# UCL-SML/Doubly-Stochastic-DGP

Hardware: AMD Instinct MI355X
Metric: ELBO-steps/sec (higher is better)
Workload: dtype f64

## Files before the change

### doubly-stochastic-dgp_amd/csrc/chain_policy.hpp

```cpp
#pragma once
#include <stdlib.h>
#include "plan_types.hpp"
#include "../../include/dsdgp.h"

#define XCH 64
#define HEAD_THREADS 512
#define GL_EPI_ROWS 64

#define SM_SMALL_BLOCKS 160
#define SM_BWD_RESIDENT_8W 768
static inline bool sm_small(int Mp, int64_t nblk, int D_in, bool bwd) {
  static const int64_t bwd_lim128 = getenv("DSDGP_SM_BWD_LIM128") ? atoll(getenv("DSDGP_SM_BWD_LIM128")) : SM_BWD_RESIDENT_8W;
  const int64_t lim = Mp > 128 ? ((int64_t)1 << 40) : (bwd ? bwd_lim128 : SM_SMALL_BLOCKS);
  return Mp >= 128 && Mp <= 256 && nblk <= lim && D_in <= XCH;
}
static inline int sm_nw(int Mp, int64_t nblk, int D_in, bool bwd) {
  return (Mp > 512 || (Mp == 512 && D_in <= XCH && !bwd)) ? 16 : (Mp > 256 ? 8 : (sm_small(Mp, nblk, D_in, bwd) ? 8 : 4));
}
static inline int64_t sm_hyp_parts(int64_t ld, int Mp, int D_in) { return (int64_t)sm_nw(Mp, ceil_div(ld, 16), D_in, true) * ceil_div(ld, 16); }
static inline int sm_adj_fusable(int Mp, int64_t nblk, int D_in, int D_out) {
  if (D_in > XCH) return 0;
  const int NW = sm_nw(Mp, nblk, D_in, true);
  const int xch = D_in < XCH ? D_in : XCH;
  return NW * 16 * xch >= 2 * 16 * D_out;
}
static inline int sm_cs_built(int Mp) { return Mp > 256 || Mp == 32 || Mp == 64 || Mp == 128 || Mp == 256; }

static inline bool save_c_enabled(int save_c, int Mp) { return save_c >= 2 || (save_c == 1 && Mp > 256); }
static inline int chain_d_split(int64_t nblk, int D_out) {
  int ds = 1;
  if (nblk < 256) ds = (int)std::min<int64_t>(4, std::max<int64_t>(1, 512 / nblk));
  else if (nblk < 512) ds = (int)std::min<int64_t>(1024 / nblk, D_out / 5);
  if (ds > D_out) ds = D_out;
  return ds < 1 ? 1 : ds;
}
static inline int bwd_d_split(int bwd_split, int Mp, bool has_part, int64_t nblk, int D_out) {
  const bool want = bwd_split >= 2 || (bwd_split == 1 && Mp > 256);
  return (want && has_part) ? chain_d_split(nblk, D_out) : 1;
}
static inline int layer_gemm_lik_blocks(int64_t Rin, int D_out) { return ceil_div(round_up(Rin, 16), GL_EPI_ROWS); }
static inline int head_draw_blocks(int64_t count) { return (int)std::min<int64_t>(64, ceil_div((count + 1) / 2, 4 * HEAD_THREADS)); }

static inline int layer_last_built(int Mp, int D_in, int D_out) { return (Mp == 128 || Mp == 256) && D_out == 1 && D_in <= 16; }
struct LastScope {
  int Mp, D_in, D_out, kern_kind;
  int hyp_rows;
  bool lik, save_A, save_C, want_F;
  int rep;
  bool whitened;
  int mean_kind, d_split;
  int bwd_d_split;
  bool want_E;
};
static inline int layer_last_fusable(const LastScope& s) {
  const int waves = s.Mp == 128 ? 4 : 8;
  return layer_last_built(s.Mp, s.D_in, s.D_out) && (s.kern_kind == DSDGP_KERN_RBF || s.kern_kind == DSDGP_KERN_MATERN52) &&
         s.hyp_rows >= waves && s.lik && s.save_A && !s.save_C && !s.want_F && s.rep == 1 && !s.whitened &&
         s.mean_kind == DSDGP_MEAN_ZERO && s.d_split <= 1 && s.bwd_d_split <= 1 && !s.want_E;
}
```

### doubly-stochastic-dgp_amd/csrc/common.hpp

```cpp
#pragma once
#include <hip/hip_runtime.h>
#include <stdint.h>
#include <stdlib.h>
#include <stdio.h>
#include <string.h>
#include <string>
#include <vector>
#include <map>

#include "../../include/dsdgp.h"

void dsdgp_set_error(const char* fmt, ...);

#define DS_HIP(call)                                                                         \
  do {                                                                                       \
    hipError_t e__ = (call);                                                                 \
    if (e__ != hipSuccess) {                                                                 \
      dsdgp_set_error("%s:%d: %s -> %s", __FILE__, __LINE__, #call, hipGetErrorString(e__)); \
      return DSDGP_ERR_HIP;                                                                  \
    }                                                                                        \
  } while (0)

#define DS_CHECK_ARG(cond)                                                  \
  do {                                                                      \
    if (!(cond)) {                                                          \
      dsdgp_set_error("%s:%d: bad argument: %s", __FILE__, __LINE__, #cond); \
      return DSDGP_ERR_BAD_ARG;                                             \
    }                                                                       \
  } while (0)

#include <atomic>
extern std::atomic<long long> g_dsdgp_launches;
#define DS_LAUNCH(...)                                                   \
  do {                                                                   \
    g_dsdgp_launches.fetch_add(1, std::memory_order_relaxed);            \
    hipLaunchKernelGGL(__VA_ARGS__);                                     \
  } while (0)

#define DS_TRY(call)            \
  do {                          \
    int rc__ = (call);          \
    if (rc__ != DSDGP_OK) return rc__; \
  } while (0)

struct ProfSlot {
  double ms = 0.0;
  int64_t launches = 0;
  std::vector<std::pair<hipEvent_t, hipEvent_t>> pending;
};

struct dsdgp_ctx {
  int device = 0;
  hipStream_t stream = nullptr;
  bool own_stream = false;
  hipStream_t side = nullptr;
  void* scratch = nullptr;
  size_t scratch_bytes = 0;
  int prof_on = 0;
  std::map<std::string, ProfSlot> prof;
  char* pin = nullptr;
  size_t pin_bytes = 0, pin_off = 0;
  void* potrf_plan = nullptr;
  void (*potrf_plan_free)(void*) = nullptr;
  int64_t potrf_key[4] = {0, 0, 0, 0};
};

int ctx_scratch(dsdgp_ctx* ctx, size_t bytes, void** out);
int ctx_upload(dsdgp_ctx* ctx, void* dst, const void* src, size_t bytes);

int multiclass_launch(dsdgp_ctx* ctx, const double* mean, const double* var, const double* Y, int64_t n, int64_t R, int K,
                      int mode, double wgt, double* out, double* dmean, double* dvar, int y_override);
int eval_mixture_launch(dsdgp_ctx* ctx, int kind, double p0, double p1, const double* p0_dev, const double* mean, const double* var,
                        const double* Y, int64_t n, int S, int DY, double* rows_out, double* acc, int accumulate);
int mixture_quantiles_launch(dsdgp_ctx* ctx, const double* mean, const double* var, double noise_var, const double* noise_dev,
                             int64_t n, int S, int DY, const double* probs, int P, double* q_out);
int mixture_calibration_launch(dsdgp_ctx* ctx, const double* mean, const double* var, double noise_var, const double* noise_dev,
                               const double* Y, int64_t n, int S, int DY, const double* probs, int P, double* rows_out, double* acc,
                               int accumulate);
int mixture_classification_launch(dsdgp_ctx* ctx, int kind, const double* mean, const double* var, const double* Y, int64_t n, int S,
                                  int DY, int bins, double* probs_out, double* rows_out, double* acc, int accumulate);

struct ProfScope {
  dsdgp_ctx* ctx;
  const char* name;
  hipEvent_t a = nullptr, b = nullptr;
  hipStream_t st;
  ProfScope(dsdgp_ctx* c, const char* n, hipStream_t stream = nullptr) : ctx(c), name(n), st(stream ? stream : c->stream) {
    if (ctx->prof_on) {
      hipEventCreate(&a);
      hipEventCreate(&b);
      hipEventRecord(a, st);
    }
  }
  ~ProfScope() {
    if (a) {
      hipEventRecord(b, st);
      ctx->prof[name].pending.push_back({a, b});
    }
  }
};

#ifdef __HIPCC__
#define DS_WAVE_ID(tid) __builtin_amdgcn_readfirstlane((int)(tid) >> 6)
#endif
#include "plan_types.hpp"
#define DSDGP_MAX_MP 2048

#ifdef __HIPCC__
typedef double d4 __attribute__((ext_vector_type(4)));
typedef const double __attribute__((address_space(1)))* gcptr;
typedef double __attribute__((address_space(1)))* gptr;
typedef double __attribute__((address_space(3)))* lptr;

#define DS_FIND_SEGMENT(idx, list, n, field, key)            \
  do {                                                       \
    int lo__ = 0, hi__ = (n)-1;                              \
    while (lo__ < hi__) {                                    \
      const int mid__ = (lo__ + hi__ + 1) >> 1;              \
      if ((key) >= (list)[mid__].field) lo__ = mid__;        \
      else hi__ = mid__ - 1;                                 \
    }                                                        \
    idx = lo__;                                              \
  } while (0)

__device__ __forceinline__ d4 mfma_f64(double a, double b, d4 c) {
  return __builtin_amdgcn_mfma_f64_16x16x4f64(a, b, c, 0, 0, 0);
}

__device__ __forceinline__ double sum_groups(double x) {
  const unsigned lo = __double2loint(x), hi = __double2hiint(x);
  const auto a = __builtin_amdgcn_permlane16_swap(lo, lo, false, false);
  const auto b = __builtin_amdgcn_permlane16_swap(hi, hi, false, false);
  const double y = __hiloint2double(b[0], a[0]) + __hiloint2double(b[1], a[1]);
  const unsigned lo2 = __double2loint(y), hi2 = __double2hiint(y);
  const auto c = __builtin_amdgcn_permlane32_swap(lo2, lo2, false, false);
  const auto d = __builtin_amdgcn_permlane32_swap(hi2, hi2, false, false);
  return __hiloint2double(d[0], c[0]) + __hiloint2double(d[1], c[1]);
}
template <int CTRL, int ROWMASK>
__device__ __forceinline__ double dpp_or_zero(double x) {
  const int lo = __builtin_amdgcn_update_dpp(0, __double2loint(x), CTRL, ROWMASK, 0xf, false);
  const int hi = __builtin_amdgcn_update_dpp(0, __double2hiint(x), CTRL, ROWMASK, 0xf, false);
  return __hiloint2double(hi, lo);
}
__device__ __forceinline__ double sum_wave(double x) {
  x += dpp_or_zero<0x111, 0xf>(x);
  x += dpp_or_zero<0x112, 0xf>(x);
  x += dpp_or_zero<0x114, 0xf>(x);
  x += dpp_or_zero<0x118, 0xf>(x);
  x += dpp_or_zero<0x142, 0xa>(x);
  x += dpp_or_zero<0x143, 0xc>(x);
  const unsigned lo = __builtin_amdgcn_readlane((int)__double2loint(x), 63);
  const unsigned hi = __builtin_amdgcn_readlane((int)__double2hiint(x), 63);
  return __hiloint2double(hi, lo);
}

template <int T>
__device__ __forceinline__ double block_sum(double x, double* red) {
  const int tid = threadIdx.x;
  __syncthreads();
  red[tid] = x;
  __syncthreads();
  for (int h = T / 2; h >= 1; h >>= 1) {
    if (tid < h) red[tid] += red[tid + h];
    __syncthreads();
  }
  return red[0];
}

template <int L>
__device__ __forceinline__ double bcast_lane(double x) {
  const unsigned lo = __builtin_amdgcn_readlane((int)__double2loint(x), L);
  const unsigned hi = __builtin_amdgcn_readlane((int)__double2hiint(x), L);
  return __hiloint2double((int)hi, (int)lo);
}

#define HYP_VAR 0
#define HYP_WVAR 1
#define HYP_KDIAG 2
#define HYP_DVAR 3
#define HYP_DWVAR 4
#define HYP_ILS 8

template <int KIND>
__device__ __forceinline__ double kern_val(double r2, double s2) {
  if (KIND == DSDGP_KERN_RBF) return s2 * exp(-0.5 * r2);
  const double s5 = 2.23606797749978969641;
  double r = sqrt(r2 + 1e-12);
  return s2 * (1.0 + s5 * r + (5.0 / 3.0) * (r * r)) * exp(-s5 * r);
}
template <int KIND>
__device__ __forceinline__ void kern_val_grad(double r2, double s2, double& k, double& dk) {
  if (KIND == DSDGP_KERN_RBF) {
    k = s2 * exp(-0.5 * r2);
    dk = -0.5 * k;
    return;
  }
  const double s5 = 2.23606797749978969641;
  double r = sqrt(r2 + 1e-12);
  double e = s2 * exp(-s5 * r);
  k = (1.0 + s5 * r + (5.0 / 3.0) * (r * r)) * e;
  dk = -(5.0 / 6.0) * (1.0 + s5 * r) * e;
}
__device__ __forceinline__ double kern_val_rt(int kind, double r2, double s2) {
  return kind == DSDGP_KERN_RBF ? kern_val<DSDGP_KERN_RBF>(r2, s2) : kern_val<DSDGP_KERN_MATERN52>(r2, s2);
}
#endif
```

### doubly-stochastic-dgp_amd/csrc/forward_plan.hpp

```cpp
#pragma once
#include "chain_policy.hpp"

static_assert(DSDGP_MAX_LAYERS <= 32, "FwdIn::caller_z is a 32-bit mask");
struct FwdIn {
  int64_t n;
  int S;
  bool prepare, save, need_last_F, lik_target, sample_w, with_grad;
  uint32_t caller_z;
  int L;
  bool white, lik_elementwise, lik_gaussian;
  int grad_first;
  bool grad_q_only, head_ok, overlap, timing;
  struct Layer {
    int Mp, M, D_in, D_out, kern_kind, mean_kind, prop;
    bool gemm, alg_g, need_tpt, has_C, has_bpart;
  } layer[DSDGP_MAX_LAYERS];
  struct { int white_fwd, cs_min_blocks, cs_min_dout, cs_max_dout, last_fuse, last_min_blocks, bwd_split, lik_fuse; } force;
};

enum DrawsAt : uint8_t { DRAWS_INLINE, DRAWS_HEAD, DRAWS_SIDE };
enum DrawFrom : uint8_t { DRAW_NONE, DRAW_CALLER, DRAW_HERE, DRAW_READY };
enum FwdLaunch : uint8_t { LAUNCH_CHAIN, LAUNCH_GEMM, LAUNCH_WITH_REVERSE };
enum LikRoute : uint8_t { LIK_NONE, LIK_IN_CHAIN, LIK_ELEMENTWISE, LIK_MULTICLASS };
struct FwdPlan {
  bool join_prep_first;
  DrawsAt draws;
  bool draws_ahead;
  int head_nblk;
  bool adjoints_from_lik, lik_in_chain;
  LikRoute lik;
  int lik_nblocks;
  struct Layer {
    int64_t Rin, ld;
    int rep;
    bool whitened, want_F;
    DrawFrom draw;
    bool save_A, save_C, save_XT1;
    int d_split;
    bool lik_epilogue;
    FwdLaunch launch;
    bool concat;
  } layer[DSDGP_MAX_LAYERS];
  int hyp_rows, bwd_d_split;
};

static inline bool last_chain_fusable(const FwdIn& in, const FwdPlan& p) {
  const int l = in.L - 1;
  const FwdIn::Layer& v = in.layer[l];
  const FwdPlan::Layer& y = p.layer[l];
  if (in.force.last_fuse == 0 || in.force.bwd_split >= 2 || !v.need_tpt || in.white || v.gemm || in.L < 2) return false;
  if (in.grad_q_only && in.grad_first == in.L - 1) return false;
  if (in.timing || ceil_div(y.Rin, 16) < in.force.last_min_blocks) return false;
  return layer_last_fusable(LastScope{v.Mp, v.D_in, v.D_out, v.kern_kind, p.hyp_rows, y.lik_epilogue, y.save_A, y.save_C, y.want_F, y.rep,
                                      y.whitened, v.mean_kind, y.d_split, p.bwd_d_split, !v.alg_g});
}

static inline FwdPlan fwd_plan(const FwdIn& in) {
  FwdPlan p{};
  const int L = in.L;
  const bool wf_ok = !in.white && !in.save && in.force.white_fwd != 0;
  p.join_prep_first = wf_ok;
  p.draws = !in.prepare ? DRAWS_INLINE : (in.head_ok ? DRAWS_HEAD : (in.overlap ? DRAWS_SIDE : DRAWS_INLINE));
  p.adjoints_from_lik = in.lik_target && in.with_grad && L > 1 && in.lik_elementwise;
  p.lik_in_chain = p.adjoints_from_lik && in.lik_gaussian && !in.sample_w && in.force.lik_fuse != 0;
  for (int l = 0; l < L; ++l) {
    const FwdIn::Layer& v = in.layer[l];
    FwdPlan::Layer& y = p.layer[l];
    const bool last = (l == L - 1);
    y.Rin = (l == 0) ? in.n : (int64_t)in.S * in.n;
    y.rep = (l == 0) ? in.S : 1;
    y.ld = round_up(y.Rin, 16);
    const int64_t nblk = y.ld / 16;
    y.want_F = !last || in.need_last_F;
    y.whitened = wf_ok && v.Mp <= 256 && !v.gemm;
    if (!y.want_F) y.draw = DRAW_NONE;
    else if (in.caller_z >> l & 1) y.draw = DRAW_CALLER;
    else y.draw = (p.draws != DRAWS_INLINE && !last) ? DRAW_READY : DRAW_HERE;
    if (y.draw == DRAW_READY) {
      p.draws_ahead = true;
      if (p.draws == DRAWS_HEAD) p.head_nblk = std::max(p.head_nblk, head_draw_blocks((int64_t)in.S * in.n * v.D_out));
    }
    y.save_A = in.save && (in.white || l >= in.grad_first);
    y.save_C = y.save_A && v.has_C && sm_cs_built(v.Mp) &&
               (v.Mp > 256 || (nblk > in.force.cs_min_blocks && v.D_out >= in.force.cs_min_dout && v.D_out <= in.force.cs_max_dout));
    if (v.gemm) y.save_C = y.save_A && v.has_C;
    const bool q_lowest = y.save_A && in.grad_q_only && !in.white && l == in.grad_first;
    if (q_lowest) y.save_C = false;
    y.save_XT1 = y.save_A && !q_lowest;
    y.d_split = chain_d_split(nblk, v.D_out);
    y.lik_epilogue = last && p.lik_in_chain;
    y.launch = v.gemm ? LAUNCH_GEMM : LAUNCH_CHAIN;
    y.concat = v.prop > 0 && !last;
  }
  const FwdIn::Layer& v = in.layer[L - 1];
  const FwdPlan::Layer& y = p.layer[L - 1];
  p.hyp_rows = (int)(sm_hyp_parts(y.ld, v.Mp, v.D_in) / (y.ld / 16));
  p.bwd_d_split = bwd_d_split(in.force.bwd_split, v.Mp, v.has_bpart, y.ld / 16, v.D_out);
  if (last_chain_fusable(in, p)) p.layer[L - 1].launch = LAUNCH_WITH_REVERSE;
  if (in.lik_target) {
    const int64_t R = (int64_t)in.S * in.n;
    p.lik = p.lik_in_chain ? LIK_IN_CHAIN : (in.lik_elementwise ? LIK_ELEMENTWISE : LIK_MULTICLASS);
    if (p.lik_in_chain) p.lik_nblocks = v.gemm ? layer_gemm_lik_blocks(y.Rin, v.D_out) : (int)(y.ld / 16) * y.d_split;
    else if (in.lik_elementwise) p.lik_nblocks = ceil_div((p.adjoints_from_lik ? round_up(R, 16) : R) * v.D_out, 256);
    else p.lik_nblocks = ceil_div(R, 256);
  }
  return p;
}

struct FwdUsed { const double *X, *z; int64_t zs_s, zs_n, zs_d; };
template <class FwdArgs>
struct FwdRecord {
  struct Layer : FwdUsed { int64_t Rin, ld; int rep; bool c_saved; } layer[DSDGP_MAX_LAYERS];
  int64_t n = 0;
  int S = 0;
  bool adjoints_from_lik = false;
  bool last_pending = false;
  FwdArgs last_fwd;
  int hyp_rows = 0;

  void forward_done(const FwdIn& in, const FwdPlan& p, const FwdUsed* used, const FwdArgs* pending) {
    n = in.n; S = in.S; adjoints_from_lik = p.adjoints_from_lik;
    for (int l = 0; l < in.L; ++l) {
      const FwdPlan::Layer& y = p.layer[l];
      Layer& r = layer[l];
      static_cast<FwdUsed&>(r) = used[l];
      r.Rin = y.Rin; r.ld = y.ld; r.rep = y.rep; r.c_saved = y.save_C;
    }
    last_pending = pending != nullptr;
    if (pending) { last_fwd = *pending; hyp_rows = p.hyp_rows; }
  }
  void adjoints_from_caller() { adjoints_from_lik = false; }
  void last_launched() { last_pending = false; }
};
```

### doubly-stochastic-dgp_amd/csrc/layer.hpp

```cpp
#pragma once
#include "common.hpp"
#include "chain_policy.hpp"

struct LayerFwdArgs {
  const double* X;
  int64_t Rin;
  int32_t rep;
  int32_t D_in, D_out, M;
  const double* Zp;
  const double* Zs;
  const double* hyp;
  const double* LinvT;
  const double* Linv;
  const double* Tp;
  const double* TpT;
  const double* qmu;
  int32_t qmu_ld;
  int32_t mean_kind;
  const double* mean_A;
  const double* mean_b;
  const double* z;
  int64_t zs_s, zs_n, zs_d;
  int64_t n_inner;
  double jitter;
  double* F;
  double* mean;
  double* var;
  double* Asave;
  double* Csave;
  int64_t ldA;
  int32_t d_split;
  double* XT1;
  unsigned long long* phase_clk;
  const double* lik_Y;
  const double* lik_const;
  double lik_w;
  double* lik_part;
  double *lik_MB, *lik_VB;
  int64_t lik_ld;
};

struct LayerBwdArgs {
  const double* X;
  int64_t Rin;
  int32_t D_in, D_out, M, DP4;
  const double* Zp;
  const double* Zs;
  const double* hyp;
  const double* Kinv;
  const double* Linv;
  const double* LinvT;
  const double* Sd;
  const double* qmu4;
  const double* Asave;
  const double* Csave;
  const double* Tp;
  const double* TpT;
  int64_t ldA;
  const double* VB;
  const double* MB;
  double* E;
  double* GW;
  double* dX;
  int32_t mean_kind;
  const double* mean_A;
  double* hyp_part;
  double* MBp;
  double* VBp;
  const double* zp;
  int64_t zp_s, zp_n, zp_d, n_inner;
  const double* varp;
  int32_t Dp, prop;
  double jitter;
  unsigned long long* phase_clk;
  int32_t d_split;
  double* part;
  int* part_cnt;
  const double* up_dF;
  int32_t up_rep, up_ld, up_off;
  const double* up_z;
  int64_t up_zs, up_zn, up_zd, up_n_inner;
  const double* up_var;
  double up_jitter;
  double *MBw, *VBw;
};

int wgrad_launch(dsdgp_ctx* ctx, const WgradJob* jobs_dev, int njobs, int total_tasks, int nsplit, int64_t ld, int64_t Rp,
                 hipStream_t stream = nullptr);
int layer_fwd_sm_launch(dsdgp_ctx* ctx, const LayerFwdArgs& a, int Mp, int kern_kind, int white);
int layer_bwd_sm_launch(dsdgp_ctx* ctx, const LayerBwdArgs& a, int Mp, int kern_kind, int white);
int layer_last_launch(dsdgp_ctx* ctx, const LayerFwdArgs& a, const LayerBwdArgs& b, int Mp, int kern_kind, int hyp_rows);

struct GemmLayerWs {
  double* T1;
  double* T2;
  double* Pb;
  double* colsq;
  double* MUT;
  double* qmuT;
  double* ZZ;
  double* OUTt;
  double* svar;
  int64_t pb_doubles;
};
#define GL_MAX_GROUPS 4
int layer_gemm_hyp_parts(int64_t ld, int Mp);
int layer_fwd_gemm_launch(dsdgp_ctx* ctx, const LayerFwdArgs& a, int Mp, int kern_kind, int white, const GemmLayerWs& ws);
int layer_bwd_gemm_launch(dsdgp_ctx* ctx, const LayerBwdArgs& b, int Mp, int kern_kind, int white, const GemmLayerWs& ws);
```

### doubly-stochastic-dgp_amd/csrc/layer_sm.hip

```cpp
#include <stdlib.h>

#include "layer.hpp"

int layer_fwd_sm_a(dsdgp_ctx*, const LayerFwdArgs&, int, int, int, int);
int layer_fwd_sm_b(dsdgp_ctx*, const LayerFwdArgs&, int, int, int, int);
int layer_fwd_sm_c(dsdgp_ctx*, const LayerFwdArgs&, int, int, int, int);
int layer_bwd_sm_a(dsdgp_ctx*, const LayerBwdArgs&, int, int, int, int);
int layer_bwd_sm_b(dsdgp_ctx*, const LayerBwdArgs&, int, int, int, int);
int layer_bwd_sm_c(dsdgp_ctx*, const LayerBwdArgs&, int, int, int, int);

int layer_fwd_sm_launch(dsdgp_ctx* ctx, const LayerFwdArgs& a, int Mp, int kern_kind, int white) {
  const int small = sm_small(Mp, ceil_div(a.Rin, 16), a.D_in, false);
  if (Mp < 128) return layer_fwd_sm_a(ctx, a, Mp, kern_kind, white, small);
  if (Mp <= 256) return layer_fwd_sm_b(ctx, a, Mp, kern_kind, white, small);
  return layer_fwd_sm_c(ctx, a, Mp, kern_kind, white, small);
}
int layer_bwd_sm_launch(dsdgp_ctx* ctx, const LayerBwdArgs& a, int Mp, int kern_kind, int white) {
  const int small = sm_small(Mp, ceil_div(a.ldA, 16), a.D_in, true);
  if (Mp < 128) return layer_bwd_sm_a(ctx, a, Mp, kern_kind, white, small);
  if (Mp <= 256) return layer_bwd_sm_b(ctx, a, Mp, kern_kind, white, small);
  return layer_bwd_sm_c(ctx, a, Mp, kern_kind, white, small);
}
```

### doubly-stochastic-dgp_amd/csrc/layer_sm_impl.hpp

```cpp
#pragma once
#include <stdlib.h>

#include "layer.hpp"

template <bool D4>
__device__ __forceinline__ int act_slot(int m) {
  return D4 ? ((m & ~15) | ((m & 3) << 2) | ((m >> 2) & 3)) : m;
}
template <bool D4>
__device__ __forceinline__ int out_slot(int ib, int g, int t) {
  return D4 ? 16 * ib + 4 * g + t : 16 * ib + g + 4 * t;
}

template <int Mp, bool D4>
__device__ __forceinline__ d4 chain_block(const double* __restrict__ WR, const double* __restrict__ WT,
                                          const double* __restrict__ actb, int ib, int kb, int g, int c, d4 acc) {
  if constexpr (D4) {
    const d4 w4 = *reinterpret_cast<const d4*>(WR + (int64_t)(16 * ib + c) * Mp + 16 * kb + 4 * g);
#pragma unroll
    for (int s = 0; s < 4; ++s) acc = mfma_f64(w4[s], actb[(16 * kb + 4 * s + g) * 16 + c], acc);
  } else {
    const double* __restrict__ w = WT + (int64_t)(16 * kb + g) * Mp + 16 * ib + c;
#pragma unroll
    for (int s = 0; s < 4; ++s) acc = mfma_f64(w[(int64_t)(4 * s) * Mp], actb[(16 * kb + 4 * s + g) * 16 + c], acc);
  }
  return acc;
}

template <int Mp, bool D4>
__device__ __forceinline__ d4 chain_range(const double* __restrict__ WR, const double* __restrict__ WT,
                                          const double* __restrict__ actb, int ib, int lo, int hi, int g, int c, d4 acc) {
  if constexpr (D4) {
#pragma unroll 4
    for (int kb = lo; kb < hi; ++kb) acc = chain_block<Mp, true>(WR, WT, actb, ib, kb, g, c, acc);
    return acc;
  } else {
    if (lo >= hi) return acc;
    const unsigned off = (unsigned)(g * Mp + 16 * ib + c);
    auto wld = [&](int kbx, int s) { return (WT + (size_t)(16 * kbx + 4 * s) * Mp)[off]; };
    double wa[4], wb[4];
    int kb = lo;
#pragma unroll
    for (int s = 0; s < 4; ++s) wa[s] = wld(kb, s);
    while (kb + 1 < hi) {
#pragma unroll
      for (int s = 0; s < 4; ++s) wb[s] = wld(kb + 1, s);
#pragma unroll
      for (int s = 0; s < 4; ++s) acc = mfma_f64(wa[s], actb[(16 * kb + 4 * s + g) * 16 + c], acc);
      ++kb;
      if (kb + 1 < hi) {
#pragma unroll
        for (int s = 0; s < 4; ++s) wa[s] = wld(kb + 1, s);
      }
#pragma unroll
      for (int s = 0; s < 4; ++s) acc = mfma_f64(wb[s], actb[(16 * kb + 4 * s + g) * 16 + c], acc);
      ++kb;
    }
    if (kb < hi) {
#pragma unroll
      for (int s = 0; s < 4; ++s) acc = mfma_f64(wa[s], actb[(16 * kb + 4 * s + g) * 16 + c], acc);
    }
    return acc;
  }
}

template <int Mp, bool UPPER>
__device__ __forceinline__ void chain_range2(const double* __restrict__ WT, const double* __restrict__ actb, int ib0, int ib1, int nkb,
                                             int g, int c, d4& acc0, d4& acc1) {
  const unsigned off0 = (unsigned)(g * Mp + 16 * ib0 + c), off1 = (unsigned)(g * Mp + 16 * ib1 + c);
  auto wld = [&](int kbx, int s, unsigned off) { return (WT + (size_t)(16 * kbx + 4 * s) * Mp)[off]; };
  if constexpr (UPPER) {
    acc0 = chain_range<Mp, false>(nullptr, WT, actb, ib0, ib0, ib1, g, c, acc0);
  }
  const int lo = UPPER ? ib1 : 0, hi = UPPER ? nkb : ib0 + 1;
  if (lo < hi) {
    double a0[4], a1[4];
    int kb = lo;
#pragma unroll
    for (int s = 0; s < 4; ++s) {
      a0[s] = wld(kb, s, off0);
      a1[s] = wld(kb, s, off1);
    }
    for (; kb + 1 < hi; ++kb) {
#pragma unroll
      for (int s = 0; s < 4; ++s) {
        const double bv = actb[(16 * kb + 4 * s + g) * 16 + c];
        acc0 = mfma_f64(a0[s], bv, acc0);
        acc1 = mfma_f64(a1[s], bv, acc1);
        a0[s] = wld(kb + 1, s, off0);
        a1[s] = wld(kb + 1, s, off1);
      }
#pragma unroll
      for (int s = 0; s < 4; ++s) {
        __builtin_amdgcn_sched_group_barrier(0x008, 2, 0);
        __builtin_amdgcn_sched_group_barrier(0x020, 2, 0);
      }
    }
#pragma unroll
    for (int s = 0; s < 4; ++s) {
      const double bv = actb[(16 * kb + 4 * s + g) * 16 + c];
      acc0 = mfma_f64(a0[s], bv, acc0);
      acc1 = mfma_f64(a1[s], bv, acc1);
    }
  }
  if constexpr (!UPPER) {
    acc1 = chain_range<Mp, false>(nullptr, WT, actb, ib1, ib0 + 1, ib1 + 1, g, c, acc1);
  }
}

template <int Mp, int MPB>
__device__ __forceinline__ void chain_dense2(const double* __restrict__ WT, const double* __restrict__ actb, int ib0, int ib1, int g, int c,
                                             d4& acc0, d4& acc1) {
  const unsigned off0 = (unsigned)(g * Mp + 16 * ib0 + c), off1 = (unsigned)(g * Mp + 16 * ib1 + c);
  auto wld = [&](int kbx, int s, unsigned off) { return (WT + (size_t)(16 * kbx + 4 * s) * Mp)[off]; };
  double a0[4], a1[4];
#pragma unroll
  for (int s = 0; s < 4; ++s) {
    a0[s] = wld(0, s, off0);
    a1[s] = wld(0, s, off1);
  }
  double bv = actb[g * 16 + c];
#pragma unroll
  for (int kb = 0; kb < MPB; ++kb) {
#pragma unroll
    for (int s = 0; s < 4; ++s) {
      const int kn = (s == 3) ? (kb + 1) % MPB : kb, sn = (s + 1) & 3;
      const double bvn = actb[(16 * kn + 4 * sn + g) * 16 + c];
      acc0 = mfma_f64(a0[s], bv, acc0);
      acc1 = mfma_f64(a1[s], bv, acc1);
      if (kb + 1 < MPB) {
        a0[s] = wld(kb + 1, s, off0);
        a1[s] = wld(kb + 1, s, off1);
      }
      bv = bvn;
      if (kb + 1 < MPB) __builtin_amdgcn_sched_barrier(0);
    }
  }
}

template <int MPB, int NW>
struct Own {
  static constexpr int NQ = (MPB + NW - 1) / NW;
  static __device__ __forceinline__ int ib(int wave, int q) {
    if (NQ >= 2) return (q & 1) ? (q >> 1) * (2 * NW) + (2 * NW - 1) - wave : (q >> 1) * (2 * NW) + wave;
    return wave;
  }
  static __device__ __forceinline__ bool skip(int ib) { return (MPB % NW != 0) && ib >= MPB; }
  static __device__ __forceinline__ bool active(int wave) { return MPB >= NW || wave < MPB; }
};

template <int MPB, int NW>
struct OwnCS {
  static constexpr bool CUSTOM = (NW == 8) && (MPB == 8 || MPB == 16);
  static constexpr int NQ = CUSTOM ? MPB / 8 : Own<MPB, NW>::NQ;
  static constexpr int NLOAD = CUSTOM ? 4 : NW;
  static __device__ __forceinline__ int ib(int wave, int q) {
    if constexpr (!CUSTOM) return Own<MPB, NW>::ib(wave, q);
    if constexpr (MPB == 8) return wave < 4 ? wave : 11 - wave;
    if (wave < 4) return q == 0 ? 7 - wave : wave;
    return q == 0 ? 19 - wave : 4 + wave;
  }
  static __device__ __forceinline__ bool active(int wave) { return CUSTOM || Own<MPB, NW>::active(wave); }
};

static inline constexpr int sm_db(int NW) { return NW == 4 ? 8 : (NW == 8 ? 4 : 1); }

struct SmLds {
  int xs, act, red, total;
};
static inline SmLds sm_lds(int Mp, int D_in, int D_out, int NW, bool wide, int nbuf = 1) {
  SmLds L;
  int o = 0;
  const int xch = D_in < XCH ? D_in : XCH;
  L.xs = o; o += 16 * (xch + 1);
  o = (int)round_up(o, 2);
  L.act = o; o += Mp * 16;
  L.red = o;
  const bool mu_early = (NW == 4) && !wide;
  const int db = sm_db(NW);
  const int red_fwd = NW * 16 + 2 * db * NW * 16 + (mu_early ? NW * 16 * D_out : 2 * db * NW * 16);
  const int red_bwd = NW * 16 * xch;
  int red = red_fwd > red_bwd ? red_fwd : red_bwd;
  if (nbuf == 2 && red < Mp * 16) red = Mp * 16;
  o += red;
  L.total = o;
  return L;
}

template <int NW>
__device__ __forceinline__ void stage_x_over_l(const double* X, const double* ils, double* xs, int Din, int j0, int jn, int64_t r0,
                                               int64_t Rin, int tid) {
  for (int idx = tid; idx < 16 * jn; idx += NW * 64) {
    const int rr = idx / jn, j = idx % jn;
    int64_t row = r0 + rr;
    if (row > Rin - 1) row = Rin - 1;
    xs[rr * (jn + 1) + j] = X[row * Din + j0 + j] * ils[j0 + j];
  }
}

template <int NQ, int MPB, int NW>
__device__ __forceinline__ void sqdist_chunk_masked(const double* __restrict__ zs, const double* xs, int Din, int j0, int jn, int wave,
                                                    int g, int c, d4 (&zx)[NQ], double (&zsq)[NQ], double& xx) {
  for (int kk = 0; kk < jn; kk += 16) {
    const int ns = (jn - kk >= 16) ? 4 : (jn - kk + 3) >> 2;
    double b[4];
    int jc[4];
    bool in[4];
#pragma unroll
    for (int s = 0; s < 4; ++s) {
      const int j = kk + 4 * s + g;
      in[s] = j < jn;
      jc[s] = in[s] ? j : jn - 1;
      const double v = xs[c * (jn + 1) + jc[s]];
      b[s] = in[s] ? v : 0.0;
      xx = fma(b[s], b[s], xx);
    }
#pragma unroll
    for (int q = 0; q < NQ; ++q) {
      const int ib = Own<MPB, NW>::ib(wave, q);
      if (Own<MPB, NW>::skip(ib)) continue;
      const double* __restrict__ zr = zs + (int64_t)(16 * ib + c) * Din + j0;
      double av[4];
#pragma unroll
      for (int s = 0; s < 4; ++s) {
        if (s < ns) {
          const double v = zr[jc[s]];
          av[s] = in[s] ? v : 0.0;
        }
      }
#pragma unroll
      for (int s = 0; s < 4; ++s) {
        if (s < ns) {
          zx[q] = mfma_f64(av[s], b[s], zx[q]);
          zsq[q] = fma(av[s], av[s], zsq[q]);
        }
      }
    }
  }
}
template <int NQ>
__device__ __forceinline__ void sqdist_finish(const d4 (&zx)[NQ], const double (&zsq)[NQ], double xx, double* scratch, int wave, int g,
                                              int c, d4 (&r2)[NQ]) {
  xx = sum_groups(xx);
  double* zrow = scratch + wave * NQ * 16;
#pragma unroll
  for (int q = 0; q < NQ; ++q) {
    const double zq = sum_groups(zsq[q]);
    if (g == 0) zrow[q * 16 + c] = zq;
  }
  __builtin_amdgcn_wave_barrier();
#pragma unroll
  for (int q = 0; q < NQ; ++q)
#pragma unroll
    for (int t = 0; t < 4; ++t) {
      const double v = zrow[q * 16 + g + 4 * t] + xx - 2.0 * zx[q][t];
      r2[q][t] = v > 0.0 ? v : 0.0;
    }
}
template <int NQ, int MPB, int NW>
__device__ __forceinline__ void sqdist_narrow(const double* __restrict__ zs, const double* xs, int Din, int wave, int g, int c, bool act,
                                              double* scratch, d4 (&r2)[NQ]) {
  d4 zx[NQ];
  double zsq[NQ];
#pragma unroll
  for (int q = 0; q < NQ; ++q) { zx[q] = (d4){0, 0, 0, 0}; zsq[q] = 0.0; }
  double xx = 0.0;
  if (act) sqdist_chunk_masked<NQ, MPB, NW>(zs, xs, Din, 0, Din, wave, g, c, zx, zsq, xx);
  sqdist_finish<NQ>(zx, zsq, xx, scratch, wave, g, c, r2);
}

template <int NQ, int MPB, int NW>
__device__ __forceinline__ void sm_sqdist(const double* __restrict__ zs, const double* __restrict__ X,
                                          const double* __restrict__ ils, double* xs, int Din, int64_t r0, int64_t Rin,
                                          int tid, int wave, int g, int c, bool act, double* scratch, d4 (&r2)[NQ]) {
  d4 zx[NQ];
  double zsq[NQ];
#pragma unroll
  for (int q = 0; q < NQ; ++q) { zx[q] = (d4){0, 0, 0, 0}; zsq[q] = 0.0; }
  double xx = 0.0;
  for (int j0 = 0; j0 < Din; j0 += XCH) {
    const int jn = (Din - j0 < XCH) ? Din - j0 : XCH;
    if (j0 > 0) __syncthreads();
    stage_x_over_l<NW>(X, ils, xs, Din, j0, jn, r0, Rin, tid);
    __syncthreads();
    if (act) {
      if ((jn & 15) == 0 && (Din & 3) == 0) {
#pragma unroll
        for (int u = 0; u < XCH / 16; ++u) {
          const int kk = 16 * u;
          if (kk >= jn) break;
          double b[4];
#pragma unroll
          for (int s = 0; s < 4; ++s) {
            b[s] = xs[c * (jn + 1) + kk + 4 * g + s];
            xx = fma(b[s], b[s], xx);
          }
#pragma unroll
          for (int q = 0; q < NQ; ++q) {
            const int ib = Own<MPB, NW>::ib(wave, q);
            if (Own<MPB, NW>::skip(ib)) continue;
            const d4 av = *reinterpret_cast<const d4*>(zs + (int64_t)(16 * ib + c) * Din + j0 + kk + 4 * g);
#pragma unroll
            for (int s = 0; s < 4; ++s) {
              zx[q] = mfma_f64(av[s], b[s], zx[q]);
// ... 239 lines not shown
  }
  fprintf(stderr, "[span] %d wgs: launch %.1f us | wg duration avg %.1f max %.1f us | start avg %.1f max %.1f us | %d late starters (avg duration %.1f us)\n",
          nwg, span, dur / nwg, dur_max, start / nwg, start_max, nlate, nlate ? late / nlate : 0.0);
  if (nwg >= 512) {
    double ds[8] = {0}, dx[8] = {0};
    int ns[8] = {0}, nx[8] = {0};
    for (int w = 0; w < nwg; ++w) {
      const double d = (double)(h[(size_t)w * 8 + last_slot] - h[(size_t)w * 8]) * 0.01;
      const int k = std::min(w >> 8, 7);
      ds[k] += d; ++ns[k]; dx[w & 7] += d; ++nx[w & 7];
    }
    fprintf(stderr, "[span]   mean duration by slot w >> 8:");
    for (int k = 0; k < 8 && ns[k]; ++k) fprintf(stderr, " %.1f", ds[k] / ns[k]);
    fprintf(stderr, " | by XCD w & 7:");
    for (int x = 0; x < 8; ++x) fprintf(stderr, " %.1f", dx[x] / std::max(nx[x], 1));
    fprintf(stderr, "\n");
  }
}
#define FWD_STAMP(i) do { if (a.phase_clk && tid == 0 && blockIdx.y == 0) a.phase_clk[(int64_t)blockIdx.x * 8 + (i)] = __builtin_amdgcn_s_memrealtime(); } while (0)
template <int MPB, int NW, bool WIDE, bool LIK>
constexpr int fwd_min_waves() { return (LIK && NW == 4) ? 5 : ((NW == 8 && MPB == 16 && !WIDE && !LIK) ? 4 : 1); }
template <int MPB, int NW, int KIND, bool WHITE, bool WIDE, bool LIK>
__global__ __launch_bounds__(NW * 64, (fwd_min_waves<MPB, NW, WIDE, LIK>())) void k_layer_fwd_sm(const LayerFwdArgs a, const SmLds L) {
  extern __shared__ __attribute__((aligned(16))) double smem[];
  constexpr int Mp = MPB * 16, NQ = Own<MPB, NW>::NQ;
  constexpr bool D4 = (MPB > 16);
  constexpr bool ILV = D4 || (MPB >= 16);
  const int Din = a.D_in, Dout = a.D_out;
  const int qld = a.qmu_ld ? a.qmu_ld : Dout;
  const int tid = threadIdx.x, lane = tid & 63, wave = DS_WAVE_ID(tid);
  const int g = lane >> 4, c = lane & 15;
  double* xs = smem + L.xs;
  double* actb = smem + L.act;
  double* red_s1 = smem + L.red;
  constexpr int DB = sm_db(NW);
  double* red_s2 = red_s1 + NW * 16;
  double* red_mu = red_s2 + 2 * DB * NW * 16;
  constexpr bool MU_EARLY = (NW == 4) && !WIDE;
  const double* ils = a.hyp + HYP_ILS;
  const int64_t r0 = (int64_t)blockIdx.x * 16;
  const bool act = Own<MPB, NW>::active(wave);
  const double s2 = a.hyp[HYP_VAR];
  FWD_STAMP(0);

  if (a.XT1 && blockIdx.y == 0) store_xt1<NW>(a, r0, tid);
  {
    d4 r2[NQ];
    if constexpr (!WIDE) {
      stage_x_over_l<NW>(a.X, ils, xs, Din, 0, Din, r0, a.Rin, tid);
      __syncthreads();
      sqdist_narrow<NQ, MPB, NW>(a.Zs, xs, Din, wave, g, c, act, red_s1, r2);
    } else {
      sm_sqdist<NQ, MPB, NW>(a.Zs, a.X, ils, xs, Din, r0, a.Rin, tid, wave, g, c, act, red_s1, r2);
    }
    if (act) {
#pragma unroll
      for (int q = 0; q < NQ; ++q) {
        const int ib = Own<MPB, NW>::ib(wave, q);
        if (Own<MPB, NW>::skip(ib)) continue;
        kuf_tile_store<KIND, D4>(r2[q], s2, a.M, actb, ib, g, c);
      }
    }
  }
  __syncthreads();
  FWD_STAMP(1);

  d4 acc[NQ];
#pragma unroll
  for (int q = 0; q < NQ; ++q) acc[q] = (d4){0, 0, 0, 0};
  constexpr bool PAIR = (NQ == 2) && !D4 && (MPB % NW == 0);
  if (act) {
    if constexpr (PAIR) {
      chain_range2<Mp, false>(a.LinvT, actb, Own<MPB, NW>::ib(wave, 0), Own<MPB, NW>::ib(wave, 1), MPB, g, c, acc[0], acc[1]);
    } else {
#pragma unroll
      for (int q = 0; q < NQ; ++q) {
        const int ib = Own<MPB, NW>::ib(wave, q);
        if (Own<MPB, NW>::skip(ib)) continue;
        acc[q] = chain_range<Mp, D4>(a.Linv, a.LinvT, actb, ib, 0, ib + 1, g, c, acc[q]);
      }
    }
  }
  sumsq_partial<NQ>(acc, red_s1, wave, g, c, act);
  __syncthreads();
  if (act) {
#pragma unroll
    for (int q = 0; q < NQ; ++q) {
      const int ib = Own<MPB, NW>::ib(wave, q);
      if (Own<MPB, NW>::skip(ib)) continue;
#pragma unroll
      for (int t = 0; t < 4; ++t) actb[out_slot<D4>(ib, g, t) * 16 + c] = acc[q][t];
    }
  }
  __syncthreads();
  FWD_STAMP(2);
  if (!WHITE) {
#pragma unroll
    for (int q = 0; q < NQ; ++q) acc[q] = (d4){0, 0, 0, 0};
    if (act) {
      if constexpr (PAIR) {
        chain_range2<Mp, true>(a.Linv, actb, Own<MPB, NW>::ib(wave, 0), Own<MPB, NW>::ib(wave, 1), MPB, g, c, acc[0], acc[1]);
      } else {
#pragma unroll
        for (int q = 0; q < NQ; ++q) {
          const int ib = Own<MPB, NW>::ib(wave, q);
          if (Own<MPB, NW>::skip(ib)) continue;
          acc[q] = chain_range<Mp, D4>(a.LinvT, a.Linv, actb, ib, ib, MPB, g, c, acc[q]);
        }
      }
    }
    __syncthreads();
    if (act) {
#pragma unroll
      for (int q = 0; q < NQ; ++q) {
        const int ib = Own<MPB, NW>::ib(wave, q);
        if (Own<MPB, NW>::skip(ib)) continue;
#pragma unroll
        for (int t = 0; t < 4; ++t) actb[out_slot<D4>(ib, g, t) * 16 + c] = acc[q][t];
      }
    }
  }
  FWD_STAMP(3);
  if constexpr (MU_EARLY) {
    for (int d0 = 0; d0 < Dout; d0 += 16) {
      d4 mu4 = (d4){0, 0, 0, 0};
      if (act) {
        const bool din = d0 + c < Dout;
        const int dc = din ? d0 + c : Dout - 1;
#pragma unroll
        for (int q = 0; q < NQ; ++q) {
          const int ib = Own<MPB, NW>::ib(wave, q);
          if (Own<MPB, NW>::skip(ib)) continue;
          double qv[4];
#pragma unroll
          for (int t = 0; t < 4; ++t) qv[t] = a.qmu[(int64_t)(16 * ib + g + 4 * t) * qld + dc];
#pragma unroll
          for (int t = 0; t < 4; ++t) mu4 = mfma_f64(din ? qv[t] : 0.0, acc[q][t], mu4);
        }
      }
#pragma unroll
      for (int t = 0; t < 4; ++t) {
        const int d = d0 + g + 4 * t;
        if (d < Dout) red_mu[(wave * Dout + d) * 16 + c] = mu4[t];
      }
    }
  }
  __syncthreads();
  FWD_STAMP(4);

  const double kdiag = a.hyp[HYP_KDIAG];
  const double lik_s2 = LIK ? a.lik_const[0] : 1.0;
  const double lik_c0 = -0.91893853320467274178 - 0.5 * log(lik_s2);
  double lik_ve = 0.0, lik_dl = 0.0;
  const int dchunk = (Dout + (int)gridDim.y - 1) / (int)gridDim.y;
  const int d_lo = (int)blockIdx.y * dchunk, d_hi = (d_lo + dchunk < Dout) ? d_lo + dchunk : Dout;
  for (int d0 = d_lo, grp = 0; d0 < d_hi; d0 += DB, ++grp) {
    const int gs = (d_hi - d0 < DB) ? d_hi - d0 : DB;
    double* rs2 = red_s2 + (grp & 1) * DB * NW * 16;
    double* rmu_g = red_mu + (grp & 1) * DB * NW * 16;
    for (int dd = 0; dd < gs; ++dd) {
      const int d = d0 + dd;
      d4 cacc[NQ];
#pragma unroll
      for (int q = 0; q < NQ; ++q) cacc[q] = (d4){0, 0, 0, 0};
      if (act) {
        const double* __restrict__ TdT = a.TpT + (int64_t)d * Mp * Mp;
        const double* __restrict__ Td = a.Tp + (int64_t)d * Mp * Mp;
        if constexpr (PAIR) {
          chain_range2<Mp, true>(Td, actb, Own<MPB, NW>::ib(wave, 0), Own<MPB, NW>::ib(wave, 1), MPB, g, c, cacc[0], cacc[1]);
        } else {
#pragma unroll
          for (int q = 0; q < NQ; ++q) {
            const int ib = Own<MPB, NW>::ib(wave, q);
            if (Own<MPB, NW>::skip(ib)) continue;
            cacc[q] = chain_range<Mp, D4>(TdT, Td, actb, ib, ib, MPB, g, c, cacc[q]);
          }
        }
      }
      double p = 0.0, mu = 0.0;
      if (act) {
        if (a.Csave) {
          const int64_t r = r0 + c;
          double* __restrict__ Cd = a.Csave + ((int64_t)blockIdx.x * Dout + d) * (Mp * 16) + c;
#pragma unroll
          for (int q = 0; q < NQ; ++q) {
            const int ib = Own<MPB, NW>::ib(wave, q);
            if (Own<MPB, NW>::skip(ib)) continue;
#pragma unroll
            for (int t = 0; t < 4; ++t) {
              const double cv = (r < a.Rin) ? cacc[q][t] : 0.0;
              Cd[out_slot<D4>(ib, g, t) * 16] = cv;
            }
          }
        }
#pragma unroll
        for (int q = 0; q < NQ; ++q) {
          const int ib = Own<MPB, NW>::ib(wave, q);
          if (Own<MPB, NW>::skip(ib)) continue;
#pragma unroll
          for (int t = 0; t < 4; ++t) {
            p = fma(cacc[q][t], cacc[q][t], p);
            if constexpr (!MU_EARLY) mu = fma(acc[q][t], a.qmu[(int64_t)(16 * ib + g + 4 * t) * qld + d], mu);
          }
        }
      }
      p = sum_groups(p);
      if constexpr (!MU_EARLY) mu = sum_groups(mu);
      if (g == 0) {
        rs2[(dd * NW + wave) * 16 + c] = p;
        if constexpr (!MU_EARLY) rmu_g[(dd * NW + wave) * 16 + c] = mu;
      }
    }
    __syncthreads();
    const bool flat = a.rep > 1 && a.mean_kind != DSDGP_MEAN_LINEAR;
    const int n_items = 16 * gs * (flat ? a.rep : 1);
    for (int e = tid; e < n_items; e += NW * 64) {
      const int s0 = flat ? e / (16 * gs) : 0, e2 = e % (16 * gs);
      const int cc = e2 / gs, dd = e2 % gs, d = d0 + dd;
      const int64_t r = r0 + cc;
      if (r >= a.Rin) {
        if (LIK && r < a.lik_ld && s0 == 0) {
          a.lik_MB[(int64_t)d * a.lik_ld + r] = 0.0;
          a.lik_VB[(int64_t)d * a.lik_ld + r] = 0.0;
        }
        continue;
      }
      double s1 = 0.0, s2sum = 0.0, mu = 0.0;
#pragma unroll
      for (int w = 0; w < NW; ++w) {
        s1 += red_s1[w * 16 + cc];
        s2sum += rs2[(dd * NW + w) * 16 + cc];
        mu += MU_EARLY ? red_mu[(w * Dout + d) * 16 + cc] : rmu_g[(dd * NW + w) * 16 + cc];
      }
      const double var = kdiag - s1 + s2sum;
      if (a.mean_kind == DSDGP_MEAN_IDENTITY) {
        mu += a.X[r * Din + d];
      } else if (a.mean_kind == DSDGP_MEAN_LINEAR) {
        double m2 = 0.0;
        for (int j = 0; j < Din; ++j) m2 = fma(a.X[r * Din + j], a.mean_A[(int64_t)j * Dout + d], m2);
        mu += m2 + (a.mean_b ? a.mean_b[d] : 0.0);
      }
      const double sd = sqrt(var + a.jitter);
      const int s_lo = flat ? s0 : 0, s_hi = flat ? s0 + 1 : a.rep;
      for (int s = s_lo; s < s_hi; ++s) {
        const int64_t orow = (int64_t)s * a.Rin + r;
        const int64_t o = orow * Dout + d;
        if (a.mean) a.mean[o] = mu;
        if (a.var) a.var[o] = var;
        if (a.F && a.z) {
          const double zv = a.z[(orow / a.n_inner) * a.zs_s + (orow % a.n_inner) * a.zs_n + d * a.zs_d];
          a.F[o] = mu + zv * sd;
        }
        if constexpr (LIK) {
          const double y = a.lik_Y[(orow % a.n_inner) * Dout + d];
          const double q = (y - mu) * (y - mu) + var;
          lik_ve += lik_c0 - 0.5 * q / lik_s2;
          lik_dl += -0.5 / lik_s2 + 0.5 * q / (lik_s2 * lik_s2);
          a.lik_MB[(int64_t)d * a.lik_ld + orow] = -a.lik_w * (y - mu) / lik_s2;
          a.lik_VB[(int64_t)d * a.lik_ld + orow] = 0.5 * a.lik_w / lik_s2;
        }
      }
    }
  }
  if constexpr (LIK) {
    lik_ve = sum_wave(lik_ve);
    lik_dl = sum_wave(lik_dl);
    __syncthreads();
    if (lane == 0) {
      red_s1[2 * wave] = lik_ve;
      red_s1[2 * wave + 1] = lik_dl;
    }
    __syncthreads();
    if (tid == 0) {
      double sv = 0.0, sd2 = 0.0;
      for (int w = 0; w < NW; ++w) {
        sv += red_s1[2 * w];
        sd2 += red_s1[2 * w + 1];
      }
      const int64_t wg = (int64_t)blockIdx.y * gridDim.x + blockIdx.x;
      a.lik_part[2 * wg] = sv;
      a.lik_part[2 * wg + 1] = sd2;
    }
  }
  FWD_STAMP(5);
  if (act && a.Asave && blockIdx.y == 0) {
    const int64_t r = r0 + c;
    if (r < a.ldA) {
#pragma unroll
      for (int q = 0; q < NQ; ++q) {
        const int ib = Own<MPB, NW>::ib(wave, q);
        if (Own<MPB, NW>::skip(ib)) continue;
#pragma unroll
        for (int t = 0; t < 4; ++t)
          a.Asave[(int64_t)(16 * ib + g + 4 * t) * a.ldA + r] = (r < a.Rin) ? actb[out_slot<D4>(ib, g, t) * 16 + c] : 0.0;
      }
    }
  }
  FWD_STAMP(6);
}

#define BWD_STAMP(i) do { if (a.phase_clk && tid == 0) a.phase_clk[(int64_t)blockIdx.x * 8 + (i)] = __builtin_amdgcn_s_memrealtime(); } while (0)
template <int MPB, int NW, bool WIDE, bool CS>
constexpr int bwd_min_waves() { return (NW == 8 && !WIDE && !CS) ? (MPB <= 8 ? 6 : 4) : ((NW == 4 && MPB == 8 && !WIDE && !CS) ? 5 : 1); }
template <int MPB, int NW, int KIND, bool WHITE, bool WIDE, bool CS>
__global__ __launch_bounds__(NW * 64, (bwd_min_waves<MPB, NW, WIDE, CS>())) void k_layer_bwd_sm(const LayerBwdArgs a, const SmLds L) {
  extern __shared__ __attribute__((aligned(16))) double smem[];
  constexpr int Mp = MPB * 16, NQ = Own<MPB, NW>::NQ;
  constexpr bool D4 = (MPB > 16);
  constexpr bool ILV = D4 || (MPB >= 16);
  const int Din = a.D_in, Dout = a.D_out;
  const int tid = threadIdx.x, lane = tid & 63, wave = tid >> 6;
  const int g = lane >> 4, c = lane & 15;
  const double* __restrict__ zs = a.Zs;
  double* xs = smem + L.xs;
  double* actb = smem + L.act;
  double* redx = smem + L.red;
  const double* ils = a.hyp + HYP_ILS;
  const int64_t r0 = (int64_t)blockIdx.x * 16;
  const bool act = Own<MPB, NW>::active(wave);
  const double s2 = a.hyp[HYP_VAR];
  const int64_t r = r0 + c;
  const bool rin = r < a.ldA, rvalid = r < a.Rin;
  BWD_STAMP(0);
  if (a.up_dF) adjoint_prologue<NW>(a, redx, L.total - L.red, r0, tid);
  d4 av[NQ], acc[NQ];
#pragma unroll
  for (int q = 0; q < NQ; ++q) {
    const int ib = Own<MPB, NW>::ib(wave, q);
    acc[q] = av[q] = (d4){0, 0, 0, 0};
    if (Own<MPB, NW>::skip(ib)) continue;
    const bool live = act && rin;
    const double* __restrict__ ap = a.Asave + (int64_t)(16 * (act ? ib : 0) + g) * a.ldA + (rin ? r : 0);
    double ld[4];
#pragma unroll
    for (int t = 0; t < 4; ++t) ld[t] = ap[(int64_t)(4 * t) * a.ldA];
#pragma unroll
    for (int t = 0; t < 4; ++t) {
      const double v = live ? ld[t] : 0.0;
      av[q][t] = v;
      if (!CS && act) actb[out_slot<D4>(ib, g, t) * 16 + c] = v;
    }
  }
  if constexpr (!WIDE) stage_x_over_l<NW>(a.X, ils, xs, Din, 0, Din, r0, a.Rin, tid);
  const double bv0l = a.MB[(int64_t)g * a.ldA + (rin ? r : 0)];
  const double bv1l = a.MB[(int64_t)(a.DP4 > 4 ? 4 + g : g) * a.ldA + (rin ? r : 0)];
  const double bv0 = (act && rin) ? bv0l : 0.0;
  const double bv1 = (act && rin && a.DP4 > 4) ? bv1l : 0.0;
  double gsum = 0.0;
  const int n_split = (int)gridDim.y;
  const int dchunk = (Dout + n_split - 1) / n_split;
  const int d_lo = (int)blockIdx.y * dchunk, d_hi = (d_lo + dchunk < Dout) ? d_lo + dchunk : Dout;
  __shared__ int s_ticket;
  auto merge_split = [&](auto& T, auto ib_of) -> bool {
    if (n_split == 1) return true;
    constexpr int NT = sizeof(T) / sizeof(T[0]);
    const int64_t pstride = (int64_t)Mp * 16 + 16;
    double* mine = a.part + ((int64_t)blockIdx.x * n_split + blockIdx.y) * pstride;
#pragma unroll
    for (int q = 0; q < NT; ++q) {
      const int ib = ib_of(q);
      if (ib < 0) continue;
#pragma unroll
      for (int t = 0; t < 4; ++t) __hip_atomic_store(&mine[(16 * ib + g + 4 * t) * 16 + c], T[q][t], __ATOMIC_RELAXED, __HIP_MEMORY_SCOPE_AGENT);
    }
    if (wave == 0 && g == 0) __hip_atomic_store(&mine[Mp * 16 + c], gsum, __ATOMIC_RELAXED, __HIP_MEMORY_SCOPE_AGENT);
    asm volatile("s_waitcnt vmcnt(0)" ::: "memory");
    __syncthreads();
    if (tid == 0) s_ticket = __hip_atomic_fetch_add(a.part_cnt + blockIdx.x, 1, __ATOMIC_RELAXED, __HIP_MEMORY_SCOPE_AGENT);
    __syncthreads();
    if (s_ticket != n_split - 1) return false;
    if (tid == 0) __hip_atomic_store(a.part_cnt + blockIdx.x, 0, __ATOMIC_RELAXED, __HIP_MEMORY_SCOPE_AGENT);
    const double* base = a.part + (int64_t)blockIdx.x * n_split * pstride;
#pragma unroll
    for (int q = 0; q < NT; ++q) T[q] = (d4){0, 0, 0, 0};
    gsum = 0.0;
    for (int y = 0; y < n_split; ++y) {
      const double* p = base + y * pstride;
#pragma unroll
      for (int q = 0; q < NT; ++q) {
        const int ib = ib_of(q);
        if (ib < 0) continue;
#pragma unroll
        for (int t = 0; t < 4; ++t) T[q][t] += __hip_atomic_load(&p[(16 * ib + g + 4 * t) * 16 + c], __ATOMIC_RELAXED, __HIP_MEMORY_SCOPE_AGENT);
      }
      gsum += __hip_atomic_load(&p[Mp * 16 + c], __ATOMIC_RELAXED, __HIP_MEMORY_SCOPE_AGENT);
    }
    return true;
  };
  BWD_STAMP(1);
  if constexpr (CS) {
    using OC = OwnCS<MPB, NW>;
    constexpr bool DBUF = (MPB <= 16);
    constexpr int NLT = OC::NLOAD * 64;
    constexpr int NS = Mp * 16 / (NLT * 2);
    double* buf1 = DBUF ? smem + L.red : actb;
    const bool stager = tid < NLT;
    const int e0 = 2 * tid;
    const int scc = e0 & 15;
    typedef double d2 __attribute__((ext_vector_type(2)));
    d2 tmp[NS];
    auto stage_load = [&](int d) {
      if (!stager) return;
      const d2 v2 = 2.0 * *reinterpret_cast<const d2*>(a.VB + (int64_t)d * a.ldA + r0 + scc);
      const double* __restrict__ Cd = a.Csave + ((int64_t)blockIdx.x * Dout + d) * (Mp * 16) + e0;
#pragma unroll
      for (int i = 0; i < NS; ++i) tmp[i] = v2 * *reinterpret_cast<const d2*>(Cd + i * 2 * NLT);
    };
    auto stage_store = [&](double* buf) {
      if (!stager) return;
#pragma unroll
      for (int i = 0; i < NS; ++i) *reinterpret_cast<d2*>(buf + e0 + i * 2 * NLT) = tmp[i];
    };
    constexpr bool PREF = (NW < 16);
    d4 cacc[OC::NQ];
#pragma unroll
    for (int q = 0; q < OC::NQ; ++q) cacc[q] = (d4){0, 0, 0, 0};
    const bool cact = OC::active(wave);
    if (PREF && d_lo < d_hi) stage_load(d_lo);
    if (DBUF && d_lo < d_hi) stage_store(actb);
    for (int d = d_lo; d < d_hi; ++d) {
      gsum += rin ? a.VB[(int64_t)d * a.ldA + r] : 0.0;
      const int dpar = (d - d_lo) & 1;
      double* cur = (DBUF && dpar) ? buf1 : actb;
      if (DBUF) {
        if (d + 1 < d_hi) stage_load(d + 1);
        __syncthreads();
      } else {
        __syncthreads();
        if (!PREF) stage_load(d);
        stage_store(actb);
        __syncthreads();
        if (PREF && d + 1 < d_hi) stage_load(d + 1);
      }
      if (cact) {
        const double* __restrict__ Td = a.Tp + (int64_t)d * Mp * Mp;
        const double* __restrict__ TdT = a.TpT + (int64_t)d * Mp * Mp;
#pragma unroll
        for (int q = 0; q < OC::NQ; ++q) {
          const int ib = OC::ib(wave, q);
          if (!OC::CUSTOM && Own<MPB, NW>::skip(ib)) continue;
#pragma unroll 4
          for (int kb = 0; kb <= ib; ++kb) cacc[q] = chain_block<Mp, D4>(Td, TdT, cur, ib, kb, g, c, cacc[q]);
        }
      }
      if (DBUF && d + 1 < d_hi) stage_store(dpar ? actb : buf1);
    }
    if (!merge_split(cacc, [&](int q) { const int ib = OC::ib(wave, q); return (cact && (OC::CUSTOM || !Own<MPB, NW>::skip(ib))) ? ib : -1; })) return;
    if (cact) {
      for (int sp = 0; sp < a.DP4 / 4; ++sp) {
        const double bv = sp == 0 ? bv0 : (sp == 1 ? bv1 : (rin ? a.MB[(int64_t)(4 * sp + g) * a.ldA + r] : 0.0));
#pragma unroll
        for (int q = 0; q < OC::NQ; ++q) {
          const int ib = OC::ib(wave, q);
          if (!OC::CUSTOM && Own<MPB, NW>::skip(ib)) continue;
          cacc[q] = mfma_f64(a.qmu4[(int64_t)(16 * ib + c) * a.DP4 + 4 * sp + g], bv, cacc[q]);
        }
      }
    }
    __syncthreads();
    if (cact) {
#pragma unroll
      for (int q = 0; q < OC::NQ; ++q) {
        const int ib = OC::ib(wave, q);
        if (!OC::CUSTOM && Own<MPB, NW>::skip(ib)) continue;
#pragma unroll
        for (int t = 0; t < 4; ++t) actb[out_slot<D4>(ib, g, t) * 16 + c] = cacc[q][t];
      }
    }
    __syncthreads();
    if (WHITE) {
      if (act) {
#pragma unroll
        for (int q = 0; q < NQ; ++q) {
          const int ib = Own<MPB, NW>::ib(wave, q);
          if (Own<MPB, NW>::skip(ib)) continue;
#pragma unroll
          for (int t = 0; t < 4; ++t) actb[out_slot<D4>(ib, g, t) * 16 + c] -= 2.0 * gsum * av[q][t];
        }
      }
      __syncthreads();
    }
  } else {
  __syncthreads();
  constexpr bool PAIRD = (NQ == 2) && !D4 && (MPB % NW == 0);
  if constexpr (PAIRD) {
    const int ib0 = Own<MPB, NW>::ib(wave, 0), ib1 = Own<MPB, NW>::ib(wave, 1);
    const unsigned off0 = (unsigned)(g * Mp + 16 * ib0 + c), off1 = (unsigned)(g * Mp + 16 * ib1 + c);
    const int t_last = d_hi * MPB - 1;
    auto wld = [&](int t, int s, unsigned off) { return (a.Sd + (size_t)(16 * t + 4 * s) * Mp)[off]; };
    double w0[4], w1[4];
    if (d_lo < d_hi) {
#pragma unroll
      for (int s = 0; s < 4; ++s) {
        w0[s] = wld(d_lo * MPB, s, off0);
        w1[s] = wld(d_lo * MPB, s, off1);
      }
    }
    const int64_t rc = rin ? r : 0;
    double vd_next = d_lo < d_hi ? a.VB[(int64_t)d_lo * a.ldA + rc] : 0.0;
    for (int d = d_lo; d < d_hi; ++d) {
      const double vd = rin ? vd_next : 0.0;
      gsum += vd;
      const double vd2 = 2.0 * vd;
      d4 y0 = (d4){0, 0, 0, 0}, y1 = (d4){0, 0, 0, 0};
      double bv = actb[g * 16 + c];
#pragma unroll
      for (int kb = 0; kb < MPB; ++kb) {
        int tn = d * MPB + kb + 1;
        if (kb == MPB - 1 && tn > t_last) tn = t_last;
#pragma unroll
        for (int s = 0; s < 4; ++s) {
          const int kn = (s == 3) ? (kb + 1) % MPB : kb, sn = (s + 1) & 3;
          const double bvn = actb[(16 * kn + 4 * sn + g) * 16 + c];
          y0 = mfma_f64(w0[s], bv, y0);
          y1 = mfma_f64(w1[s], bv, y1);
          w0[s] = wld(tn, s, off0);
          w1[s] = wld(tn, s, off1);
          bv = bvn;
          if (kb == 1 && s == 0) vd_next = a.VB[(int64_t)(d + 1 < d_hi ? d + 1 : d) * a.ldA + rc];
          __builtin_amdgcn_sched_barrier(0);
        }
      }
#pragma unroll
      for (int t = 0; t < 4; ++t) {
        acc[0][t] = fma(vd2, y0[t], acc[0][t]);
        acc[1][t] = fma(vd2, y1[t], acc[1][t]);
      }
    }
  } else
  for (int d = d_lo; d < d_hi; ++d) {
    const double vd = rin ? a.VB[(int64_t)d * a.ldA + r] : 0.0;
    gsum += vd;
    const double vd2 = 2.0 * vd;
    if (act) {
      const double* __restrict__ Sd = a.Sd + (int64_t)d * Mp * Mp;
      if constexpr (ILV) {
        d4 y[NQ];
#pragma unroll
        for (int q = 0; q < NQ; ++q) y[q] = (d4){0, 0, 0, 0};
#pragma unroll 4
        for (int kb = 0; kb < MPB; ++kb) {
#pragma unroll
          for (int q = 0; q < NQ; ++q) {
            const int ibq = Own<MPB, NW>::ib(wave, q);
            if (!Own<MPB, NW>::skip(ibq)) y[q] = chain_block<Mp, D4>(Sd, Sd, actb, ibq, kb, g, c, y[q]);
          }
        }
#pragma unroll
        for (int q = 0; q < NQ; ++q)
#pragma unroll
          for (int t = 0; t < 4; ++t) acc[q][t] = fma(vd2, y[q][t], acc[q][t]);
      } else {
#pragma unroll
        for (int q = 0; q < NQ; ++q) {
          const int ib = Own<MPB, NW>::ib(wave, q);
          if (Own<MPB, NW>::skip(ib)) continue;
          const double* __restrict__ W = Sd + 16 * ib + c + (int64_t)g * Mp;
          d4 y = (d4){0, 0, 0, 0};
#pragma unroll 4
          for (int kb = 0; kb < MPB; ++kb) {
#pragma unroll
            for (int s = 0; s < 4; ++s)
              y = mfma_f64(W[(int64_t)(16 * kb + 4 * s) * Mp], actb[(16 * kb + 4 * s + g) * 16 + c], y);
          }
#pragma unroll
          for (int t = 0; t < 4; ++t) acc[q][t] = fma(vd2, y[t], acc[q][t]);
        }
      }
    }
  }
  if (!merge_split(acc, [&](int q) { const int ib = Own<MPB, NW>::ib(wave, q); return (act && !Own<MPB, NW>::skip(ib)) ? ib : -1; })) return;
  }
  BWD_STAMP(2);
  if constexpr (!CS) {
  if (act) {
    for (int sp = 0; sp < a.DP4 / 4; ++sp) {
      const double bv = sp == 0 ? bv0 : (sp == 1 ? bv1 : (rin ? a.MB[(int64_t)(4 * sp + g) * a.ldA + r] : 0.0));
#pragma unroll
      for (int q = 0; q < NQ; ++q) {
        const int ib = Own<MPB, NW>::ib(wave, q);
        if (Own<MPB, NW>::skip(ib)) continue;
        acc[q] = mfma_f64(a.qmu4[(int64_t)(16 * ib + c) * a.DP4 + 4 * sp + g], bv, acc[q]);
      }
    }
  }
  __syncthreads();
  if (act) {
#pragma unroll
    for (int q = 0; q < NQ; ++q) {
      const int ib = Own<MPB, NW>::ib(wave, q);
      if (Own<MPB, NW>::skip(ib)) continue;
#pragma unroll
      for (int t = 0; t < 4; ++t) {
        if (WHITE) acc[q][t] -= 2.0 * gsum * av[q][t];
        actb[out_slot<D4>(ib, g, t) * 16 + c] = acc[q][t];
      }
    }
  }
  __syncthreads();
  }
  BWD_STAMP(3);
  d4 bb[NQ];
#pragma unroll
  for (int q = 0; q < NQ; ++q) bb[q] = (d4){0, 0, 0, 0};
  constexpr bool PAIRK = (NQ == 2) && !D4 && !CS && (MPB % NW == 0);
  if constexpr (PAIRK) {
    if constexpr (WHITE) {
      const int wu = DS_WAVE_ID(tid);
      chain_range2<Mp, true>(a.Linv, actb, Own<MPB, NW>::ib(wu, 0), Own<MPB, NW>::ib(wu, 1), MPB, g, c, bb[0], bb[1]);
    } else {
      chain_dense2<Mp, MPB>(a.Kinv, actb, Own<MPB, NW>::ib(wave, 0), Own<MPB, NW>::ib(wave, 1), g, c, bb[0], bb[1]);
    }
  } else
  if (act) {
    if (WHITE || !ILV) {
#pragma unroll
      for (int q = 0; q < NQ; ++q) {
        const int ib = Own<MPB, NW>::ib(wave, q);
        if (Own<MPB, NW>::skip(ib)) continue;
#pragma unroll 4
        for (int kb = (WHITE ? ib : 0); kb < MPB; ++kb)
          bb[q] = WHITE ? chain_block<Mp, D4>(a.LinvT, a.Linv, actb, ib, kb, g, c, bb[q])
                        : chain_block<Mp, D4>(a.Kinv, a.Kinv, actb, ib, kb, g, c, bb[q]);
      }
    } else {
#pragma unroll 4
      for (int kb = 0; kb < MPB; ++kb) {
#pragma unroll
        for (int q = 0; q < NQ; ++q) {
          const int ibq = Own<MPB, NW>::ib(wave, q);
          if (!Own<MPB, NW>::skip(ibq)) bb[q] = chain_block<Mp, D4>(a.Kinv, a.Kinv, actb, ibq, kb, g, c, bb[q]);
        }
      }
    }
  }
  BWD_STAMP(4);
  d4 r2[NQ];
  if constexpr (WIDE) sm_sqdist<NQ, MPB, NW>(zs, a.X, ils, xs, Din, r0, a.Rin, tid, wave, g, c, act, redx, r2);
  else sqdist_narrow<NQ, MPB, NW>(zs, xs, Din, wave, g, c, act, redx, r2);
  __syncthreads();
  BWD_STAMP(5);
  double svar = 0.0;
  if (act) {
#pragma unroll
    for (int q = 0; q < NQ; ++q) {
      const int ib = Own<MPB, NW>::ib(wave, q);
      if (Own<MPB, NW>::skip(ib)) continue;
#pragma unroll
      for (int t = 0; t < 4; ++t) {
        const int m = 16 * ib + g + 4 * t;
        const double e = WHITE ? bb[q][t] : bb[q][t] - gsum * av[q][t];
        const double kbar = WHITE ? e : e - gsum * av[q][t];
        bb[q][t] = kbar_to_w<KIND>(kbar, r2[q][t], s2, rvalid && (m < a.M), svar);
        if (rin && a.E) a.E[(int64_t)m * a.ldA + r] = e;
      }
    }
  }
  BWD_STAMP(6);
  double* hp = hyp_part_row(a, NW, wave);
  hyp_head_store(svar, gsum, s2, rvalid, hp, wave, lane);
  if constexpr (!(NW == 4 && MPB == 8 && !WIDE && !CS)) {
    input_side_epilogue<NQ, MPB, NW, WIDE>(a, bb, xs, redx, hp, r0, tid, wave, g, c, act);
  } else {
    for (int j0 = 0; j0 < Din; j0 += XCH) {
      const int jn = (Din - j0 < XCH) ? Din - j0 : XCH;
      const bool single = 16 * jn <= NW * 64;
      double pre_mb = 0.0, pre_z = 0.0, pre_var = 1.0;
      if ((a.dX || a.MBp) && single && tid < 16 * jn) {
        const int j = a.MBp ? tid / 16 : tid % jn, cc = a.MBp ? tid % 16 : tid / jn;
        const int64_t row = r0 + cc;
        if (row < a.Rin) {
          if (a.mean_kind == DSDGP_MEAN_IDENTITY) pre_mb = a.MB[(int64_t)(j0 + j) * a.ldA + row];
          const int d = j0 + j - a.prop;
          if (a.MBp && d >= 0) {
            pre_z = a.zp[(row / a.n_inner) * a.zp_s + (row % a.n_inner) * a.zp_n + d * a.zp_d];
            pre_var = a.varp[row * a.Dp + d];
          }
        }
      }
      double w1 = 0.0;
      if (act) {
#pragma unroll
        for (int q = 0; q < NQ; ++q)
#pragma unroll
          for (int t = 0; t < 4; ++t) w1 += bb[q][t];
      }
      w1 = sum_groups(w1);
      for (int kk = 0; kk < jn; kk += 16) {
        d4 wz = (d4){0, 0, 0, 0}, z2 = (d4){0, 0, 0, 0};
        if (act) {
          const int jc = (kk + c < jn) ? kk + c : jn - 1;
#pragma unroll
          for (int q = 0; q < NQ; ++q) {
            const int ib = Own<MPB, NW>::ib(wave, q);
            if (Own<MPB, NW>::skip(ib)) continue;
            double zv[4];
#pragma unroll
            for (int t = 0; t < 4; ++t) zv[t] = zs[(int64_t)(16 * ib + g + 4 * t) * Din + j0 + jc];
#pragma unroll
            for (int t = 0; t < 4; ++t) {
              wz = mfma_f64(zv[t], bb[q][t], wz);
              z2 = mfma_f64(zv[t] * zv[t], bb[q][t], z2);
            }
          }
        }
#pragma unroll
        for (int t = 0; t < 4; ++t) {
          const int j = kk + g + 4 * t;
          const bool in = j < jn;
          const double xv = xs[c * (jn + 1) + (in ? j : jn - 1)];
          if ((a.dX || a.MBp) && in) redx[(wave * jn + j) * 16 + c] = act ? fma(xv, w1, -wz[t]) : 0.0;
          double sl = act ? fma(xv * xv, w1, fma(-2.0 * xv, wz[t], z2[t])) : 0.0;
          sl += dpp_or_zero<0x111, 0xf>(sl);
          sl += dpp_or_zero<0x112, 0xf>(sl);
          sl += dpp_or_zero<0x114, 0xf>(sl);
          sl += dpp_or_zero<0x118, 0xf>(sl);
          if (c == 15 && in) hp[2 + j0 + j] = -2.0 * ils[j0 + j] * sl;
        }
      }
      if (a.dX || a.MBp) {
        __syncthreads();
        for (int idx = tid; idx < 16 * jn; idx += NW * 64) {
          const int j = a.MBp ? idx / 16 : idx % jn, cc = a.MBp ? idx % 16 : idx / jn;
          const int64_t row = r0 + cc;
          if (row < a.Rin) {
            double sx = 0.0;
#pragma unroll
            for (int w = 0; w < NW; ++w) sx += redx[(w * jn + j) * 16 + cc];
            double dx = 2.0 * ils[j0 + j] * sx;
            if (a.mean_kind == DSDGP_MEAN_IDENTITY) {
              dx += single ? pre_mb : a.MB[(int64_t)(j0 + j) * a.ldA + row];
            } else if (a.mean_kind == DSDGP_MEAN_LINEAR) {
              for (int d = 0; d < Dout; ++d) dx = fma(a.mean_A[(int64_t)(j0 + j) * Dout + d], a.MB[(int64_t)d * a.ldA + row], dx);
            }
            if (a.MBp) {
              const int d = j0 + j - a.prop;
              if (d >= 0) {
                const double zv = single ? pre_z : a.zp[(row / a.n_inner) * a.zp_s + (row % a.n_inner) * a.zp_n + d * a.zp_d];
                const double vv = single ? pre_var : a.varp[row * a.Dp + d];
                a.MBp[(int64_t)d * a.ldA + row] = dx;
                a.VBp[(int64_t)d * a.ldA + row] = dx * zv * 0.5 * rsqrt(vv + a.jitter);
              }
            } else {
              a.dX[row * Din + j0 + j] = dx;
            }
          } else if (a.MBp && row < a.ldA && j0 + j >= a.prop) {
            a.MBp[(int64_t)(j0 + j - a.prop) * a.ldA + row] = 0.0;
            a.VBp[(int64_t)(j0 + j - a.prop) * a.ldA + row] = 0.0;
          }
        }
      }
    }
  }
  if (act && rin) acc_to_global<NQ, MPB, NW>(bb, a.GW, a.ldA, r, true, wave, g);
  BWD_STAMP(7);
}


template <int MPB, int NW, int KIND, bool WHITE, bool WIDE, bool LIK>
static int fwd_sm_go2(dsdgp_ctx* ctx, const LayerFwdArgs& a) {
  const SmLds L = sm_lds(MPB * 16, a.D_in, a.D_out, NW, WIDE);
  const size_t lds = (size_t)L.total * sizeof(double);
  if (lds > 160 * 1024) {
    dsdgp_set_error("layer_fwd(sm): needs %zu B LDS (> 160 KiB): D_out too large for this M", lds);
    return DSDGP_ERR_UNSUPPORTED;
  }
  if (lds > 64 * 1024)
    {
      static int lds_set = 0;
      if ((int)lds > lds_set) {
        DS_HIP(hipFuncSetAttribute((const void*)k_layer_fwd_sm<MPB, NW, KIND, WHITE, WIDE, LIK>, hipFuncAttributeMaxDynamicSharedMemorySize, (int)lds));
        lds_set = (int)lds;
      }
    }
  ProfScope ps(ctx, "layer_fwd");
  const int nrow = ceil_div(a.Rin, 16);
  int ds = a.d_split > 0 ? a.d_split : 1;
  if (ds > a.D_out) ds = a.D_out;
  static const bool timing = getenv("DSDGP_FWD_TIMING") != nullptr;
  if (timing) {
    unsigned long long* clk = nullptr;
    DS_HIP(hipMalloc(&clk, (size_t)nrow * 8 * sizeof(unsigned long long)));
    LayerFwdArgs b = a;
    b.phase_clk = clk;
    DS_LAUNCH((k_layer_fwd_sm<MPB, NW, KIND, WHITE, WIDE, LIK>), dim3(nrow, ds), dim3(NW * 64), lds, ctx->stream, b, L);
    DS_HIP(hipStreamSynchronize(ctx->stream));
    std::vector<unsigned long long> h((size_t)nrow * 8);
    DS_HIP(hipMemcpy(h.data(), clk, h.size() * sizeof(unsigned long long), hipMemcpyDeviceToHost));
    hipFree(clk);
    double ph[6] = {0, 0, 0, 0, 0, 0};
    for (int w = 0; w < nrow; ++w)
      for (int i = 0; i < 6; ++i) ph[i] += (double)(h[(size_t)w * 8 + i + 1] - h[(size_t)w * 8 + i]);
    phase_span_report(h, nrow, 6);
    const double u = 0.01 / nrow;
    fprintf(stderr, "[fwd phases] Mp=%d NW=%d D_out=%d wgs=%dx%d  us/wg: Kuf tile %.2f | a1 %.2f | a %.2f | mean partials %.2f | per-output + epilogue %.2f | "
            "Asave %.2f | sum %.2f\n", MPB * 16, NW, a.D_out, nrow, ds, ph[0] * u, ph[1] * u, ph[2] * u, ph[3] * u, ph[4] * u,
            ph[5] * u, (ph[0] + ph[1] + ph[2] + ph[3] + ph[4] + ph[5]) * u);
    return DSDGP_OK;
  }
  DS_LAUNCH((k_layer_fwd_sm<MPB, NW, KIND, WHITE, WIDE, LIK>), dim3(nrow, ds), dim3(NW * 64), lds, ctx->stream, a, L);
  DS_HIP(hipGetLastError());
  return DSDGP_OK;
}
template <int MPB, int NW, int KIND, bool WHITE, bool WIDE>
static int fwd_sm_go(dsdgp_ctx* ctx, const LayerFwdArgs& a) {
  if (a.lik_Y) return fwd_sm_go2<MPB, NW, KIND, WHITE, WIDE, true>(ctx, a);
  return fwd_sm_go2<MPB, NW, KIND, WHITE, WIDE, false>(ctx, a);
}
template <int MPB, int NW, int KIND, bool WHITE, bool WIDE, bool CS>
static int bwd_phase_timing(dsdgp_ctx* ctx, const LayerBwdArgs& a0, const SmLds& L, size_t lds) {
  const int nwg = (int)ceil_div(a0.ldA, 16);
  unsigned long long* clk = nullptr;
  DS_HIP(hipMalloc(&clk, (size_t)nwg * 8 * sizeof(unsigned long long)));
  LayerBwdArgs a = a0;
  a.phase_clk = clk;
  DS_LAUNCH((k_layer_bwd_sm<MPB, NW, KIND, WHITE, WIDE, CS>), dim3(nwg, a.d_split > 1 ? a.d_split : 1), dim3(NW * 64), lds, ctx->stream, a, L);
  DS_HIP(hipStreamSynchronize(ctx->stream));
  std::vector<unsigned long long> h((size_t)nwg * 8);
  DS_HIP(hipMemcpy(h.data(), clk, h.size() * sizeof(unsigned long long), hipMemcpyDeviceToHost));
  hipFree(clk);
  double ph[7] = {0, 0, 0, 0, 0, 0, 0};
  for (int w = 0; w < nwg; ++w) {
    for (int i = 0; i < 7; ++i) ph[i] += (double)(h[(size_t)w * 8 + i + 1] - h[(size_t)w * 8 + i]);
  }
  phase_span_report(h, nwg, 7);
  const double u = 0.01 / nwg;
  fprintf(stderr, "[bwd phases] Mp=%d NW=%d D_out=%d wgs=%d  us/wg: A-tile %.2f | d-loop %.2f | mean+abar %.2f | Kinv %.2f | x-stage %.2f | "
          "kernel+E/GW %.2f | hyp+dX %.2f | sum %.2f\n", MPB * 16, NW, a.D_out, nwg, ph[0] * u, ph[1] * u, ph[2] * u, ph[3] * u, ph[4] * u, ph[5] * u,
          ph[6] * u, (ph[0] + ph[1] + ph[2] + ph[3] + ph[4] + ph[5] + ph[6]) * u);
  return DSDGP_OK;
}
template <int MPB, int NW, int KIND, bool WHITE, bool WIDE, bool CS>
static int bwd_sm_go2(dsdgp_ctx* ctx, const LayerBwdArgs& a) {
  const SmLds L = sm_lds(MPB * 16, a.D_in, a.D_out, NW, WIDE, (CS && MPB <= 16) ? 2 : 1);
  const size_t lds = (size_t)L.total * sizeof(double);
  if (lds > 160 * 1024) {
    dsdgp_set_error("layer_bwd(sm): needs %zu B LDS (> 160 KiB)", lds);
    return DSDGP_ERR_UNSUPPORTED;
  }
  if (lds > 64 * 1024)
    {
      static int lds_set = 0;
      if ((int)lds > lds_set) {
        DS_HIP(hipFuncSetAttribute((const void*)k_layer_bwd_sm<MPB, NW, KIND, WHITE, WIDE, CS>, hipFuncAttributeMaxDynamicSharedMemorySize, (int)lds));
        lds_set = (int)lds;
      }
    }
  ProfScope ps(ctx, "layer_bwd");
  static const bool timing = getenv("DSDGP_BWD_TIMING") != nullptr;
  if (timing) return bwd_phase_timing<MPB, NW, KIND, WHITE, WIDE, CS>(ctx, a, L, lds);
  DS_LAUNCH((k_layer_bwd_sm<MPB, NW, KIND, WHITE, WIDE, CS>), dim3(ceil_div(a.ldA, 16), a.d_split > 1 ? a.d_split : 1), dim3(NW * 64), lds,
                     ctx->stream, a, L);
  DS_HIP(hipGetLastError());
  return DSDGP_OK;
}
template <int MPB, int NW>
constexpr bool sm_cs_inst() { return MPB > 16 || MPB == 2 || MPB == 4 || MPB == 8 || MPB == 16; }
template <int MPB, int NW, int KIND, bool WHITE, bool WIDE>
static int bwd_sm_go(dsdgp_ctx* ctx, const LayerBwdArgs& a) {
  if constexpr (sm_cs_inst<MPB, NW>()) {
    if (a.Csave) return bwd_sm_go2<MPB, NW, KIND, WHITE, WIDE, true>(ctx, a);
  }
  return bwd_sm_go2<MPB, NW, KIND, WHITE, WIDE, false>(ctx, a);
}



#define SM_CASE2(FN, MPB, NW, KIND, ARGS)                                                              \
  if (wide) return white ? FN<MPB, NW, KIND, true, true> ARGS : FN<MPB, NW, KIND, false, true> ARGS;      \
  return white ? FN<MPB, NW, KIND, true, false> ARGS : FN<MPB, NW, KIND, false, false> ARGS;
#define SM_CASE(FN, MPB, NW, ARGS)                                           \
  case MPB * 16:                                                             \
    if (kern_kind == DSDGP_KERN_RBF) { SM_CASE2(FN, MPB, NW, DSDGP_KERN_RBF, ARGS) }   \
    SM_CASE2(FN, MPB, NW, DSDGP_KERN_MATERN52, ARGS)
#define SM_SMALL_CASE(FN, MPB, ARGS)                                                                       \
  if (Mp == MPB * 16) {                                                                                    \
    if (kern_kind == DSDGP_KERN_RBF)                                                                       \
      return white ? FN<MPB, 8, DSDGP_KERN_RBF, true, false> ARGS : FN<MPB, 8, DSDGP_KERN_RBF, false, false> ARGS; \
    return white ? FN<MPB, 8, DSDGP_KERN_MATERN52, true, false> ARGS : FN<MPB, 8, DSDGP_KERN_MATERN52, false, false> ARGS; \
  }
#define SM_NOT_BUILT                                                                     \
  dsdgp_set_error("layer chain: padded inducing count %d not built (32..1024)", Mp);     \
  return DSDGP_ERR_UNSUPPORTED;
```

### doubly-stochastic-dgp_amd/csrc/model.hip

```cpp
#include "layer.hpp"
#include "likelihood.hpp"
#include "linalg.hpp"
#include <stdlib.h>
#include <hip/hip_ext.h>

int gram_launch(dsdgp_ctx* ctx, int kind, const double* X, int64_t n, const double* X2, int64_t n2, int D,
                const double* hyp_dev, double diag_add, int symmetric, double* out, int64_t ld);

#define SOFTPLUS_LOWER 1e-6

#include "model_plan.hpp"
#include "prepare_plan.hpp"
#include "forward_plan.hpp"
#include "model_types.hpp"
#include "model_layout.hpp"
#include "model_kernels.hpp"

static int validate_desc(const dsdgp_model_desc* d) {
  DS_CHECK_ARG(d && d->L >= 1 && d->L <= DSDGP_MAX_LAYERS && d->n_theta > 0);
  DS_CHECK_ARG(d->lik_kind == DSDGP_LIK_MULTICLASS || lik_family(d->lik_kind) != LIKF_NONE);
  DS_CHECK_ARG((d->lik_kind != DSDGP_LIK_POISSON && d->lik_kind != DSDGP_LIK_STUDENT_T) || d->lik_aux > 0.0);
  DS_CHECK_ARG(!lik_has_param(d->lik_kind) || (d->off_lik_var >= 0 && d->off_lik_var < d->n_theta));
  for (int l = 0; l < d->L; ++l) {
    const dsdgp_layer_desc& y = d->layers[l];
    DS_CHECK_ARG(y.M >= 1 && y.D_in >= 1 && y.D_out >= 1);
    DS_CHECK_ARG(y.kern_kind == DSDGP_KERN_RBF || y.kern_kind == DSDGP_KERN_MATERN52);
    if (pad_M(y.M) > DSDGP_MAX_MP) {
      dsdgp_set_error("layer %d: M=%d inducing points: built up to M = %d", l, y.M, DSDGP_MAX_MP);
      return DSDGP_ERR_UNSUPPORTED;
    }
    DS_CHECK_ARG(y.input_prop_dim >= 0 && y.input_prop_dim <= y.D_in);
    if (l > 0) DS_CHECK_ARG(y.D_in == d->layers[l - 1].D_out + d->layers[l - 1].input_prop_dim);
    if (y.mean_kind == DSDGP_MEAN_IDENTITY) DS_CHECK_ARG(y.D_in == y.D_out);
    if (y.mean_kind == DSDGP_MEAN_LINEAR) DS_CHECK_ARG(y.mean_A != nullptr || y.off_mean_A >= 0);
  }
  return DSDGP_OK;
}

extern "C" int dsdgp_model_workspace_bytes(const dsdgp_model_desc* desc, int64_t n_max, int32_t s_max, int64_t* bytes) {
  DS_TRY(validate_desc(desc));
  DS_CHECK_ARG(bytes && n_max > 0 && s_max > 0);
  dsdgp_model tmp{};
  parse_force(&tmp);
  tmp.desc = *desc;
  tmp.n_max = n_max;
  tmp.s_max = s_max;
  size_t total = 0;
  layout(&tmp, nullptr, &total);
  *bytes = (int64_t)total;
  return DSDGP_OK;
}

static void fill_gemm(GemmProblem& P, const double* A, const double* B, double* C, int m, int n, int k, int lda, int ldb,
                      int ldc, int tA, int tB, int batch, int64_t sA, int64_t sB, int64_t sC, int reduce) {
  memset(&P, 0, sizeof(P));
  P.A = A; P.B = B; P.C = C;
  P.m = m; P.n = n; P.k = k;
  P.lda = lda; P.ldb = ldb; P.ldc = ldc;
  P.transA = tA; P.transB = tB;
  P.batch = batch; P.sA = sA; P.sB = sB; P.sC = sC; P.batch_reduce = reduce;
  P.alpha = 1.0; P.beta = 0.0;
}

extern "C" int dsdgp_model_create(dsdgp_ctx* ctx, const dsdgp_model_desc* desc, int64_t n_max, int32_t s_max,
                                  double* theta, double* grad, double* adam_m, double* adam_v, void* workspace,
                                  int64_t workspace_bytes, dsdgp_model** out) {
  DS_CHECK_ARG(ctx && out && theta && workspace);
  DS_TRY(validate_desc(desc));
  DS_CHECK_ARG(((uintptr_t)workspace & 255) == 0);
  DS_CHECK_ARG(((uintptr_t)theta & 15) == 0 && ((uintptr_t)grad & 15) == 0 && ((uintptr_t)adam_m & 15) == 0 && ((uintptr_t)adam_v & 15) == 0);
  dsdgp_model* m = new dsdgp_model();
  parse_force(m);
  m->ctx = ctx;
  m->desc = *desc;
  m->n_max = n_max;
  m->s_max = s_max;
  m->theta = theta; m->grad = grad; m->adam_m = adam_m; m->adam_v = adam_v;
  size_t total = 0;
  layout(m, (char*)workspace, &total);
  for (int l = 0; l < desc->L; ++l)
    if (m->L[l].dev.Mp > 1024 && !m->L[l].gemm) {
      dsdgp_set_error("layer %d: M=%d needs the GEMM-formulated passes, which DSDGP_FORCE switched off", l, desc->layers[l].M);
      delete m;
      return DSDGP_ERR_UNSUPPORTED;
    }
  if ((int64_t)total > workspace_bytes) {
    dsdgp_set_error("workspace too small: need %zu bytes, got %lld", total, (long long)workspace_bytes);
    delete m;
    return DSDGP_ERR_WORKSPACE;
  }
  hipStream_t st = ctx->stream;
  DS_HIP(hipMemsetAsync(workspace, 0, total, st));
  for (int l = 0; l < desc->L; ++l) {
    LayerState& S = m->L[l];
    S.meanA = (S.dev.off_mean_A >= 0) ? theta + S.dev.off_mean_A : S.d.mean_A;
    S.meanb = (S.dev.off_mean_b >= 0) ? theta + S.dev.off_mean_b : nullptr;
  }
  const int L = desc->L;
  std::vector<LayerDev> ld(L);
  std::vector<PotrfItem> items(L);
  std::vector<GemmProblem> gf, g1, g2, w1, w2, w3, wz, gpt;
  m->gemm_order_used = 0;
  auto plan_lpt = [&](GemmProblem* probs, int n) -> int {
    std::vector<int32_t> order;
    const int total = gemm_plan_lpt(probs, n, order);
    if (order.empty() || m->gemm_order_used + (int64_t)order.size() > m->gemm_order_cap) return gemm_plan(probs, n);
    int32_t* dst = m->gemm_order + m->gemm_order_used;
    if (hipMemcpyAsync(dst, order.data(), order.size() * sizeof(int32_t), hipMemcpyHostToDevice, st) != hipSuccess ||
        hipStreamSynchronize(st) != hipSuccess)
      return gemm_plan(probs, n);
    for (int i = 0; i < n; ++i) {
      probs[i].order = dst;
      probs[i].n_order = (int32_t)(order.size() / 2);
    }
    m->gemm_order_used += (int64_t)order.size();
    return total;
  };
  int64_t asm_elems = 0;
  for (int l = 0; l < L; ++l) {
    const LayerDev& v = m->L[l].dev;
    ld[l] = v;
    items[l] = PotrfItem{v.Kp, v.Linv, v.LinvT, v.scal, v.Mp, v.Mp, v.M,
                         getenv("DSDGP_POTRF_TIMING") ? 7 : (desc->white ? 0 : 8) , 0, 0};
    const int Mp = v.Mp;
    const int64_t MM = (int64_t)Mp * Mp;
    GemmProblem P;
    const size_t gf0 = gf.size() + 1, g10 = g1.size(), g20 = g2.size(), gp0 = gpt.size();
    fill_gemm(P, v.LinvT, v.Linv, v.Kinv, Mp, Mp, Mp, Mp, Mp, Mp, 0, 0, 1, 0, 0, 0, 0);
    P.lower_only = 1; P.tri = 8 | 1 | 16;
    gf.push_back(P);
    fill_gemm(P, v.Linv, v.Tp, v.V, Mp, Mp, Mp, Mp, Mp, Mp, 0, 0, v.D_out, 0, MM, MM, 0);
    P.lower_only = 1; P.tri = 2 | 1;
    gf.push_back(P);
    fill_gemm(P, v.Linv, v.qmu4, v.nL, Mp, v.DP4, Mp, Mp, v.DP4, v.DP4, 0, 0, 1, 0, 0, 0, 0);
    P.tri = 2;
    gf.push_back(P);
    if (!(Mp > 256 && save_c_enabled(m->force.save_c, Mp)) || v.alg_g) {
      fill_gemm(P, v.Tp, v.Tp, v.Sd, Mp, Mp, Mp, Mp, Mp, Mp, 0, 1, v.D_out, MM, MM, MM, 0);
      P.lower_only = 1; P.tri = 2 | 4 | 16;
      gf.push_back(P);
    }
    fill_gemm(P, v.Kinv, v.Tp, v.U, Mp, Mp, Mp, Mp, Mp, Mp, 0, 0, v.D_out, 0, MM, MM, 0);
    P.tri = 1;
    g1.push_back(P);
    fill_gemm(P, v.Kinv, v.qmu4, v.n4, Mp, v.DP4, Mp, Mp, v.DP4, v.DP4, 0, 0, 1, 0, 0, 0, 0);
    g1.push_back(P);
    fill_gemm(P, v.bigred + MM, v.Tp, v.PT, Mp, Mp, Mp, Mp, Mp, Mp, 0, 0, v.D_out, MM, MM, MM, 0);
    P.lower_only = 1; P.tri = 1;
    gpt.push_back(P);
    if (v.alg_g) {
      fill_gemm(P, v.Kinv, v.Sd, v.KS, Mp, Mp, Mp, Mp, Mp, Mp, 0, 0, v.D_out, 0, MM, MM, 0);
      g1.push_back(P);
      fill_gemm(P, v.KS, v.bigred + MM, v.GS, Mp, Mp, Mp, Mp, Mp, Mp, 0, 0, v.D_out, MM, MM, MM, 0);
      gpt.push_back(P);
    }
    fill_gemm(P, v.U, v.U, v.UU, Mp, Mp, Mp, Mp, Mp, Mp, 0, 1, v.D_out, MM, MM, MM, 0);
    P.lower_only = 1; P.tri = 16;
    g2.push_back(P);
    if (v.D_in > WIDE_DIN) {
      fill_gemm(P, v.wm, v.Zp1, v.WZ, Mp, v.DinP16, Mp, Mp, v.DinP16, v.DinP16, 0, 0, 1, 0, 0, 0, 0);
      wz.push_back(P);
    }
    {
      LayerState& Sq = m->L[l];
      std::vector<GemmProblem> lq(gf.begin() + gf0, gf.end());
      Sq.lq_nf = (int)lq.size();
      Sq.lq_tf = plan_lpt(lq.data(), Sq.lq_nf);
      std::vector<GemmProblem> q1(g1.begin() + g10, g1.end()), q2(g2.begin() + g20, g2.end());
      Sq.lq_n1 = (int)q1.size(); Sq.lq_t1 = plan_lpt(q1.data(), Sq.lq_n1);
      Sq.lq_n2 = (int)q2.size(); Sq.lq_t2 = plan_lpt(q2.data(), Sq.lq_n2);
      std::vector<GemmProblem> qp(gpt.begin() + gp0, gpt.end());
      Sq.lq_np = (int)qp.size(); Sq.lq_tp = plan_lpt(qp.data(), Sq.lq_np);
      lq.insert(lq.end(), q1.begin(), q1.end());
      lq.insert(lq.end(), q2.begin(), q2.end());
      lq.insert(lq.end(), qp.begin(), qp.end());
      DS_CHECK_ARG(lq.size() <= 12);
      DS_HIP(hipMemcpyAsync(Sq.lq, lq.data(), lq.size() * sizeof(GemmProblem), hipMemcpyHostToDevice, st));
      DS_HIP(hipStreamSynchronize(st));
    }
    m->kuu_blocks = std::max(m->kuu_blocks, std::min(1024, (Mp / 16) * (Mp / 16)));
    asm_elems = std::max<int64_t>(asm_elems, (int64_t)v.D_out * v.M * v.M);
    m->prep_blocks = (int)std::max<int64_t>(m->prep_blocks, std::min<int64_t>(2048, (int64_t)v.D_out * Mp * Mp / 2048));
    fill_gemm(P, v.bigred + MM, v.Tp, v.PT, Mp, Mp, Mp, Mp, Mp, Mp, 0, 0, v.D_out, MM, MM, MM, 0);
    w1.push_back(P);
    fill_gemm(P, v.Kp, v.wLbar, v.wH, Mp, Mp, Mp, Mp, Mp, Mp, 1, 0, 1, 0, 0, 0, 0);
    w1.push_back(P);
    fill_gemm(P, v.wH, v.Linv, v.wY, Mp, Mp, Mp, Mp, Mp, Mp, 0, 0, 1, 0, 0, 0, 0);
    w2.push_back(P);
    fill_gemm(P, v.Linv, v.wY, v.wX, Mp, Mp, Mp, Mp, Mp, Mp, 1, 0, 1, 0, 0, 0, 0);
    w3.push_back(P);
    {
      LayerState& St = m->L[l];
      GemmProblem ng[4];
      fill_gemm(ng[0], v.ngTI, v.ngTbar, v.ngH, Mp, Mp, Mp, Mp, Mp, Mp, 1, 0, v.D_out, MM, MM, MM, 0);
      fill_gemm(ng[1], v.ngTinv, v.ngTinv, v.ngSinv, Mp, Mp, Mp, Mp, Mp, Mp, 1, 0, v.D_out, MM, MM, MM, 0);
      ng[0].lower_only = 1; ng[0].tri = 8 | 1;
      ng[1].lower_only = 1; ng[1].tri = 8 | 1 | 16;
      St.ng_t1 = plan_lpt(ng, 2);
      fill_gemm(ng[2], v.ngH, v.ngTinv, v.ngY, Mp, Mp, Mp, Mp, Mp, Mp, 0, 0, v.D_out, MM, MM, MM, 0);
      ng[2].tri = 2 | 1;
      St.ng_t2 = plan_lpt(ng + 2, 1);
      fill_gemm(ng[3], v.ngTinv, v.ngY, v.ngX, Mp, Mp, Mp, Mp, Mp, Mp, 1, 0, v.D_out, MM, MM, MM, 0);
      ng[3].tri = 8 | 1;
      St.ng_t3 = plan_lpt(ng + 3, 1);
      DS_HIP(hipMemcpyAsync(St.ng_gp, ng, sizeof(ng), hipMemcpyHostToDevice, st));
      std::vector<PotrfItem> it(v.D_out);
      for (int d = 0; d < v.D_out; ++d)
        it[d] = PotrfItem{v.ngA + d * MM, v.ngLAinv + d * MM, v.ngLAinvT + d * MM, v.ngScal + 2 * d, Mp, Mp, v.M, 0, 0, 0};
      DS_HIP(hipMemcpyAsync(St.ng_items, it.data(), it.size() * sizeof(PotrfItem), hipMemcpyHostToDevice, st));
      DS_HIP(hipStreamSynchronize(st));
      St.big = Mp >= big_mp(m->uniform_big) && Mp % 64 == 0;
      if (St.big) {
        const bool need_lu = desc->white != 0;
        if (!m->uniform_big) DS_TRY(bigchol_build(ctx, St.big_k, v.Kp, v.Linv, v.LinvT, v.scal, 1, MM, 2, Mp, v.M, nullptr, false, need_lu));
        else if (l == 0) DS_TRY(bigchol_build(ctx, m->big_all, v.Kp, v.Linv, v.LinvT, v.scal, L, MM, 8, Mp, v.M, nullptr, false, need_lu));
        DS_TRY(bigchol_build(ctx, St.big_ngA, v.ngA, v.ngLAinv, v.ngLAinvT, v.ngScal, v.D_out, MM, 2, Mp, v.M, nullptr, false, false));
        DS_TRY(bigchol_build(ctx, St.big_ngT, v.ngTI, v.ngTinv, nullptr, nullptr, v.D_out, MM, 0, Mp, v.M, nullptr, true));
      }
    }
  }
  m->tail_ok = m->force.tail != 0 && !desc->white;
  for (int l = 0; l < L; ++l) {
    m->tail_ok = m->tail_ok && m->L[l].dev.D_in <= WIDE_DIN;
    m->mp_max_all = std::max(m->mp_max_all, (int)m->L[l].dev.Mp);
    m->m_max_all = std::max(m->m_max_all, (int)m->L[l].dev.M);
  }
  for (int l = 0; l < L; ++l) {
    LayerDev& v = m->L[l].dev;
    const bool fold = v.D_in <= WIDE_DIN && (int64_t)m->kuu_blocks * 256 >= (int64_t)v.Mp * v.Mp;
    v.hyp_parts = m->tail_ok ? v.M : (fold ? m->kuu_blocks : -NPART);
    ld[l].hyp_parts = v.hyp_parts;
    v.kl_parts = ld[l].kl_parts = m->mp_max_all >= 512 ? 512 : NPART;
    if (!fold) m->need_hyp_part = true;
  }
  m->head_ok = m->force.head != 0 && !m->uniform_big;
  for (int l = 0; l < L; ++l) m->head_ok = m->head_ok && m->L[l].dev.Mp <= HEAD_MAX_N && m->L[l].dev.D_in <= HEAD_MAX_DIN;
  m->n_fwd = (int)gf.size(); m->t_fwd = plan_lpt(gf.data(), m->n_fwd);
  m->n_bwd1 = (int)g1.size(); m->t_bwd1 = plan_lpt(g1.data(), m->n_bwd1);
  m->n_pt = (int)gpt.size(); m->t_pt = plan_lpt(gpt.data(), m->n_pt);
  DS_HIP(hipMemcpyAsync(m->gp_pt, gpt.data(), gpt.size() * sizeof(GemmProblem), hipMemcpyHostToDevice, st));
  m->n_bwd2 = (int)g2.size(); m->t_bwd2 = plan_lpt(g2.data(), m->n_bwd2);
  m->n_wz = (int)wz.size();
  if (m->n_wz) {
    m->t_wz = plan_lpt(wz.data(), m->n_wz);
    DS_HIP(hipMemcpyAsync(m->gp_wz, wz.data(), wz.size() * sizeof(GemmProblem), hipMemcpyHostToDevice, st));
  }
  m->asm_blocks = (int)std::min<int64_t>(2048, std::max<int64_t>(64, asm_elems / 1024));
  m->n_w = L;
  m->t_w1 = plan_lpt(w1.data(), 2 * L); m->t_w2 = plan_lpt(w2.data(), L); m->t_w3 = plan_lpt(w3.data(), L);
  DS_HIP(hipMemcpyAsync(m->gp_w1, w1.data(), w1.size() * sizeof(GemmProblem), hipMemcpyHostToDevice, st));
  DS_HIP(hipMemcpyAsync(m->gp_w2, w2.data(), w2.size() * sizeof(GemmProblem), hipMemcpyHostToDevice, st));
  DS_HIP(hipMemcpyAsync(m->gp_w3, w3.data(), w3.size() * sizeof(GemmProblem), hipMemcpyHostToDevice, st));
  DS_HIP(hipMemcpyAsync(m->layers_dev, ld.data(), L * sizeof(LayerDev), hipMemcpyHostToDevice, st));
  DS_HIP(hipMemcpyAsync(m->potrf_items, items.data(), L * sizeof(PotrfItem), hipMemcpyHostToDevice, st));
  DS_HIP(hipMemcpyAsync(m->gp_fwd, gf.data(), gf.size() * sizeof(GemmProblem), hipMemcpyHostToDevice, st));
  DS_HIP(hipMemcpyAsync(m->gp_bwd1, g1.data(), g1.size() * sizeof(GemmProblem), hipMemcpyHostToDevice, st));
  DS_HIP(hipMemcpyAsync(m->gp_bwd2, g2.data(), g2.size() * sizeof(GemmProblem), hipMemcpyHostToDevice, st));
  std::vector<double> mask(desc->n_theta, 0.0);
  auto mark = [&](int64_t off, int64_t cnt, int on) {
    for (int64_t i = 0; i < cnt; ++i) mask[off + i] = (double)on;
  };
  for (int l = 0; l < L; ++l) {
    const dsdgp_layer_desc& y = desc->layers[l];
    mark(y.off_Z, (int64_t)y.M * y.D_in, y.trainable_Z);
    mark(y.off_q_mu, (int64_t)y.M * y.D_out, y.trainable_q_mu);
    if (y.trainable_q_sqrt)
      for (int64_t d = 0; d < y.D_out; ++d)
        for (int64_t i = 0; i < y.M; ++i) mark(y.off_q_sqrt + (d * y.M + i) * y.M, i + 1, 1);
    mark(y.off_kvar, 1, 2 * y.trainable_kvar);
    mark(y.off_kls, y.ard ? y.D_in : 1, 2 * y.trainable_kls);
    if (y.has_white) mark(y.off_wvar, 1, 2 * y.trainable_wvar);
    if (y.mean_kind == DSDGP_MEAN_LINEAR && y.off_mean_A >= 0) mark(y.off_mean_A, (int64_t)y.D_in * y.D_out, y.trainable_mean_A);
    if (y.mean_kind == DSDGP_MEAN_LINEAR && y.off_mean_b >= 0) mark(y.off_mean_b, y.D_out, y.trainable_mean_b);
  }
  if (lik_has_param(desc->lik_kind)) mark(desc->off_lik_var, 1, 2 * desc->trainable_lik_var);
  DS_HIP(hipMemcpyAsync(m->mask, mask.data(), mask.size() * sizeof(double), hipMemcpyHostToDevice, st));
  DS_HIP(hipStreamSynchronize(st));
  m->overlap = !(getenv("DSDGP_NO_OVERLAP") && atoi(getenv("DSDGP_NO_OVERLAP")));
  if (!ctx->side) DS_HIP(hipStreamCreateWithFlags(&ctx->side, hipStreamNonBlocking));
  m->side = ctx->side;

  const unsigned evf = hipEventDisableTiming;
  for (int l = 0; l < L; ++l) {
    DS_HIP(hipEventCreateWithFlags(&m->ev_bwd[l], evf));
  }
  DS_HIP(hipEventCreateWithFlags(&m->ev_side, evf));
  DS_HIP(hipEventCreateWithFlags(&m->ev_fork, evf));
  DS_HIP(hipEventCreateWithFlags(&m->ev_prep_side, evf));
  DS_HIP(hipEventCreateWithFlags(&m->ev_z, evf));
  DS_HIP(hipEventCreateWithFlags(&m->ev_kinv, evf));
  m->plan_n = -1;
  m->plan_S = -1;
  *out = m;
  return DSDGP_OK;
}

extern "C" int dsdgp_model_destroy(dsdgp_model* m) {
  if (m) {
    hipStreamSynchronize(m->ctx->stream);
    hipStreamSynchronize(m->side);

    for (int l = 0; l < m->desc.L; ++l) {
      hipEventDestroy(m->ev_bwd[l]);
    }
    hipEventDestroy(m->ev_side);

    hipEventDestroy(m->ev_fork); hipEventDestroy(m->ev_prep_side); hipEventDestroy(m->ev_z); hipEventDestroy(m->ev_kinv);
    for (int l = 0; l < m->desc.L; ++l) {
      if (l == 0) bigchol_free(m->big_all);
      bigchol_free(m->L[l].big_k); bigchol_free(m->L[l].big_ngA); bigchol_free(m->L[l].big_ngT);
    }
    delete m;
  }
  return DSDGP_OK;
}

#include "model_schedule.hpp"

extern "C" int dsdgp_model_train_step(dsdgp_model* m, const double* X, const double* Y, int64_t n, int32_t S, const double* const* zs,
                                      const int64_t* zstride, uint64_t seed, double data_scale, double kl_weight, double lr, double beta1,
                                      double beta2, double eps, int64_t t, double* out) {
  DS_CHECK_ARG(X && Y);
  return train_step_impl(m, X, Y, n, S, zs, zstride, seed, data_scale, kl_weight, lr, beta1, beta2, eps, t, out, nullptr);
}
extern "C" int dsdgp_model_train_step_minibatch(dsdgp_model* m, const double* X_all, const double* Y_all, const int64_t* idx,
                                                int64_t idx_offset, int64_t n, int32_t S, uint64_t seed, double data_scale, double kl_weight,
                                                double lr, double beta1, double beta2, double eps, int64_t t, double* out) {
  DS_CHECK_ARG(X_all && Y_all && idx && idx_offset >= 0);
  const GatherSrc gs{X_all, Y_all, idx + idx_offset};
  return train_step_impl(m, nullptr, nullptr, n, S, nullptr, nullptr, seed, data_scale, kl_weight, lr, beta1, beta2, eps, t, out, &gs);
}

extern "C" int dsdgp_model_set_bucket_callback(dsdgp_model* m, dsdgp_bucket_fn fn, void* user) {
  DS_CHECK_ARG(m != nullptr);
  if (fn) {
    for (int l = 0; l < m->desc.L; ++l) {
      const dsdgp_layer_desc& d = m->L[l].d;
      const int64_t lo = theta_segment_lo(m, l), hi = theta_segment_lo(m, l + 1);
      const int64_t offs[] = {d.off_q_mu, d.off_q_sqrt, d.off_kvar, d.off_kls, d.has_white ? d.off_wvar : lo,
                              d.off_mean_A >= 0 ? d.off_mean_A : lo, d.off_mean_b >= 0 ? d.off_mean_b : lo};
      bool ok = lo < hi;
      for (int64_t o : offs) ok = ok && o >= lo && o < hi;
      if (!ok) {
        dsdgp_set_error("dsdgp_model_set_bucket_callback: the parameters of layer %d do not form one contiguous segment of theta "
                        "ordered [layer 0 | layer 1 | ... | likelihood]", l);
        return DSDGP_ERR_UNSUPPORTED;
      }
    }
  }
  m->bucket_fn = fn;
  m->bucket_user = user;
  return DSDGP_OK;
}

extern "C" int dsdgp_model_set_grad_first_layer(dsdgp_model* m, int32_t first) {
  DS_CHECK_ARG(m && first >= 0 && first < m->desc.L);
  m->grad_first = first;
  return DSDGP_OK;
}
extern "C" int dsdgp_model_set_grad_q_only(dsdgp_model* m, int32_t on) {
  DS_CHECK_ARG(m != nullptr);
  m->grad_q_only = on != 0;
  return DSDGP_OK;
}

extern "C" int dsdgp_model_track_theta(dsdgp_model* m, int enable) {
  DS_CHECK_ARG(m != nullptr);
  m->ps.set_track_theta(enable != 0);
  return DSDGP_OK;
}
extern "C" int dsdgp_model_theta_changed(dsdgp_model* m) {
  DS_CHECK_ARG(m != nullptr);
  m->ps.theta_moved();
  return DSDGP_OK;
}

extern "C" int dsdgp_model_layer_kl(dsdgp_model* m, int32_t l, double* out) {
  DS_CHECK_ARG(m && out && l >= 0 && l < m->desc.L);
  DS_TRY(ensure_prepared(m));
  DS_LAUNCH(k_kl_final, dim3(1), dim3(256), 0, m->ctx->stream, m->layers_dev, m->desc.L);
  DS_HIP(hipGetLastError());
  DS_HIP(hipMemcpyAsync(out, m->L[l].dev.klv, sizeof(double), hipMemcpyDeviceToDevice, m->ctx->stream));
  return DSDGP_OK;
}

extern "C" int dsdgp_model_layer_matrix(dsdgp_model* m, int32_t l, int32_t which, double* out, int64_t ld_out) {
  DS_CHECK_ARG(m && out && l >= 0 && l < m->desc.L);
  DS_CHECK_ARG(which >= DSDGP_MAT_LU && which <= DSDGP_MAT_KUINV);
  const LayerDev& v = m->L[l].dev;
  DS_CHECK_ARG(ld_out >= v.Mp);
  if (which == DSDGP_MAT_LU && !m->desc.white) {
    dsdgp_set_error("dsdgp_model_layer_matrix: layer %d keeps no Lu (it is written back for white = True models only)", l);
    return DSDGP_ERR_UNSUPPORTED;
  }
  DS_TRY(ensure_prepared(m));
  DS_TRY(join_prep(m));
  const double* src = which == DSDGP_MAT_LU ? v.Kp : which == DSDGP_MAT_LUINV ? v.Linv : which == DSDGP_MAT_LUINVT ? v.LinvT : v.Kinv;
  const size_t row = (size_t)v.Mp * sizeof(double);
  DS_HIP(hipStreamSynchronize(m->side));
  DS_HIP(hipMemcpy2DAsync(out, (size_t)ld_out * sizeof(double), src, row, row, (size_t)v.Mp, hipMemcpyDefault, m->ctx->stream));
  DS_HIP(hipStreamSynchronize(m->ctx->stream));
  return DSDGP_OK;
}

extern "C" int dsdgp_lik_elbo_readout(dsdgp_ctx* ctx, int32_t kind, double p0, double p1, const double* mean, const double* var,
                                      const double* Y, int64_t n, int32_t S, int32_t DY, double w, const double* sample_w,
                                      double* part, double* dmean, double* dvar, double* MBt, double* VBt, int64_t ldt) {
  DS_CHECK_ARG(ctx && mean && var && Y && part && n > 0 && S > 0 && DY > 0);
  DS_CHECK_ARG(lik_params_ok(kind, p0, p1));
  DS_CHECK_ARG(!dmean == !dvar && !MBt == !VBt && !(dmean && MBt));
  const int64_t R = (int64_t)S * n, total = R * DY;
  DS_CHECK_ARG(!MBt || ldt >= R);
  const int64_t cover = MBt ? ldt * DY : total;
  DS_CHECK_ARG((cover + 255) / 256 <= 0x7fffffff);
  const int nblocks = ceil_div(cover, 256);
  void* scr;
  DS_TRY(ctx_scratch(ctx, 2 * sizeof(double), &scr));
  const double lc[2] = {p0, 0.0};
  DS_TRY(ctx_upload(ctx, scr, lc, sizeof(lc)));
  lik_dispatch(kind, [&](auto fam) {
    DS_LAUNCH(k_lik_elbo<decltype(fam)::value>, dim3(nblocks), dim3(256), 0, ctx->stream, (int)kind, (const double*)scr, p1, mean, var, Y, n,
              (int)S, (int)DY, w, sample_w, part, dmean, dvar, MBt, VBt, ldt);
  });
  DS_HIP(hipGetLastError());
  return DSDGP_OK;
}

extern "C" int dsdgp_multiclass_readout(dsdgp_ctx* ctx, const double* mean, const double* var, const double* Y, int64_t n, int32_t S,
                                        int32_t K, double w, const double* sample_w, double* ve, double* dmean, double* dvar) {
  DS_CHECK_ARG(ctx && mean && var && Y && ve && dmean && dvar && n > 0 && S > 0);
  const int64_t R = (int64_t)S * n;
  DS_TRY(multiclass_launch(ctx, mean, var, Y, n, R, K, 0, w, ve, dmean, dvar, -1));
  if (sample_w) {
    const int64_t cnt = R * K;
    DS_LAUNCH(k_scale_by_sample, dim3((int)std::min<int64_t>(2048, ceil_div(cnt, 256))), dim3(256), 0, ctx->stream, sample_w, n, (int)S,
              (int)K, R, ve, dmean, dvar);
  }
  DS_HIP(hipGetLastError());
  return DSDGP_OK;
}

extern "C" int dsdgp_model_layer_conditional(dsdgp_model* m, int32_t l, const double* X, int64_t n, double* mean,
                                             double* var) {
  DS_CHECK_ARG(m && X && mean && var && l >= 0 && l < m->desc.L && n > 0);
  m->ps.workspace_overwritten();
  DS_TRY(ensure_prepared(m));
  LayerState& St = m->L[l];
  const LayerDev& v = St.dev;
  LayerFwdArgs a{};
  a.X = X; a.Rin = n; a.rep = 1;
  a.D_in = v.D_in; a.D_out = v.D_out; a.M = v.M;
  a.Zp = v.Zp; a.Zs = v.Zs; a.hyp = v.hyp; a.LinvT = v.LinvT; a.Linv = v.Linv; a.Tp = v.Tp; a.TpT = v.TpT; a.qmu = v.qmu;
  a.mean_kind = St.d.mean_kind; a.mean_A = St.meanA; a.mean_b = St.meanb;
  a.jitter = m->desc.jitter;
  a.n_inner = n;
  a.mean = mean; a.var = var;
  a.ldA = round_up(n, 16);
  if (St.gemm) {
    const int64_t chunk = St.ld_max - St.ld_max % 16;
    DS_CHECK_ARG(chunk > 0);
    for (int64_t r0 = 0; r0 < n; r0 += chunk) {
      LayerFwdArgs c = a;
      c.Rin = std::min<int64_t>(chunk, n - r0);
      c.n_inner = c.Rin;
      c.X = X + r0 * v.D_in;
      c.mean = mean + r0 * v.D_out;
      c.var = var + r0 * v.D_out;
      c.ldA = round_up(c.Rin, 16);
      DS_TRY(layer_fwd_gemm_launch(m->ctx, c, v.Mp, v.kern_kind, m->desc.white ? 1 : 0, m->gws));
    }
    return DSDGP_OK;
  }
  return layer_fwd_sm_launch(m->ctx, a, v.Mp, v.kern_kind, m->desc.white);
}

extern "C" int dsdgp_reparameterize(dsdgp_ctx* ctx, const double* mean, const double* var, const double* z, double jitter,
                                    int64_t count, double* out) {
  DS_CHECK_ARG(ctx && mean && var && z && out && count > 0);
  const int nb = (int)std::min<int64_t>(4096, ceil_div(count, 256));
  DS_LAUNCH(k_reparam, dim3(nb), dim3(256), 0, ctx->stream, mean, var, z, jitter, count, out);
  DS_HIP(hipGetLastError());
  return DSDGP_OK;
}

extern "C" int dsdgp_randn(dsdgp_ctx* ctx, uint64_t seed, uint64_t stream, int64_t count, double* out) {
  DS_CHECK_ARG(ctx && out && count > 0);
  return randn_async(ctx, seed, stream, count, out);
}

#include "model_extras.hpp"
```

### doubly-stochastic-dgp_amd/csrc/model_layout.hpp

```cpp
#pragma once
static void layout(dsdgp_model* m, char* base, size_t* total) {
  Bump b{base, 0};
  const dsdgp_model_desc& D = m->desc;
  m->layers_dev = b.take<LayerDev>(D.L);
  m->mask = b.take<double>(D.n_theta);
  m->lik_const = b.take<double>(8);
  m->scal4 = b.take<double>(8);
  const int64_t Rlast = (int64_t)m->s_max * m->n_max;
  m->lik_blocks_max = std::max(ceil_div((Rlast + 16) * D.layers[D.L - 1].D_out, 256) + 1,
                               4 * ceil_div(Rlast, 16) + 4);
  m->lik_part = b.take<double>((size_t)m->lik_blocks_max * 2);
  m->Xmb = b.take<double>((size_t)m->n_max * D.layers[0].D_in);
  m->Ymb = b.take<double>((size_t)m->n_max * D.layers[D.L - 1].D_out);
  m->lik_dmean = b.take<double>((size_t)Rlast * D.layers[D.L - 1].D_out);
  m->lik_dvar = b.take<double>((size_t)Rlast * D.layers[D.L - 1].D_out);
  m->potrf_items = b.take<PotrfItem>(D.L);
  m->gp_fwd = b.take<GemmProblem>(4 * D.L);
  m->gp_bwd1 = b.take<GemmProblem>(4 * D.L);
  m->gp_pt = b.take<GemmProblem>(2 * D.L);
  m->gp_bwd2 = b.take<GemmProblem>(D.L);
  m->gp_wz = b.take<GemmProblem>(D.L);
  m->gp_w1 = b.take<GemmProblem>(2 * D.L); m->gp_w2 = b.take<GemmProblem>(D.L); m->gp_w3 = b.take<GemmProblem>(D.L);
  m->rjobs_cap = 0;
  for (int l = 0; l < D.L; ++l) m->rjobs_cap += plan_red_slots(D.layers[l].D_out);
  m->rjobs = b.take<RedJob>(m->rjobs_cap);
  bool uniform = D.L > 1 && pad_M(D.layers[0].M) >= big_mp(true);
  for (int l = 1; l < D.L; ++l) uniform = uniform && D.layers[l].M == D.layers[0].M;
  uniform = uniform && pad_M(D.layers[0].M) % 64 == 0;
  m->uniform_big = uniform;
  double *Kp_all = nullptr, *Linv_all = nullptr, *LinvT_all = nullptr, *scal_all = nullptr;
  if (uniform) {
    const size_t MM0 = (size_t)pad_M(D.layers[0].M) * pad_M(D.layers[0].M);
    Kp_all = b.take<double>(D.L * MM0); Linv_all = b.take<double>(D.L * MM0); LinvT_all = b.take<double>(D.L * MM0);
    scal_all = b.take<double>(D.L * 8);
  }
  for (int l = 0; l < D.L; ++l) {
    LayerState& S = m->L[l];
    const dsdgp_layer_desc& d = D.layers[l];
    S.d = d;
    LayerDev& v = S.dev;
    v.M = d.M; v.Mp = pad_M(d.M); v.D_in = d.D_in; v.D_out = d.D_out;
    v.DP4 = (int)round_up(d.D_out, 4); v.DP16 = (int)round_up(d.D_out, 16); v.DinP16 = (int)round_up(d.D_in + 1, 16);
    v.kern_kind = d.kern_kind; v.ard = d.ard; v.has_white = d.has_white; v.white = D.white; v.hyp_parts = -NPART;
    v.off_Z = d.off_Z; v.off_q_mu = d.off_q_mu; v.off_q_sqrt = d.off_q_sqrt;
    v.off_kvar = d.off_kvar; v.off_kls = d.off_kls; v.off_wvar = d.off_wvar; v.kvar_identity = d.kvar_identity ? 1 : 0;
    const size_t Mp = v.Mp, MM = Mp * Mp;
    v.Zp = b.take<double>(Mp * d.D_in);
    v.Zs = b.take<double>(Mp * d.D_in);
    v.hyp = b.take<double>(HYP_ILS + 2 * d.D_in + 8);
    v.Tp = b.take<double>(d.D_out * MM);
    v.TpT = b.take<double>(d.D_out * MM);
    v.qmu = b.take<double>(Mp * d.D_out);
    v.qmu4 = b.take<double>(Mp * v.DP4);
    if (uniform) {
      v.Kp = Kp_all + l * MM; v.Linv = Linv_all + l * MM; v.LinvT = LinvT_all + l * MM; v.scal = scal_all + l * 8;
    } else {
      v.Kp = b.take<double>(MM); v.Linv = b.take<double>(MM); v.LinvT = b.take<double>(MM); v.scal = b.take<double>(16);
    }
    v.Kinv = b.take<double>(MM);
    v.V = b.take<double>(d.D_out * MM); v.nL = b.take<double>(Mp * v.DP4); v.Sd = b.take<double>(d.D_out * MM);
    v.klv = b.take<double>(8);
    v.U = b.take<double>(d.D_out * MM); v.n4 = b.take<double>(Mp * v.DP4); v.PT = b.take<double>(d.D_out * MM);
    v.UU = b.take<double>(d.D_out * MM); v.Kbar = b.take<double>(MM); v.wm = b.take<double>(MM); v.wk = b.take<double>(MM);
    v.bigred = b.take<double>((1 + d.D_out) * MM);
    v.thinq = b.take<double>(Mp * v.DP16);
    v.thinz = b.take<double>(Mp * v.DinP16);
    v.hyp_red = b.take<double>(d.D_in + 2 + 8);
    v.klpart = b.take<double>(512);
    v.ngTI = b.take<double>(d.D_out * MM); v.ngTinv = b.take<double>(d.D_out * MM); v.ngTbar = b.take<double>(d.D_out * MM);
    v.ngH = b.take<double>(d.D_out * MM); v.ngY = b.take<double>(d.D_out * MM); v.ngX = b.take<double>(d.D_out * MM);
    v.ngSinv = b.take<double>(d.D_out * MM); v.ngA = b.take<double>(d.D_out * MM); v.ngLAinv = b.take<double>(d.D_out * MM);
    v.ngLAinvT = b.take<double>(d.D_out * MM); v.ngV = b.take<double>(d.D_out * Mp);
    v.ngTheta1 = b.take<double>(d.D_out * Mp); v.ngScal = b.take<double>(4 * d.D_out + 8);
    v.wLbar = b.take<double>(MM); v.wH = b.take<double>(MM); v.wY = b.take<double>(MM); v.wX = b.take<double>(MM);
    v.hyp2part = b.take<double>(1024 * (d.D_in + 2));
    {
      const int alg_env = m->force.alg_g;
      const int64_t R_l = (l == 0) ? m->n_max : (int64_t)m->s_max * m->n_max;
      v.alg_g = (!D.white && (alg_env == 1 || (alg_env < 0 && (int64_t)4 * d.D_out * v.Mp <= R_l))) ? 1 : 0;
      v.need_tpt = (v.Mp > 256 || save_c_enabled(m->force.save_c, v.Mp) || (m->force.gemm_mp > 0 && v.Mp >= m->force.gemm_mp)) ? 1 : 0;
      if (l == D.L - 1 && D.L >= 2 && !D.white && m->force.last_fuse != 0 && layer_last_built(v.Mp, d.D_in, d.D_out)) v.need_tpt = 1;
      v.KS = v.alg_g ? b.take<double>(d.D_out * MM) : nullptr;
      v.GS = v.alg_g ? b.take<double>(d.D_out * MM) : nullptr;
    }
    v.off_mean_A = (d.mean_kind == DSDGP_MEAN_LINEAR) ? d.off_mean_A : -1;
    v.off_mean_b = (d.mean_kind == DSDGP_MEAN_LINEAR) ? d.off_mean_b : -1;
    S.mean_grad = (v.off_mean_A >= 0 && d.trainable_mean_A) || (v.off_mean_b >= 0 && d.trainable_mean_b);
    v.meanAB = S.mean_grad ? b.take<double>((size_t)64 * ceil_div(v.DinP16, 64) * v.DP16) : nullptr;
    v.R2 = b.take<double>(MM);
    v.Zp1 = b.take<double>(Mp * v.DinP16); v.WZ = b.take<double>(Mp * v.DinP16);
    S.R_max = (int64_t)m->s_max * m->n_max;
    const int64_t Rin_max = (l == 0) ? m->n_max : S.R_max;
    S.ld_max = round_up(Rin_max, 16);
    const size_t Mw = pad_Mw(v.Mp);
    S.A = b.take<double>(Mw * S.ld_max); S.E = b.take<double>(Mw * S.ld_max); S.GW = b.take<double>(Mw * S.ld_max);
    S.C = save_c_enabled(m->force.save_c, (int)Mp) ? b.take<double>((size_t)d.D_out * Mp * S.ld_max) : nullptr;
    S.VB = b.take<double>(v.DP16 * S.ld_max); S.MB = b.take<double>(v.DP16 * S.ld_max);
    S.XT1 = b.take<double>((size_t)round_up(v.DinP16, 64) * S.ld_max);
    S.F = b.take<double>(S.R_max * d.D_out); S.mean = b.take<double>(S.R_max * d.D_out);
    S.var = b.take<double>(S.R_max * d.D_out); S.zbuf = b.take<double>(S.R_max * d.D_out + 2);
    S.prop = (l + 1 < D.L) ? d.input_prop_dim : 0;
    S.dF = b.take<double>(S.R_max * (d.D_out + S.prop));
    S.Xcat = S.prop ? b.take<double>(S.R_max * (d.D_out + S.prop)) : nullptr;
    S.cap = plan_caps(v.alg_g, d.D_out, v.Mp, v.DP16, v.DinP16, S.mean_grad, S.ld_max);
    S.part_big = b.take<double>(S.cap.part_big); S.part_thin = b.take<double>(S.cap.part_thin);
    S.part_mean = S.mean_grad ? b.take<double>(S.cap.part_mean) : nullptr;
    S.gemm = m->force.gemm_mp > 0 && v.Mp >= m->force.gemm_mp;
    S.hyp_part = b.take<double>((size_t)(std::max<int64_t>(std::max<int64_t>(sm_hyp_parts(S.ld_max, v.Mp, d.D_in), layer_gemm_hyp_parts(S.ld_max, v.Mp)),
                                                           8 * 160) + 16) * (d.D_in + 2));
    S.bpart = b.take<double>((size_t)1024 * (Mp * 16 + 16));
    S.bcnt = b.take<int>(512);
    S.lq = b.take<GemmProblem>(12);
    S.wj = b.take<WgradJob>(S.cap.jobs); S.wtick = b.take<int32_t>(S.cap.ticks);
    S.ng_gp = b.take<GemmProblem>(4);
    S.ng_items = b.take<PotrfItem>(d.D_out);
  }
  {
    int64_t cap = 0;
    for (int l = 0; l < D.L; ++l) {
      const int64_t t64 = ceil_div(pad_Mw(m->L[l].dev.Mp), 64);
      cap += (int64_t)(20 * D.layers[l].D_out + 24) * t64 * t64;
    }
    m->gemm_order_cap = 2 * 2 * cap;
    m->gemm_order = b.take<int32_t>((size_t)m->gemm_order_cap);
  }
  {
    int64_t ML = 0, cq = 0, mut = 0, qt = 0, zz = 0, ot = 0, sv = 0;
    for (int l = 0; l < D.L; ++l) {
      const LayerState& S = m->L[l];
      if (!S.gemm) continue;
      const LayerDev& v = S.dev;
      const int64_t ld = S.ld_max, nzz16 = round_up(2 * v.D_in + 1, 16);
      ML = std::max<int64_t>(ML, (int64_t)v.Mp * ld);
      cq = std::max<int64_t>(cq, (int64_t)(1 + v.D_out) * ceil_div(v.Mp, 128) * ld);
      mut = std::max<int64_t>(mut, (int64_t)v.DP16 * ld);
      qt = std::max<int64_t>(qt, (int64_t)v.DP16 * v.Mp);
      zz = std::max<int64_t>(zz, nzz16 * v.Mp);
      ot = std::max<int64_t>(ot, nzz16 * ld);
      sv = std::max<int64_t>(sv, (int64_t)ceil_div(ld, 32) * ceil_div(v.Mp, 32));
    }
    if (ML > 0) {
      m->gws.T1 = b.take<double>(ML); m->gws.T2 = b.take<double>(ML); m->gws.Pb = b.take<double>((GL_MAX_GROUPS + 1) * ML);
      m->gws.pb_doubles = (GL_MAX_GROUPS + 1) * ML;
      m->gws.colsq = b.take<double>(cq); m->gws.MUT = b.take<double>(mut); m->gws.qmuT = b.take<double>(qt);
      m->gws.ZZ = b.take<double>(zz); m->gws.OUTt = b.take<double>(ot); m->gws.svar = b.take<double>(sv + 16);
    }
  }
  *total = (size_t)round_up((int64_t)b.off, 256);
}
```

### doubly-stochastic-dgp_amd/csrc/model_schedule.hpp

```cpp
#pragma once
static bool overlap_on(const dsdgp_model* m, int64_t n, int S) {
  const char* no = getenv("DSDGP_NO_OVERLAP");
  if (!m->overlap || (no && atoi(no))) return false;
  int mp_max = 0;
  for (int l = 0; l < m->desc.L; ++l) mp_max = std::max(mp_max, (int)m->L[l].dev.Mp);
  return n * S * (int64_t)mp_max >= (int64_t)m->force.overlap_min;
}

static const GemmProblem* lq_unks(const LayerState& S) { return S.lq + S.lq_nf; }
static const GemmProblem* lq_uut(const LayerState& S) { return lq_unks(S) + S.lq_n1; }
static const GemmProblem* lq_pt(const LayerState& S) { return lq_uut(S) + S.lq_n2; }

static int join_prep(dsdgp_model* m) {
  if (m->side_pending) {
    DS_HIP(hipStreamWaitEvent(m->ctx->stream, m->ev_prep_side, 0));
    m->side_pending = false;
  }
  return DSDGP_OK;
}

static_assert(DSDGP_MAX_LAYERS <= 32, "PrepIn::blocked is a 32-bit mask");
static PrepIn prep_in(const dsdgp_model* m, bool with_grad, bool side) {
  PrepIn in{with_grad, side, m->desc.L, m->desc.white != 0, m->grad_first, m->head_ok, m->uniform_big, 0u, 0, big_mp(false), m->force.ext_ev != 0};
  for (int l = 0; l < in.L; ++l) {
    in.mp_max = std::max(in.mp_max, (int)m->L[l].dev.Mp);
    if (m->L[l].big) in.blocked |= 1u << l;
  }
  return in;
}
static int launch_grad_side(dsdgp_ctx* ctx, const LayerState& Sq, hipStream_t st) {
  DS_TRY(gemm_launch(ctx, lq_unks(Sq), Sq.lq_n1, Sq.lq_t1, st));
  return gemm_launch(ctx, lq_uut(Sq), Sq.lq_n2, Sq.lq_t2, st);
}
static int prepare_async(dsdgp_model* m, bool with_grad = false, bool side = false, const HeadRand* hr = nullptr,
                         const HeadGather* hg = nullptr) {
  dsdgp_ctx* ctx = m->ctx;
  const int L = m->desc.L;
  m->ps.workspace_overwritten();
  DS_TRY(join_prep(m));
  const PrepIn in = prep_in(m, with_grad, side);
  const PrepPlan p = prep_plan(m->ps, in);
  const int mp_max = in.mp_max;
  if (p.head) {
    ProfScope ps(ctx, "potrf");
    const size_t lds = head_lds_bytes(mp_max);
    static size_t lds_set = 0;
    if (lds > lds_set) {
      DS_HIP(hipFuncSetAttribute((const void*)k_head, hipFuncAttributeMaxDynamicSharedMemorySize, (int)lds));
      lds_set = lds;
    }
    HeadRand none{};
    const HeadRand& r = hr ? *hr : none;
    HeadGather gnone{};
    const HeadGather& gq = hg ? *hg : gnone;
    const int nprep = std::max(32, m->prep_blocks / 2);
    g_dsdgp_launches.fetch_add(1, std::memory_order_relaxed);
    hipExtLaunchKernelGGL(k_head, dim3(1 + nprep + r.nblk + gq.nblk, L), dim3(HEAD_THREADS), (uint32_t)lds, ctx->stream, nullptr,
                          p.fork_on_head ? m->ev_fork : nullptr, 0, (const double*)m->theta, (const LayerDev*)m->layers_dev, m->lik_const,
                          (int64_t)m->desc.off_lik_var, lik_has_param(m->desc.lik_kind) ? 1 : 0, m->desc.jitter, nprep,
                          p.keep_kuu ? 1 : 0, m->desc.white ? 1 : 0, getenv("DSDGP_POTRF_TIMING") ? 1 : 0, r, gq);
    DS_HIP(hipGetLastError());
  } else if (p.prep_kuu) {
    DS_LAUNCH(k_prep_kuu, dim3(m->prep_blocks + (p.kuu_blocks ? m->kuu_blocks : 0), L), dim3(256), 0, ctx->stream, m->theta, m->layers_dev,
                       m->lik_const, m->desc.off_lik_var, lik_has_param(m->desc.lik_kind) ? 1 : 0, m->desc.jitter,
                       m->prep_blocks, p.keep_kuu ? 1 : 0);
    DS_HIP(hipGetLastError());
  }
  switch (p.factor) {
    case FACTOR_NONE: case FACTOR_IN_HEAD: break;
    case FACTOR_BATCHED_BLOCKED: DS_TRY(bigchol_run(ctx, m->big_all)); break;
    case FACTOR_PER_LAYER:
      for (int l = 0; l < L; ++l) {
        if (p.blocked >> l & 1) DS_TRY(bigchol_run(ctx, m->L[l].big_k));
        else DS_TRY(potrf_launch(ctx, m->potrf_items + l, 1, m->L[l].dev.Mp));
      }
      break;
    case FACTOR_ONE_WG_BATCH: DS_TRY(potrf_launch(ctx, m->potrf_items, L, mp_max)); break;
  }
  if (p.early) {
    m->ps.prepare_done(p);
    return DSDGP_OK;
  }
  hipStream_t st = ctx->stream;
  if (p.fork) {
    if (!p.fork_on_head) DS_HIP(hipEventRecord(m->ev_fork, ctx->stream));
    DS_HIP(hipStreamWaitEvent(m->side, m->ev_fork, 0));
    st = m->side;
  }
  const int klb = mp_max >= 512 ? 512 : NPART;
  if (p.fwd == REDO_LAYER) {
    LayerState& Sq = m->L[p.fwd_layer];
    DS_TRY(gemm_launch(ctx, Sq.lq, Sq.lq_nf, Sq.lq_tf, st));
    DS_LAUNCH(k_kl_part, dim3(klb, 1), dim3(256), 0, st, m->layers_dev + p.fwd_layer);
  } else if (p.fwd == REDO_ALL) {
    DS_TRY(gemm_launch(ctx, m->gp_fwd, m->n_fwd, m->t_fwd, st));
    DS_LAUNCH(k_kl_part, dim3(klb, L), dim3(256), 0, st, m->layers_dev);
  }
  DS_HIP(hipGetLastError());
  m->kinv_pending = false;
  if (p.rec_kinv) {
    DS_HIP(hipEventRecord(m->ev_kinv, m->side));
    m->kinv_pending = true;
  }
  if (p.grad == REDO_LAYER) DS_TRY(launch_grad_side(ctx, m->L[p.grad_layer], st));
  else if (p.grad == REDO_FROM) {
    for (int l = p.grad_layer; l < L; ++l) DS_TRY(launch_grad_side(ctx, m->L[l], st));
  } else if (p.grad == REDO_ALL) {
    DS_TRY(gemm_launch(ctx, m->gp_bwd1, m->n_bwd1, m->t_bwd1, st));
    DS_TRY(gemm_launch(ctx, m->gp_bwd2, m->n_bwd2, m->t_bwd2, st));
  }
  if (p.rec_prep_side) {
    DS_HIP(hipEventRecord(m->ev_prep_side, m->side));
    m->side_pending = true;
  }
  m->ps.prepare_done(p);
  return DSDGP_OK;
}
static int ensure_prepared(dsdgp_model* m) { return m->ps.prepared ? DSDGP_OK : prepare_async(m); }

static int read_info(dsdgp_model* m, int* info) {
  if (!info) return DSDGP_OK;
  *info = 0;
  if (getenv("DSDGP_POTRF_TIMING")) {
    double sc[12];
    hipMemcpyAsync(sc, m->L[0].dev.scal, sizeof(sc), hipMemcpyDeviceToHost, m->ctx->stream);
    hipStreamSynchronize(m->ctx->stream);
    if (m->head_ok)
      fprintf(stderr, "[head cycles] start + Z staging %.0f | Ku %.0f | first panel %.0f | block columns 1.. (+ inverse rows) %.0f | logdet + last two "
              "inverse rows %.0f || wave 0 in the loop: tile %.0f, barrier %.0f, panel %.0f, barrier %.0f\n", sc[2], sc[3], sc[4], sc[5], sc[6], sc[7],
              sc[8], sc[9], sc[10]);
    else
      fprintf(stderr, "[potrf cycles] factor %.0f inverse %.0f panel %.0f trailing %.0f logdet+writeback %.0f copyin+trtri %.0f\n", sc[2],
              sc[3], sc[4], sc[5], sc[6], sc[7]);
  }
  for (int l = 0; l < m->desc.L; ++l) {
    double sc[2];
    DS_HIP(hipMemcpyAsync(sc, m->L[l].dev.scal, sizeof(sc), hipMemcpyDeviceToHost, m->ctx->stream));
    DS_HIP(hipStreamSynchronize(m->ctx->stream));
    if (sc[1] != 0.0 && *info == 0) *info = (int)sc[1];
  }
  if (*info) {
    dsdgp_set_error("Cholesky decomposition was not successful (layer Kuu pivot %d)", *info);
    return DSDGP_ERR_NOT_SPD;
  }
  return DSDGP_OK;
}

extern "C" int dsdgp_model_prepare(dsdgp_model* m, int* info) {
  DS_CHECK_ARG(m != nullptr);
  DS_TRY(prepare_async(m));
  return read_info(m, info);
}

static int randn_async(dsdgp_ctx* ctx, uint64_t seed, uint64_t stream, int64_t count, double* out, hipStream_t st = nullptr) {
  const int nb = (int)std::min<int64_t>(2048, ceil_div((count + 1) / 2, 256));
  DS_LAUNCH(k_randn, dim3(nb > 0 ? nb : 1), dim3(256), 0, st ? st : ctx->stream, seed, stream, count, out);
  DS_HIP(hipGetLastError());
  return DSDGP_OK;
}

struct FwdCall {
  const double* X;
  int64_t n;
  int S;
  const double* const* zs;
  const int64_t* zstride;
  uint64_t seed;
  double *const *Fs, *const *Fmeans, *const *Fvars;
  const double* lik_Y;
  double lik_w;
};
struct GatherSrc {
  const double *Xs, *Ys;
  const int64_t* idx;
};
static FwdIn fwd_in(const dsdgp_model* m, const FwdCall& c, bool prepare, bool save, bool need_last_F, bool lik_target) {
  static const bool timing = getenv("DSDGP_FWD_TIMING") || getenv("DSDGP_BWD_TIMING");
  const dsdgp_model::Force& f = m->force;
  FwdIn in{};
  in.n = c.n; in.S = c.S;
  in.prepare = prepare; in.save = in.with_grad = save; in.need_last_F = need_last_F; in.lik_target = lik_target; in.sample_w = m->sample_w != nullptr;
  in.L = m->desc.L; in.white = m->desc.white != 0;
  in.lik_elementwise = lik_family(m->desc.lik_kind) != LIKF_NONE; in.lik_gaussian = m->desc.lik_kind == DSDGP_LIK_GAUSSIAN;
  in.grad_first = m->grad_first; in.grad_q_only = m->grad_q_only; in.head_ok = m->head_ok; in.overlap = overlap_on(m, c.n, c.S); in.timing = timing;
  for (int l = 0; l < in.L; ++l) {
    const LayerState& St = m->L[l];
    const LayerDev& v = St.dev;
    if (c.zs && c.zs[l]) in.caller_z |= 1u << l;
    in.layer[l] = FwdIn::Layer{v.Mp, v.M, v.D_in, v.D_out, v.kern_kind, St.d.mean_kind, St.prop, St.gemm, v.alg_g != 0, v.need_tpt != 0, St.C != nullptr,
                               St.bpart != nullptr};
  }
  in.force = {f.white_fwd, f.cs_min_blocks, f.cs_min_dout, f.cs_max_dout, f.last_fuse, f.last_min_blocks, f.bwd_split, f.lik_fuse};
  return in;
}

static int forward_layers(dsdgp_model* m, const FwdCall& c, const FwdIn& in, const FwdPlan& p) {
  dsdgp_ctx* ctx = m->ctx;
  const int L = m->desc.L;
  m->ps.workspace_overwritten();
  if (p.join_prep_first) DS_TRY(join_prep(m));
  const double* Xin = c.X;
  FwdUsed used[DSDGP_MAX_LAYERS];
  LayerFwdArgs a{};
  for (int l = 0; l < L; ++l) {
    LayerState& St = m->L[l];
    const LayerDev& v = St.dev;
    const FwdPlan::Layer& y = p.layer[l];
    a = LayerFwdArgs{};
    a.X = Xin; a.Rin = y.Rin; a.rep = y.rep;
    a.D_in = v.D_in; a.D_out = v.D_out; a.M = v.M;
    a.Zp = v.Zp; a.Zs = v.Zs; a.hyp = v.hyp; a.LinvT = v.LinvT; a.Linv = v.Linv; a.Tp = v.Tp; a.TpT = v.TpT; a.qmu = v.qmu;
    if (y.whitened) { a.Tp = v.V; a.qmu = v.nL; a.qmu_ld = v.DP4; }
    a.mean_kind = St.d.mean_kind; a.mean_A = St.meanA; a.mean_b = St.meanb;
    a.jitter = m->desc.jitter;
    a.n_inner = c.n;
    if (y.draw == DRAW_CALLER) {
      a.z = c.zs[l];
      a.zs_s = c.zstride[3 * l]; a.zs_n = c.zstride[3 * l + 1]; a.zs_d = c.zstride[3 * l + 2];
    } else if (y.draw != DRAW_NONE) {
      if (y.draw == DRAW_HERE) DS_TRY(randn_async(ctx, c.seed, (uint64_t)l, (int64_t)c.S * c.n * v.D_out, St.zbuf));
      a.z = St.zbuf;
      a.zs_s = c.n * v.D_out; a.zs_n = v.D_out; a.zs_d = 1;
    }
    a.F = y.want_F ? ((c.Fs && c.Fs[l]) ? c.Fs[l] : St.F) : nullptr;
    a.mean = (c.Fmeans && c.Fmeans[l]) ? c.Fmeans[l] : St.mean;
    a.var = (c.Fvars && c.Fvars[l]) ? c.Fvars[l] : St.var;
    a.ldA = y.ld;
    a.Asave = y.save_A ? St.A : nullptr; a.Csave = y.save_C ? St.C : nullptr; a.XT1 = y.save_XT1 ? St.XT1 : nullptr;
    a.d_split = y.d_split;
    if (y.lik_epilogue) {
      a.lik_Y = c.lik_Y; a.lik_const = m->lik_const; a.lik_w = c.lik_w; a.lik_part = m->lik_part;
      a.lik_MB = St.MB; a.lik_VB = St.VB; a.lik_ld = y.ld;
    }
    switch (y.launch) {
      case LAUNCH_WITH_REVERSE: break;
      case LAUNCH_GEMM: DS_TRY(layer_fwd_gemm_launch(ctx, a, v.Mp, v.kern_kind, m->desc.white ? 1 : 0, m->gws)); break;
      case LAUNCH_CHAIN: DS_TRY(layer_fwd_sm_launch(ctx, a, v.Mp, v.kern_kind, m->desc.white || y.whitened)); break;
    }
    used[l] = FwdUsed{a.X, a.z, a.zs_s, a.zs_n, a.zs_d};
    if (y.concat) {
      const int64_t R = (int64_t)c.S * c.n, cnt = R * (v.D_out + St.prop);
      DS_LAUNCH(k_concat_prop, dim3((int)std::min<int64_t>(4096, ceil_div(cnt, 256))), dim3(256), 0, ctx->stream, Xin, y.Rin,
                         v.D_in, St.prop, a.F, v.D_out, R, St.Xcat);
      DS_HIP(hipGetLastError());
      Xin = St.Xcat;
    } else {
      Xin = a.F;
    }
  }
  m->fwd.forward_done(in, p, used, p.layer[L - 1].launch == LAUNCH_WITH_REVERSE ? &a : nullptr);
  return DSDGP_OK;
}

static HeadRand head_rand(const dsdgp_model* m, const FwdCall& c, const FwdPlan& p) {
  HeadRand hr{};
  hr.seed = c.seed; hr.nblk = p.head_nblk;
  for (int l = 0; l < m->desc.L; ++l)
    if (p.layer[l].draw == DRAW_READY) {
      hr.out[l] = m->L[l].zbuf;
      hr.count[l] = (int64_t)c.S * c.n * m->L[l].dev.D_out;
    }
  return hr;
}
static int inner_draws(dsdgp_model* m, const FwdCall& c, const FwdPlan& p) {
  DS_HIP(hipEventRecord(m->ev_fork, m->ctx->stream));
  DS_HIP(hipStreamWaitEvent(m->side, m->ev_fork, 0));
  for (int l = 0; l < m->desc.L; ++l)
    if (p.layer[l].draw == DRAW_READY) DS_TRY(randn_async(m->ctx, c.seed, (uint64_t)l, (int64_t)c.S * c.n * m->L[l].dev.D_out, m->L[l].zbuf, m->side));
  if (p.draws_ahead) DS_HIP(hipEventRecord(m->ev_z, m->side));
  return DSDGP_OK;
}
static int forward_pass(dsdgp_model* m, const FwdCall& c, const FwdIn& in, const GatherSrc* gs = nullptr, FwdPlan* plan = nullptr) {
  DS_CHECK_ARG(c.n > 0 && c.n <= m->n_max && c.S > 0 && c.S <= m->s_max);
  const FwdPlan p = fwd_plan(in);
  if (in.prepare) {
    const bool ahead_in_head = p.draws == DRAWS_HEAD && p.draws_ahead;
    const HeadRand hr = ahead_in_head ? head_rand(m, c, p) : HeadRand{};
    if (p.draws == DRAWS_SIDE) DS_TRY(inner_draws(m, c, p));
    HeadGather hg{};
    if (gs) {
      const int dx = m->desc.layers[0].D_in, dy = (m->desc.lik_kind == DSDGP_LIK_MULTICLASS) ? 1 : m->desc.layers[in.L - 1].D_out;
      if (m->head_ok) {
        hg = HeadGather{gs->Xs, gs->Ys, gs->idx, m->Xmb, m->Ymb, c.n, dx, dy, (int)std::min<int64_t>(16, ceil_div(c.n * (dx + dy), 2 * HEAD_THREADS))};
      } else {
        DS_TRY(dsdgp_gather_rows2(m->ctx, gs->Xs, dx, m->Xmb, gs->Ys, dy, m->Ymb, gs->idx, c.n, 0));
      }
    }
    DS_TRY(prepare_async(m, in.with_grad, in.overlap, ahead_in_head ? &hr : nullptr, (gs && m->head_ok) ? &hg : nullptr));
    if (p.draws == DRAWS_SIDE && p.draws_ahead) DS_HIP(hipStreamWaitEvent(m->ctx->stream, m->ev_z, 0));
  } else {
    DS_TRY(ensure_prepared(m));
  }
  if (plan) *plan = p;
  return forward_layers(m, c, in, p);
}

extern "C" int dsdgp_model_propagate(dsdgp_model* m, const double* X, int64_t n, int32_t S, const double* const* zs,
                                     const int64_t* zstride, uint64_t seed, double* const* Fs, double* const* Fmeans,
                                     double* const* Fvars) {
  DS_CHECK_ARG(m && X);
  DS_CHECK_ARG(!zs || zstride);
  const FwdCall c{X, n, S, zs, zstride, seed, Fs, Fmeans, Fvars, nullptr, 0.0};
  return forward_pass(m, c, fwd_in(m, c, false, false, true, false));
}

static int mixture_forward(const char* who, dsdgp_model* m, const double* X, int64_t n, int S, const double* const* zs,
                           const int64_t* zstride, uint64_t seed, bool needs_gaussian, const LayerState** last) {
  DS_CHECK_ARG(!zs || zstride);
  if (m->sample_w) {
    dsdgp_set_error("%s: quadrature sample weights are set (dsdgp_model_set_sample_weights); the mixture is an unweighted mean", who);
    return DSDGP_ERR_UNSUPPORTED;
  }
  if (needs_gaussian && m->desc.lik_kind != DSDGP_LIK_GAUSSIAN) {
    dsdgp_set_error("%s: the predictive y of likelihood kind %d is not a Gaussian mixture; only the latent f (level 0) is covered", who,
                    m->desc.lik_kind);
    return DSDGP_ERR_UNSUPPORTED;
  }
  const FwdCall c{X, n, S, zs, zstride, seed, nullptr, nullptr, nullptr, nullptr, 0.0};
  DS_TRY(forward_pass(m, c, fwd_in(m, c, false, false, true, false)));
  *last = &m->L[m->desc.L - 1];
  return DSDGP_OK;
}

extern "C" int dsdgp_model_evaluate(dsdgp_model* m, const double* X, const double* Y, int64_t n, int32_t S, const double* const* zs,
                                    const int64_t* zstride, uint64_t seed, double* rows_out, double* acc, int accumulate) {
  DS_CHECK_ARG(m && X && Y && acc);
  const LayerState* last;
  DS_TRY(mixture_forward("dsdgp_model_evaluate", m, X, n, S, zs, zstride, seed, false, &last));
  const int kind = m->desc.lik_kind;
  DS_CHECK_ARG(kind != DSDGP_LIK_MULTICLASS || last->dev.D_out == m->desc.num_classes);
  return eval_mixture_launch(m->ctx, kind, 1.0, m->desc.lik_aux, lik_has_param(kind) ? m->lik_const : nullptr, last->mean, last->var, Y, n,
                             S, last->dev.D_out, rows_out, acc, accumulate);
}

extern "C" int dsdgp_model_quantiles(dsdgp_model* m, const double* X, int64_t n, int32_t S, const double* const* zs,
                                     const int64_t* zstride, uint64_t seed, int32_t level, const double* probs, int32_t P,
                                     double* q_out) {
  DS_CHECK_ARG(m && X && probs && q_out);
  DS_CHECK_ARG(!zs || zstride);
  DS_CHECK_ARG(level == 0 || level == 1);
  const LayerState* last;
  DS_TRY(mixture_forward("dsdgp_model_quantiles", m, X, n, S, zs, zstride, seed, level == 1, &last));
  return mixture_quantiles_launch(m->ctx, last->mean, last->var, 0.0, level == 1 ? m->lik_const : nullptr, n, S, last->dev.D_out, probs, P,
                                  q_out);
}
extern "C" int dsdgp_model_calibration(dsdgp_model* m, const double* X, const double* Y, int64_t n, int32_t S, const double* const* zs,
                                       const int64_t* zstride, uint64_t seed, const double* probs, int32_t P, double* rows_out,
                                       double* acc, int accumulate) {
  DS_CHECK_ARG(m && X && Y && probs && acc);
  const LayerState* last;
  DS_TRY(mixture_forward("dsdgp_model_calibration", m, X, n, S, zs, zstride, seed, true, &last));
  return mixture_calibration_launch(m->ctx, last->mean, last->var, 0.0, m->lik_const, Y, n, S, last->dev.D_out, probs, P, rows_out, acc,
                                    accumulate);
}

extern "C" int dsdgp_model_classification(dsdgp_model* m, const double* X, const double* Y, int64_t n, int32_t S, const double* const* zs,
                                          const int64_t* zstride, uint64_t seed, int32_t bins, double* probs_out, double* rows_out,
                                          double* acc, int accumulate) {
  DS_CHECK_ARG(m && X && Y && acc);
  const int kind = m->desc.lik_kind;
  if (kind != DSDGP_LIK_MULTICLASS && kind != DSDGP_LIK_BERNOULLI) {
    dsdgp_set_error("dsdgp_model_classification: likelihood kind %d has no classes; MultiClass and Bernoulli are covered", kind);
    return DSDGP_ERR_UNSUPPORTED;
  }
  const LayerState* last;
  DS_TRY(mixture_forward("dsdgp_model_classification", m, X, n, S, zs, zstride, seed, false, &last));
  DS_CHECK_ARG(kind != DSDGP_LIK_MULTICLASS || last->dev.D_out == m->desc.num_classes);
  return mixture_classification_launch(m->ctx, kind, last->mean, last->var, Y, n, S, last->dev.D_out, bins, probs_out, rows_out, acc,
                                       accumulate);
}

static int ensure_plan(dsdgp_model* m, int64_t n, int S) {
  if (m->plan_n == n && m->plan_S == S) return DSDGP_OK;
  dsdgp_ctx* ctx = m->ctx;
  const int L = m->desc.L, overlap = overlap_on(m, n, S);
  std::vector<RedJob> red;
  PlanOut P;
  for (int l = 0; l < L; ++l) {
    LayerState& St = m->L[l];
    const LayerDev& v = St.dev;
    const int64_t ld = round_up((l == 0) ? n : (int64_t)S * n, 16);
    const int hyp_parts = St.gemm ? layer_gemm_hyp_parts(ld, v.Mp) : (int)sm_hyp_parts(ld, v.Mp, v.D_in);
    plan_layer(PlanIn{&v, &St, ld, hyp_parts, m->force.wg_red, m->force.wg_group, overlap}, P);
    if (P.ticks > St.cap.ticks) {
      dsdgp_set_error("internal: weight-gradient ticket list overflow (%d > %d)", P.ticks, St.cap.ticks);
      return DSDGP_ERR_WORKSPACE;
    }
    if ((int)P.jobs.size() > St.cap.jobs) {
      dsdgp_set_error("internal: weight-gradient job list overflow (%d jobs > %d slots of wj)", (int)P.jobs.size(), St.cap.jobs);
      return DSDGP_ERR_WORKSPACE;
    }
    St.njobs = (int)P.jobs.size(); St.njobsA = P.njobsA; St.totA = P.totA; St.tot_big = P.tot; St.ns_big = P.ns;
    St.red_off = (int)red.size();
    red.insert(red.end(), P.red.begin(), P.red.end());
    DS_HIP(hipMemsetAsync(St.wtick, 0, (size_t)St.cap.ticks * sizeof(int32_t), ctx->stream));
    DS_HIP(hipMemsetAsync(St.part_big, 0, St.cap.part_big * sizeof(double), ctx->stream));
    DS_HIP(hipMemcpyAsync(St.wj, P.jobs.data(), P.jobs.size() * sizeof(WgradJob), hipMemcpyHostToDevice, ctx->stream));
    DS_HIP(hipStreamSynchronize(ctx->stream));
  }
  const RedPlan rp = plan_reductions(red);
  for (int l = 0; l < L; ++l) m->L[l].red_blk0 = red[m->L[l].red_off].blk_start;
  if ((int)red.size() > m->rjobs_cap) {
    dsdgp_set_error("internal: reduction job list overflow");
    return DSDGP_ERR_WORKSPACE;
  }
  DS_HIP(hipMemcpyAsync(m->rjobs, red.data(), red.size() * sizeof(RedJob), hipMemcpyHostToDevice, ctx->stream));
  DS_HIP(hipStreamSynchronize(ctx->stream));
  m->n_red = (int)red.size(); m->red_blocks = rp.blocks;
  m->red_lds = rp.any64 ? 64 * 65 * sizeof(double) : 0;
  m->plan_n = n; m->plan_S = S;
  return DSDGP_OK;
}

static int64_t theta_segment_lo(const dsdgp_model* m, int l) {
  return l < m->desc.L ? m->L[l].d.off_Z : (lik_has_param(m->desc.lik_kind) ? m->desc.off_lik_var : m->desc.n_theta);
}
static int64_t lik_var_offset(const dsdgp_model* m) { return lik_has_param(m->desc.lik_kind) ? m->desc.off_lik_var : (int64_t)-1; }
static FinArgs fin_args(const dsdgp_model* m) {
  return FinArgs{m->lik_part, m->fin.nblocks, m->fin.w, m->fin.kl_weight, m->lik_const, lik_var_offset(m), m->fin.out, m->desc.L, 1};
}

static int launch_finalize(dsdgp_model* m, hipStream_t st) {
  DS_LAUNCH(k_finalize, dim3(1), dim3(256), 0, st, m->layers_dev, m->desc.L, m->lik_part, m->fin.nblocks, m->fin.w,
                     m->fin.kl_weight, m->lik_const, m->grad, lik_var_offset(m), m->fin.with_grad, m->fin.out);
  DS_HIP(hipGetLastError());
  m->fin.done = true;
  return DSDGP_OK;
}

enum AdjFrom : uint8_t { ADJ_PRODUCER, ADJ_PROLOGUE, ADJ_PREP };
enum ProductsAt : uint8_t { PROD_MAIN, PROD_SIDE, PROD_DEFERRED };
struct BwdSchedule {
  int gfirst; bool overlap, bucketed, pipelined, kinv_only, q_only, defer_upper, red_ahead;
  struct Layer { AdjFrom adj; bool chain; int d_split; ProductsAt products; } layer[DSDGP_MAX_LAYERS];
};
static BwdSchedule bwd_schedule(const dsdgp_model* m) {
  const int L = m->desc.L;
  BwdSchedule s{}; s.overlap = overlap_on(m, m->fwd.n, m->fwd.S);
  const int g = s.gfirst = m->desc.white ? 0 : m->grad_first;
  s.bucketed = m->bucket_fn != nullptr && m->tail_ok && g == 0 && !m->fuse_adam.on;
  s.pipelined = s.bucketed || (s.overlap && m->force.pipe_tail != 0 && !m->desc.white);
  s.kinv_only = s.overlap && !s.pipelined && !m->desc.white && m->kinv_pending && m->side_pending;
  s.q_only = m->grad_q_only && !m->desc.white;
  s.defer_upper = s.overlap && !s.pipelined && (m->force.wg_defer == 2 || (m->force.wg_defer < 0 && L - g >= 4));
  s.red_ahead = s.overlap && !s.pipelined && g == 0 && L > 1 && m->force.red_ahead != 0;
  for (int l = g; l < L; ++l) {
    const LayerState& St = m->L[l];
    const LayerDev& v = St.dev;
    BwdSchedule::Layer& y = s.layer[l];
    const bool last = (l == L - 1), produced = last ? m->fwd.adjoints_from_lik : l >= 1;
    const int64_t nblk = m->fwd.layer[l].ld / 16;
    y.chain = !(s.q_only && l == g);
    const bool prologue = !produced && !last && y.chain && m->force.adj_fuse != 0 && !m->fwd.layer[l].c_saved && !St.gemm && sm_adj_fusable(v.Mp, nblk, v.D_in, v.D_out);
    y.adj = produced ? ADJ_PRODUCER : (prologue ? ADJ_PROLOGUE : ADJ_PREP);
    y.d_split = bwd_d_split(m->force.bwd_split, v.Mp, St.bpart != nullptr, nblk, v.D_out);
    const bool on_main = s.overlap && l == g && L - g > 1;
    y.products = (!s.overlap || on_main) ? PROD_MAIN : ((s.defer_upper && l >= g + 2) ? PROD_DEFERRED : PROD_SIDE);
  }
  return s;
}

static LayerBwdArgs fill_bwd_args(const dsdgp_model* m, int l, const BwdSchedule& sc) {
  const LayerState& St = m->L[l];
  const LayerDev& v = St.dev;
  const auto& R = m->fwd.layer[l];
  const int64_t n = m->fwd.n;
  LayerBwdArgs b{};
  b.X = R.X; b.Rin = R.Rin; b.D_in = v.D_in; b.D_out = v.D_out; b.M = v.M; b.DP4 = v.DP4;
  b.Zp = v.Zp; b.Zs = v.Zs; b.hyp = v.hyp; b.Kinv = v.Kinv; b.Linv = v.Linv; b.LinvT = v.LinvT; b.Sd = v.Sd; b.qmu4 = v.qmu4;
  b.Asave = St.A; b.Csave = R.c_saved ? St.C : nullptr; b.Tp = v.Tp; b.TpT = v.TpT; b.ldA = R.ld; b.VB = St.VB; b.MB = St.MB;
  b.E = v.alg_g ? nullptr : St.E; b.GW = St.GW;
  b.dX = (l > sc.gfirst) ? m->L[l - 1].dF : nullptr;
  if (l >= 2 && l > sc.gfirst) {
    const LayerState& Pv = m->L[l - 1];
    const auto& Rp = m->fwd.layer[l - 1];
    b.dX = nullptr;
    b.MBp = Pv.MB; b.VBp = Pv.VB;
    b.zp = Rp.z; b.zp_s = Rp.zs_s; b.zp_n = Rp.zs_n; b.zp_d = Rp.zs_d; b.n_inner = n;
    b.varp = Pv.var; b.Dp = Pv.dev.D_out; b.prop = Pv.prop; b.jitter = m->desc.jitter;
  }
  b.mean_kind = St.d.mean_kind; b.mean_A = St.meanA; b.hyp_part = St.hyp_part;
  if (sc.layer[l].adj == ADJ_PROLOGUE) {
    b.up_dF = St.dF; b.up_rep = R.rep; b.up_ld = v.D_out + St.prop; b.up_off = St.prop;
    b.up_z = R.z; b.up_zs = R.zs_s; b.up_zn = R.zs_n; b.up_zd = R.zs_d; b.up_n_inner = n;
    b.up_var = St.var; b.up_jitter = m->desc.jitter; b.MBw = St.MB; b.VBw = St.VB;
  }
  b.d_split = sc.layer[l].d_split; b.part = St.bpart; b.part_cnt = St.bcnt;
  return b;
}

static int launch_reduce(dsdgp_model* m, int first, int end, hipStream_t st) {
  const LayerState& S0 = m->L[first];
  const int njobs = (end < m->desc.L ? m->L[end].red_off : m->n_red) - S0.red_off;
  const int nblk = (end < m->desc.L ? m->L[end].red_blk0 : m->red_blocks) - S0.red_blk0;
  DS_LAUNCH(k_reduce_grouped, dim3(nblk), dim3(256), m->red_lds, st, m->rjobs + S0.red_off, njobs, S0.red_blk0);
  DS_HIP(hipGetLastError());
  return DSDGP_OK;
}
static int launch_wgrad(dsdgp_model* m, const BwdSchedule& sc, int l, hipStream_t st) {
  const LayerState& Sx = m->L[l];
  const bool all = sc.layer[l].chain;
  const int64_t ld = m->fwd.layer[l].ld;
  return wgrad_launch(m->ctx, Sx.wj, all ? Sx.njobs : Sx.njobsA, all ? Sx.tot_big : Sx.totA, Sx.ns_big, ld, ld, st);
}
static int layer_tail(dsdgp_model* m, const BwdSchedule& sc, int l, hipStream_t st, double kl_weight) {
  const LayerState& St = m->L[l];
  DS_TRY(launch_reduce(m, l, l + 1, st));
  DS_TRY(gemm_launch(m->ctx, lq_pt(St), St.lq_np, St.lq_tp, st));
  if (sc.bucketed) {
    DS_LAUNCH(k_asm_rows, dim3(St.dev.M, 1), dim3(256), (size_t)m->mp_max_all * sizeof(double), st, (const LayerDev*)(m->layers_dev + l), m->grad,
              kl_weight, m->mp_max_all, m->force.asm_pre);
    DS_LAUNCH(k_tail, dim3(1), dim3(256), 0, st, m->layers_dev, l, 1, m->grad, FinArgs{}, AdamArgs{});
    DS_HIP(hipGetLastError());
    const int64_t lo = theta_segment_lo(m, l);
    m->bucket_fn(m->bucket_user, l, m->grad + lo, theta_segment_lo(m, l + 1) - lo, (void*)st);
  }
  return DSDGP_OK;
}

static int end_last_bucket(dsdgp_model* m, hipStream_t st) {
  const int L = m->desc.L;
  DS_LAUNCH(k_tail, dim3(1), dim3(256), 0, st, m->layers_dev, 0, 0, m->grad, fin_args(m), AdamArgs{});
  DS_HIP(hipGetLastError());
  m->fin.done = true;
  const int64_t lo = theta_segment_lo(m, L);
  const bool tail_scalars = m->fin.out == m->grad + m->desc.n_theta;
  m->bucket_fn(m->bucket_user, L, m->grad + lo, (m->desc.n_theta - lo) + (tail_scalars ? 4 : 0), (void*)st);
  if (!tail_scalars) m->bucket_fn(m->bucket_user, L + 1, m->fin.out, 4, (void*)st);
  return DSDGP_OK;
}
static int end_rows_tail(dsdgp_model* m, hipStream_t st, int gfirst, int La, double kl_weight) {
  DS_LAUNCH(k_asm_rows, dim3(m->m_max_all, La), dim3(256), (size_t)m->mp_max_all * sizeof(double), st, (const LayerDev*)(m->layers_dev + gfirst),
            m->grad, kl_weight, m->mp_max_all, m->force.asm_pre);
  AdamArgs A{m->theta, m->adam_m, m->adam_v, m->mask, m->desc.n_theta, m->fuse_adam.lr_t, m->fuse_adam.b1, m->fuse_adam.b2,
             m->fuse_adam.eps, (m->fuse_adam.on && gfirst == 0) ? 1 : 0};
  const int nadam = A.on ? (int)std::min<int64_t>(2048, ceil_div(m->desc.n_theta, 512)) : 0;
  DS_LAUNCH(k_tail, dim3(La + 1 + nadam), dim3(256), 0, st, m->layers_dev, gfirst, La, m->grad, fin_args(m), A);
  DS_HIP(hipGetLastError());
  m->fin.done = true;
  return DSDGP_OK;
}
static int end_unfused(dsdgp_model* m, hipStream_t st, const LayerDev* lay, int La, double kl_weight) {
  DS_LAUNCH(k_asm_kbar, dim3(m->kuu_blocks, La), dim3(256), 0, st, lay, kl_weight);
  if (m->n_wz) DS_TRY(gemm_launch(m->ctx, m->gp_wz, m->n_wz, m->t_wz));
  if (m->need_hyp_part) DS_LAUNCH(k_asm_hyp_part, dim3(NPART, La), dim3(256), 0, st, lay);
  DS_LAUNCH(k_asm_params, dim3(m->asm_blocks + 1, La), dim3(256), 0, st, lay, m->grad, kl_weight);
  DS_HIP(hipGetLastError());
  return DSDGP_OK;
}

static int backward_layers(dsdgp_model* m, double kl_weight) {
  dsdgp_ctx* ctx = m->ctx;
  const int L = m->desc.L;
  const int64_t n = m->fwd.n;
  DS_TRY(ensure_plan(m, n, m->fwd.S));
  const BwdSchedule sc = bwd_schedule(m);
  const int gfirst = sc.gfirst;
  if (sc.kinv_only) DS_HIP(hipStreamWaitEvent(ctx->stream, m->ev_kinv, 0));
  else DS_TRY(join_prep(m));
  for (int l = L - 1; l >= gfirst; --l) {
    LayerState& St = m->L[l];
    const LayerDev& v = St.dev;
    const bool last = (l == L - 1);
    const auto& R = m->fwd.layer[l];
    const int64_t ld = R.ld;
    if (sc.layer[l].adj == ADJ_PREP)
      DS_LAUNCH(k_adj_prep, dim3(ceil_div(ld, 256), std::max(v.DP16, v.DinP16)), dim3(256), 0, ctx->stream, last ? nullptr : St.dF,
                         last ? m->lik_dmean : nullptr, last ? m->lik_dvar : nullptr, R.z, R.zs_s, R.zs_n,
                         R.zs_d, n, St.var, R.X, R.Rin, R.rep, v.D_in, v.D_out, v.DP16, v.DinP16, m->desc.jitter, ld,
                         St.MB, St.VB, St.XT1, v.D_out + St.prop, St.prop);
    DS_HIP(hipGetLastError());
    const LayerBwdArgs b = fill_bwd_args(m, l, sc);
    if (last && m->fwd.last_pending) {
      DS_TRY(layer_last_launch(ctx, m->fwd.last_fwd, b, v.Mp, v.kern_kind, m->fwd.hyp_rows));
      m->fwd.last_launched();
    } else if (!sc.layer[l].chain) {  }
    else if (St.gemm) DS_TRY(layer_bwd_gemm_launch(ctx, b, v.Mp, v.kern_kind, m->desc.white ? 1 : 0, m->gws));
    else DS_TRY(layer_bwd_sm_launch(ctx, b, v.Mp, v.kern_kind, m->desc.white));
    if (sc.layer[l].products == PROD_MAIN) {
      DS_TRY(launch_wgrad(m, sc, l, ctx->stream));
      for (int lu = l + 1; lu < L; ++lu)
        if (sc.layer[lu].products == PROD_DEFERRED) DS_TRY(launch_wgrad(m, sc, lu, ctx->stream));
      if (sc.pipelined) DS_TRY(layer_tail(m, sc, l, ctx->stream, kl_weight));
    } else if (sc.layer[l].products == PROD_SIDE) {
      DS_HIP(hipEventRecord(m->ev_bwd[l], ctx->stream));
      DS_HIP(hipStreamWaitEvent(m->side, m->ev_bwd[l], 0));
      DS_TRY(launch_wgrad(m, sc, l, m->side));
      if (sc.pipelined) DS_TRY(layer_tail(m, sc, l, m->side, kl_weight));
    }
  }
  if (sc.red_ahead) DS_TRY(launch_reduce(m, 0, 1, ctx->stream));
  if (sc.overlap) {
    if (!m->fin.done && !m->tail_ok) DS_TRY(launch_finalize(m, m->side));
    DS_HIP(hipEventRecord(m->ev_side, m->side));
    DS_HIP(hipStreamWaitEvent(ctx->stream, m->ev_side, 0));
    m->side_pending = false;
  }
  if (!sc.pipelined) {
    DS_TRY(launch_reduce(m, sc.red_ahead ? 1 : gfirst, L, ctx->stream));
    if (m->desc.white) {
      DS_LAUNCH(k_white_lbar, dim3(32, L), dim3(256), 0, ctx->stream, m->layers_dev);
      DS_TRY(gemm_launch(ctx, m->gp_w1, 2 * L, m->t_w1));
      DS_LAUNCH(k_white_phi, dim3(32, L), dim3(256), 0, ctx->stream, m->layers_dev);
      DS_TRY(gemm_launch(ctx, m->gp_w2, L, m->t_w2));
      DS_TRY(gemm_launch(ctx, m->gp_w3, L, m->t_w3));
    } else if (gfirst > 0) {
      for (int l = gfirst; l < L; ++l) DS_TRY(gemm_launch(ctx, lq_pt(m->L[l]), m->L[l].lq_np, m->L[l].lq_tp));
    } else {
      DS_TRY(gemm_launch(ctx, m->gp_pt, m->n_pt, m->t_pt));
    }
  }
  if (sc.bucketed) return end_last_bucket(m, ctx->stream);
  if (m->tail_ok) return end_rows_tail(m, ctx->stream, gfirst, L - gfirst, kl_weight);
  return end_unfused(m, ctx->stream, m->layers_dev + gfirst, L - gfirst, kl_weight);
}

static int finish_value(dsdgp_model* m) {
  if (!m->fin.done) {
    DS_TRY(join_prep(m));
    DS_TRY(launch_finalize(m, m->ctx->stream));
  }
  return DSDGP_OK;
}

static int elbo_impl(dsdgp_model* m, const double* X, const double* Y, int64_t n, int32_t S, const double* const* zs,
                     const int64_t* zstride, uint64_t seed, double data_scale, double kl_weight, int with_grad, double* out,
                     const GatherSrc* gs) {
  DS_CHECK_ARG(m && out && ((X && Y) || gs));
  DS_CHECK_ARG(!zs || zstride);
  DS_CHECK_ARG(!m->sample_w || S == m->sample_w_S);
  if (with_grad) {
    DS_CHECK_ARG(m->grad != nullptr);
  }
  dsdgp_ctx* ctx = m->ctx;
  if (gs) {
    X = m->Xmb;
    Y = m->Ymb;
  }
  const double w = data_scale / (double)S;
  const FwdCall c{X, n, S, zs, zstride, seed, nullptr, nullptr, nullptr, Y, w};
  FwdPlan p;
  DS_TRY(forward_pass(m, c, fwd_in(m, c, true, with_grad != 0, false, true), gs, &p));
  LayerState& last = m->L[m->desc.L - 1];
  const int DY = last.dev.D_out;
  const bool own_adj = with_grad && !p.adjoints_from_lik;
  if (p.lik == LIK_ELEMENTWISE) {
    const int64_t ldt = round_up((int64_t)S * n, 16);
    double* mbt = p.adjoints_from_lik ? last.MB : nullptr;
    double* vbt = p.adjoints_from_lik ? last.VB : nullptr;
    lik_dispatch(m->desc.lik_kind, [&](auto fam) {
      DS_LAUNCH(k_lik_elbo<decltype(fam)::value>, dim3(p.lik_nblocks), dim3(256), 0, ctx->stream, (int)m->desc.lik_kind, (const double*)m->lik_const,
                m->desc.lik_aux, last.mean, last.var, Y, n, S, DY, w, m->sample_w, m->lik_part, own_adj ? m->lik_dmean : nullptr,
                own_adj ? m->lik_dvar : nullptr, mbt, vbt, ldt);
    });
  } else if (p.lik == LIK_MULTICLASS) {
    DS_CHECK_ARG(DY == m->desc.num_classes);
    const int64_t R = (int64_t)S * n;
    DS_TRY(multiclass_launch(ctx, last.mean, last.var, Y, n, R, DY, 0, w, last.F, with_grad ? m->lik_dmean : nullptr,
                             with_grad ? m->lik_dvar : nullptr, -1));
    if (m->sample_w) {
      const int64_t cnt = R * DY;
      DS_LAUNCH(k_scale_by_sample, dim3((int)std::min<int64_t>(2048, ceil_div(cnt, 256))), dim3(256), 0, ctx->stream,
                         m->sample_w, n, S, DY, R, last.F, with_grad ? m->lik_dmean : nullptr, with_grad ? m->lik_dvar : nullptr);
    }
    DS_LAUNCH(k_partial_sum, dim3(p.lik_nblocks), dim3(256), 0, ctx->stream, last.F, R, m->lik_part);
  }
  DS_HIP(hipGetLastError());
  m->fin.nblocks = p.lik_nblocks; m->fin.w = w; m->fin.kl_weight = kl_weight; m->fin.with_grad = with_grad; m->fin.out = out;
  m->fin.done = false;
  if (with_grad) {
    DS_TRY(backward_layers(m, kl_weight));
    m->ps.grad_evaluated(pass_is_pruned(m->desc.white, m->grad_first, m->grad_q_only));
  }
  return finish_value(m);
}

extern "C" int dsdgp_model_elbo(dsdgp_model* m, const double* X, const double* Y, int64_t n, int32_t S,
                                const double* const* zs, const int64_t* zstride, uint64_t seed, double data_scale,
                                double kl_weight, int with_grad, double* out) {
  DS_CHECK_ARG(X && Y);
  return elbo_impl(m, X, Y, n, S, zs, zstride, seed, data_scale, kl_weight, with_grad, out, nullptr);
}

static int vjp_refusals(const char* who, const dsdgp_model* m) {
  if (m->bucket_fn) {
    dsdgp_set_error("%s: a bucket callback is set (dsdgp_model_set_bucket_callback); the vector-Jacobian product is single-process", who);
    return DSDGP_ERR_UNSUPPORTED;
  }
  if (m->sample_w) {
    dsdgp_set_error("%s: quadrature sample weights are set (dsdgp_model_set_sample_weights); the caller's adjoints carry their own weights", who);
    return DSDGP_ERR_UNSUPPORTED;
  }
  if (pass_is_pruned(m->desc.white, m->grad_first, m->grad_q_only)) {
    dsdgp_set_error("%s: the reverse pass is restricted to layers >= %d%s (dsdgp_model_set_grad_first_layer / _q_only)", who, m->grad_first,
                    m->grad_q_only ? ", (q_mu, q_sqrt) only" : "");
    return DSDGP_ERR_BAD_ARG;
  }
  return DSDGP_OK;
}
extern "C" int dsdgp_model_forward_saved(dsdgp_model* m, const double* X, int64_t n, int32_t S, const double* const* zs,
                                         const int64_t* zstride, uint64_t seed, double* mean_out, double* var_out) {
  DS_CHECK_ARG(m && X && m->grad != nullptr);
  DS_CHECK_ARG(!zs || zstride);
  DS_CHECK_ARG(n > 0 && n <= m->n_max && S > 0 && S <= m->s_max);
  DS_TRY(vjp_refusals("dsdgp_model_forward_saved", m));
  dsdgp_ctx* ctx = m->ctx;
  const FwdCall c{X, n, S, zs, zstride, seed, nullptr, nullptr, nullptr, nullptr, 0.0};
  DS_TRY(forward_pass(m, c, fwd_in(m, c, true, true, false, false)));
  const LayerState& last = m->L[m->desc.L - 1];
  const size_t bytes = (size_t)S * n * last.dev.D_out * sizeof(double);
  if (mean_out) DS_HIP(hipMemcpyAsync(mean_out, last.mean, bytes, hipMemcpyDeviceToDevice, ctx->stream));
  if (var_out) DS_HIP(hipMemcpyAsync(var_out, last.var, bytes, hipMemcpyDeviceToDevice, ctx->stream));
  m->ps.saved_recorded(n, S);
  return DSDGP_OK;
}
extern "C" int dsdgp_model_backward_adjoints(dsdgp_model* m, const double* dmean, const double* dvar, double kl_weight, double* out) {
  DS_CHECK_ARG(m && dmean && dvar && out && m->grad != nullptr);
  if (!m->ps.saved) {
    dsdgp_set_error("dsdgp_model_backward_adjoints: the model's last evaluation is not a dsdgp_model_forward_saved (another evaluation, a "
                    "change of theta or an optimiser step since then drops the saved forward pass)");
    return DSDGP_ERR_BAD_ARG;
  }
  DS_TRY(vjp_refusals("dsdgp_model_backward_adjoints", m));
  dsdgp_ctx* ctx = m->ctx;
  const int64_t n = m->ps.saved_n;
  const int S = m->ps.saved_S;
  m->ps.saved_consumed();
  const int64_t count = (int64_t)S * n * m->L[m->desc.L - 1].dev.D_out;
  DS_LAUNCH(k_seed_adjoints, dim3((int)std::min<int64_t>(2048, ceil_div(count, 256))), dim3(256), 0, ctx->stream, dmean, dvar, count,
            m->lik_dmean, m->lik_dvar);
  DS_HIP(hipGetLastError());
  m->fwd.adjoints_from_caller();
  m->fin.nblocks = 0; m->fin.w = 0.0; m->fin.kl_weight = kl_weight; m->fin.with_grad = 1; m->fin.out = out;
  m->fin.done = false;
  DS_TRY(backward_layers(m, kl_weight));
  m->ps.grad_evaluated(false);
  DS_TRY(finish_value(m));
  const int64_t ol = lik_var_offset(m);
  if (ol >= 0) DS_HIP(hipMemsetAsync(m->grad + ol, 0, sizeof(double), ctx->stream));
  return DSDGP_OK;
}

extern "C" int dsdgp_model_set_sample_weights(dsdgp_model* m, const double* w, int32_t S) {
  DS_CHECK_ARG(m && (!w || (S > 0 && S <= m->s_max)));
  m->sample_w = w;
  m->sample_w_S = w ? S : 0;
  return DSDGP_OK;
}

static double adam_lr_t(double lr, double b1, double b2, int64_t t) { return lr * sqrt(1.0 - pow(b2, (double)t)) / (1.0 - pow(b1, (double)t)); }

extern "C" int dsdgp_model_adam_step(dsdgp_model* m, double lr, double beta1, double beta2, double eps, int64_t t) {
  DS_CHECK_ARG(m && m->grad && m->adam_m && m->adam_v && t >= 1);
  if (m->ps.grad_pruned) {
    dsdgp_set_error("dsdgp_model_adam_step: the last gradient was evaluated for layers >= %d only (dsdgp_model_set_grad_first_layer)", m->grad_first);
    return DSDGP_ERR_BAD_ARG;
  }
  const double lr_t = adam_lr_t(lr, beta1, beta2, t);
  const int64_t n = m->desc.n_theta;
  const int nb = (int)std::min<int64_t>(2048, ceil_div(n, 512));
  DS_LAUNCH(k_adam, dim3(nb), dim3(256), 0, m->ctx->stream, m->theta, m->grad, m->adam_m, m->adam_v, m->mask, n,
                     lr_t, beta1, beta2, eps, (const LayerDev*)m->layers_dev, m->desc.L);
  DS_HIP(hipGetLastError());
  m->ps.theta_moved();
  return DSDGP_OK;
}

static int train_step_impl(dsdgp_model* m, const double* X, const double* Y, int64_t n, int32_t S, const double* const* zs,
                           const int64_t* zstride, uint64_t seed, double data_scale, double kl_weight, double lr, double beta1,
                           double beta2, double eps, int64_t t, double* out, const GatherSrc* gs) {
  DS_CHECK_ARG(m && m->grad && m->adam_m && m->adam_v && t >= 1);
  if (pass_is_pruned(m->desc.white, m->grad_first, m->grad_q_only)) {
    dsdgp_set_error("dsdgp_model_train_step: the reverse pass is restricted to layers >= %d%s (dsdgp_model_set_grad_first_layer / _q_only)",
                    m->grad_first, m->grad_q_only ? ", (q_mu, q_sqrt) only" : "");
    return DSDGP_ERR_BAD_ARG;
  }
  if (!m->tail_ok) {
    DS_TRY(elbo_impl(m, X, Y, n, S, zs, zstride, seed, data_scale, kl_weight, 1, out, gs));
    return dsdgp_model_adam_step(m, lr, beta1, beta2, eps, t);
  }
  m->fuse_adam.on = 1;
  m->fuse_adam.lr_t = adam_lr_t(lr, beta1, beta2, t);
  m->fuse_adam.b1 = beta1; m->fuse_adam.b2 = beta2; m->fuse_adam.eps = eps;
  const int rc = elbo_impl(m, X, Y, n, S, zs, zstride, seed, data_scale, kl_weight, 1, out, gs);
  m->fuse_adam.on = 0;
  DS_TRY(rc);
  m->ps.theta_moved();
  return DSDGP_OK;
}
```

### doubly-stochastic-dgp_amd/csrc/model_types.hpp

```cpp
#pragma once
#define NPART 32
#define PREP_BLOCKS 64
#define WIDE_DIN 32

struct LayerState : PlanBufs {
  dsdgp_layer_desc d;
  LayerDev dev;
  int64_t R_max;
  int64_t ld_max;
  double* C;
  double *F, *mean, *var, *zbuf, *dF;
  const double *meanA, *meanb;
  int njobs;
  int njobsA = 0, totA = 0;
  double* Xcat;
  int prop;
  int red_off = 0, red_blk0 = 0;
  double* bpart = nullptr;
  int* bcnt = nullptr;
  bool big = false;
  BigChol big_k, big_ngA, big_ngT;
  GemmProblem* ng_gp;
  PotrfItem* ng_items;
  int ng_t1, ng_t2, ng_t3;
  GemmProblem* lq = nullptr;
  int lq_nf = 0, lq_tf = 0, lq_n1 = 0, lq_t1 = 0, lq_n2 = 0, lq_t2 = 0, lq_np = 0, lq_tp = 0;
  WgradJob* wj;
  int ns_big, tot_big;
  bool gemm = false;
};

struct dsdgp_model {
  dsdgp_ctx* ctx;
  dsdgp_model_desc desc;
  int64_t n_max;
  int s_max;
  double *theta, *grad, *adam_m, *adam_v;
  LayerState L[DSDGP_MAX_LAYERS];
  LayerDev* layers_dev;
  double* mask;
  double* lik_const;
  double* lik_part;
  int lik_blocks_max;
  double *lik_dmean, *lik_dvar;
  double* scal4;
  PotrfItem* potrf_items;
  GemmProblem *gp_fwd, *gp_bwd1, *gp_bwd2, *gp_w1, *gp_w2, *gp_w3;
  GemmProblem* gp_pt;
  int n_pt = 0, t_pt = 0;
  hipEvent_t ev_fork, ev_prep_side, ev_z;
  hipEvent_t ev_kinv;
  bool kinv_pending = false;
  int32_t* gemm_order = nullptr;
  int64_t gemm_order_cap = 0, gemm_order_used = 0;
  GemmLayerWs gws{};
  ParamState ps;
  int grad_first = 0;
  bool grad_q_only = false;
  bool side_pending = false;
  int n_fwd, n_bwd1, n_bwd2, t_fwd, t_bwd1, t_bwd2, n_w, t_w1, t_w2, t_w3;
  const double* sample_w = nullptr;
  int sample_w_S = 0;
  GemmProblem* gp_wz;
  int n_wz = 0, t_wz = 0, kuu_blocks = 32, asm_blocks = 64, prep_blocks = PREP_BLOCKS;
  bool uniform_big = false;
  BigChol big_all;
  bool need_hyp_part = false;
  bool tail_ok = false;
  struct { int on; double lr_t, b1, b2, eps; } fuse_adam = {0, 0, 0, 0, 0};
  int mp_max_all = 0, m_max_all = 0;
  dsdgp_bucket_fn bucket_fn = nullptr;
  void* bucket_user = nullptr;
  double *Xmb = nullptr, *Ymb = nullptr;
  bool head_ok = false;
  FwdRecord<LayerFwdArgs> fwd;
  struct { int nblocks; double w, kl_weight; int with_grad; double* out; bool done; } fin;
  RedJob* rjobs;
  int rjobs_cap, n_red, red_blocks;
  size_t red_lds = 0;
  int64_t plan_n;
  int plan_S;
  hipStream_t side;
  hipEvent_t ev_bwd[DSDGP_MAX_LAYERS];
  hipEvent_t ev_side;
  bool overlap;
  struct Force { int save_c = 1, cs_min_blocks = 160, cs_min_dout = 3, cs_max_dout = 1 << 20, wg_defer = -1, alg_g = -1, bwd_split = 1, pipe_tail = 0, head = 1, tail = 1, adj_fuse = 1, ext_ev = 1, lik_fuse = 1, red_ahead = 1, white_fwd = 1, gemm_mp = 512, last_fuse = 1, last_min_blocks = 1, asm_pre = 1, overlap_min = 1 << 18, wg_red = 1, wg_group = 1; } force;
};
static void parse_force(dsdgp_model* m) {
  using F = dsdgp_model::Force;
  static const struct { const char* name; int F::*field; } keys[] = {
      {"save_c", &F::save_c}, {"cs_min_blocks", &F::cs_min_blocks}, {"cs_min_dout", &F::cs_min_dout}, {"cs_max_dout", &F::cs_max_dout},
      {"wg_defer", &F::wg_defer}, {"alg_g", &F::alg_g}, {"bwd_split", &F::bwd_split}, {"red_ahead", &F::red_ahead},
      {"white_fwd", &F::white_fwd}, {"pipe_tail", &F::pipe_tail}, {"head", &F::head}, {"tail", &F::tail}, {"adj_fuse", &F::adj_fuse},
      {"ext_ev", &F::ext_ev}, {"lik_fuse", &F::lik_fuse}, {"gemm_mp", &F::gemm_mp}, {"last_fuse", &F::last_fuse},
      {"last_min_blocks", &F::last_min_blocks}, {"asm_pre", &F::asm_pre}, {"overlap_min", &F::overlap_min}, {"wg_red", &F::wg_red},
      {"wg_group", &F::wg_group}};
  const char* e = getenv("DSDGP_FORCE");
  if (!e) return;
  const std::string str(e);
  for (size_t pos = 0; pos < str.size();) {
    size_t end = str.find(',', pos);
    if (end == std::string::npos) end = str.size();
    const std::string kv = str.substr(pos, end - pos);
    const size_t eq = kv.find('=');
    if (eq != std::string::npos)
      for (const auto& k : keys)
        if (kv.compare(0, eq, k.name) == 0) m->force.*k.field = atoi(kv.c_str() + eq + 1);
    pos = end + 1;
  }
}

struct Bump {
  char* base;
  size_t off;
  template <class T>
  T* take(size_t count) {
    off = (size_t)round_up((int64_t)off, 256);
    T* p = base ? (T*)(base + off) : nullptr;
    off += count * sizeof(T);
    return p;
  }
};

static int big_mp(bool uniform) {
  static const int nonuniform = getenv("DSDGP_BIG_MP") ? atoi(getenv("DSDGP_BIG_MP")) : 192;
  return uniform ? 192 : nonuniform;
}
```

Before: 2005.

## Precompute S_d·A products on side stream for backward d-loop reuse

Adds a Tsave buffer and an MFMA kernel that computes T = S_d·A per output dimension for the first layer when the batch is small. The kernel runs on the side stream, forked by an event fired at the end of the forward chain kernel via hipExtLaunchKernelGGL. The backward kernel gets a TS variant whose d-loop reads precomputed T instead of recomputing the S_d products from LDS, and the backward waits on the tsave event. This trades extra memory, an extra launch and cross-stream synchronisation for less arithmetic on the backward critical path.

```diff
diff --git a/doubly-stochastic-dgp_amd/csrc/chain_policy.hpp b/doubly-stochastic-dgp_amd/csrc/chain_policy.hpp
--- a/doubly-stochastic-dgp_amd/csrc/chain_policy.hpp
+++ b/doubly-stochastic-dgp_amd/csrc/chain_policy.hpp
@@ -38,6 +38,24 @@
   const bool want = bwd_split >= 2 || (bwd_split == 1 && Mp > 256);
   return (want && has_part) ? chain_d_split(nblk, D_out) : 1;
 }
+#define TSAVE_MAX_BLOCKS 16
+static inline int64_t tsave_cols(int t_save, int l, int Mp, bool gemm, int64_t ld_max) {
+  if (t_save <= 0 || gemm || Mp > 256) return 0;
+  if (t_save >= 2) return ld_max;
+  return l == 0 ? std::min<int64_t>(ld_max, (int64_t)16 * TSAVE_MAX_BLOCKS) : 0;
+}
+struct TsaveIn {
+  int t_save, l, Mp;
+  int64_t nblk, t_cols;
+  bool train;
+  bool chain;
+  bool c_saved, bwd_runs, overlap;
+};
+static inline bool tsave_keep(const TsaveIn& s) {
+  if (s.t_save <= 0 || !s.train || !s.chain || s.c_saved || !s.bwd_runs || s.Mp > 256 || 16 * s.nblk > s.t_cols) return false;
+  if (s.t_save >= 2) return true;
+  return s.l == 0 && s.overlap && s.nblk <= TSAVE_MAX_BLOCKS;
+}
 static inline int layer_gemm_lik_blocks(int64_t Rin, int D_out) { return ceil_div(round_up(Rin, 16), GL_EPI_ROWS); }
 static inline int head_draw_blocks(int64_t count) { return (int)std::min<int64_t>(64, ceil_div((count + 1) / 2, 4 * HEAD_THREADS)); }
 
diff --git a/doubly-stochastic-dgp_amd/csrc/common.hpp b/doubly-stochastic-dgp_amd/csrc/common.hpp
--- a/doubly-stochastic-dgp_amd/csrc/common.hpp
+++ b/doubly-stochastic-dgp_amd/csrc/common.hpp
@@ -54,6 +54,7 @@
   hipStream_t stream = nullptr;
   bool own_stream = false;
   hipStream_t side = nullptr;
+  hipEvent_t chain_done = nullptr;
   void* scratch = nullptr;
   size_t scratch_bytes = 0;
   int prof_on = 0;
diff --git a/doubly-stochastic-dgp_amd/csrc/forward_plan.hpp b/doubly-stochastic-dgp_amd/csrc/forward_plan.hpp
--- a/doubly-stochastic-dgp_amd/csrc/forward_plan.hpp
+++ b/doubly-stochastic-dgp_amd/csrc/forward_plan.hpp
@@ -14,8 +14,9 @@
   struct Layer {
     int Mp, M, D_in, D_out, kern_kind, mean_kind, prop;
     bool gemm, alg_g, need_tpt, has_C, has_bpart;
+    int64_t t_cols;
   } layer[DSDGP_MAX_LAYERS];
-  struct { int white_fwd, cs_min_blocks, cs_min_dout, cs_max_dout, last_fuse, last_min_blocks, bwd_split, lik_fuse; } force;
+  struct { int white_fwd, cs_min_blocks, cs_min_dout, cs_max_dout, last_fuse, last_min_blocks, bwd_split, lik_fuse, t_save; } force;
 };
 
 enum DrawsAt : uint8_t { DRAWS_INLINE, DRAWS_HEAD, DRAWS_SIDE };
@@ -36,6 +37,7 @@
     bool whitened, want_F;
     DrawFrom draw;
     bool save_A, save_C, save_XT1;
+    bool save_T;
     int d_split;
     bool lik_epilogue;
     FwdLaunch launch;
@@ -97,6 +99,12 @@
   p.hyp_rows = (int)(sm_hyp_parts(y.ld, v.Mp, v.D_in) / (y.ld / 16));
   p.bwd_d_split = bwd_d_split(in.force.bwd_split, v.Mp, v.has_bpart, y.ld / 16, v.D_out);
   if (last_chain_fusable(in, p)) p.layer[L - 1].launch = LAUNCH_WITH_REVERSE;
+  for (int l = 0; l < L; ++l) {
+    const FwdIn::Layer& vl = in.layer[l];
+    FwdPlan::Layer& yl = p.layer[l];
+    yl.save_T = tsave_keep(TsaveIn{in.force.t_save, l, vl.Mp, yl.ld / 16, vl.t_cols, in.with_grad && in.lik_target, yl.launch == LAUNCH_CHAIN,
+                                   yl.save_C, yl.save_XT1, in.overlap});
+  }
   if (in.lik_target) {
     const int64_t R = (int64_t)in.S * in.n;
     p.lik = p.lik_in_chain ? LIK_IN_CHAIN : (in.lik_elementwise ? LIK_ELEMENTWISE : LIK_MULTICLASS);
@@ -110,7 +118,7 @@
 struct FwdUsed { const double *X, *z; int64_t zs_s, zs_n, zs_d; };
 template <class FwdArgs>
 struct FwdRecord {
-  struct Layer : FwdUsed { int64_t Rin, ld; int rep; bool c_saved; } layer[DSDGP_MAX_LAYERS];
+  struct Layer : FwdUsed { int64_t Rin, ld; int rep; bool c_saved, t_saved; } layer[DSDGP_MAX_LAYERS];
   int64_t n = 0;
   int S = 0;
   bool adjoints_from_lik = false;
@@ -124,11 +132,14 @@
       const FwdPlan::Layer& y = p.layer[l];
       Layer& r = layer[l];
       static_cast<FwdUsed&>(r) = used[l];
-      r.Rin = y.Rin; r.ld = y.ld; r.rep = y.rep; r.c_saved = y.save_C;
+      r.Rin = y.Rin; r.ld = y.ld; r.rep = y.rep; r.c_saved = y.save_C; r.t_saved = y.save_T;
     }
     last_pending = pending != nullptr;
     if (pending) { last_fwd = *pending; hyp_rows = p.hyp_rows; }
   }
-  void adjoints_from_caller() { adjoints_from_lik = false; }
+  void adjoints_from_caller() {
+    adjoints_from_lik = false;
+    for (Layer& r : layer) r.t_saved = false;
+  }
   void last_launched() { last_pending = false; }
 };
diff --git a/doubly-stochastic-dgp_amd/csrc/layer.hpp b/doubly-stochastic-dgp_amd/csrc/layer.hpp
--- a/doubly-stochastic-dgp_amd/csrc/layer.hpp
+++ b/doubly-stochastic-dgp_amd/csrc/layer.hpp
@@ -56,6 +56,7 @@
   const double* Csave;
   const double* Tp;
   const double* TpT;
+  const double* Tsave;
   int64_t ldA;
   const double* VB;
   const double* MB;
@@ -89,6 +90,7 @@
                  hipStream_t stream = nullptr);
 int layer_fwd_sm_launch(dsdgp_ctx* ctx, const LayerFwdArgs& a, int Mp, int kern_kind, int white);
 int layer_bwd_sm_launch(dsdgp_ctx* ctx, const LayerBwdArgs& a, int Mp, int kern_kind, int white);
+int tsave_launch(dsdgp_ctx* ctx, const double* Sd, const double* A, double* T, int Mp, int D_out, int64_t ld, hipStream_t stream);
 int layer_last_launch(dsdgp_ctx* ctx, const LayerFwdArgs& a, const LayerBwdArgs& b, int Mp, int kern_kind, int hyp_rows);
 
 struct GemmLayerWs {
diff --git a/doubly-stochastic-dgp_amd/csrc/layer_sm.hip b/doubly-stochastic-dgp_amd/csrc/layer_sm.hip
--- a/doubly-stochastic-dgp_amd/csrc/layer_sm.hip
+++ b/doubly-stochastic-dgp_amd/csrc/layer_sm.hip
@@ -15,6 +15,33 @@
   if (Mp <= 256) return layer_fwd_sm_b(ctx, a, Mp, kern_kind, white, small);
   return layer_fwd_sm_c(ctx, a, Mp, kern_kind, white, small);
 }
+__global__ __launch_bounds__(256) void k_tsave(const double* __restrict__ Sd, const double* __restrict__ A, double* __restrict__ T, int Mp,
+                                               int64_t ld) {
+  const int lane = threadIdx.x & 63, wave = threadIdx.x >> 6;
+  const int g = lane >> 4, c = lane & 15;
+  const int ib = (int)blockIdx.y * 4 + wave;
+  if (16 * ib >= Mp) return;
+  const int d = (int)blockIdx.z;
+  const int64_t r = (int64_t)blockIdx.x * 16 + c;
+  const double* __restrict__ W = Sd + ((int64_t)d * Mp + g) * Mp + 16 * ib + c;
+  const double* __restrict__ B = A + (int64_t)g * ld + r;
+  d4 y = (d4){0, 0, 0, 0};
+#pragma unroll 8
+  for (int k = 0; k < Mp; k += 4) y = mfma_f64(W[(int64_t)k * Mp], B[(int64_t)k * ld], y);
+#pragma unroll
+  for (int t = 0; t < 4; ++t) T[((int64_t)d * Mp + 16 * ib + g + 4 * t) * ld + r] = y[t];
+}
+int tsave_launch(dsdgp_ctx* ctx, const double* Sd, const double* A, double* T, int Mp, int D_out, int64_t ld, hipStream_t stream) {
+  if (!Sd || !A || !T || Mp % 16 || ld % 16 || ld <= 0 || D_out <= 0) {
+    dsdgp_set_error("tsave_launch: bad arguments (Mp %d, D_out %d, ld %lld)", Mp, D_out, (long long)ld);
+    return DSDGP_ERR_BAD_ARG;
+  }
+  DS_LAUNCH(k_tsave, dim3((unsigned)(ld / 16), (unsigned)ceil_div(Mp / 16, 4), (unsigned)D_out), dim3(256), 0, stream ? stream : ctx->stream, Sd, A, T,
+            Mp, ld);
+  DS_HIP(hipGetLastError());
+  return DSDGP_OK;
+}
+
 int layer_bwd_sm_launch(dsdgp_ctx* ctx, const LayerBwdArgs& a, int Mp, int kern_kind, int white) {
   const int small = sm_small(Mp, ceil_div(a.ldA, 16), a.D_in, true);
   if (Mp < 128) return layer_bwd_sm_a(ctx, a, Mp, kern_kind, white, small);
diff --git a/doubly-stochastic-dgp_amd/csrc/layer_sm_impl.hpp b/doubly-stochastic-dgp_amd/csrc/layer_sm_impl.hpp
--- a/doubly-stochastic-dgp_amd/csrc/layer_sm_impl.hpp
+++ b/doubly-stochastic-dgp_amd/csrc/layer_sm_impl.hpp
@@ -1,5 +1,7 @@
 #pragma once
 #include <stdlib.h>
+
+#include <hip/hip_ext.h>
 
 #include "layer.hpp"
 
@@ -845,7 +847,7 @@
 #define BWD_STAMP(i) do { if (a.phase_clk && tid == 0) a.phase_clk[(int64_t)blockIdx.x * 8 + (i)] = __builtin_amdgcn_s_memrealtime(); } while (0)
 template <int MPB, int NW, bool WIDE, bool CS>
 constexpr int bwd_min_waves() { return (NW == 8 && !WIDE && !CS) ? (MPB <= 8 ? 6 : 4) : ((NW == 4 && MPB == 8 && !WIDE && !CS) ? 5 : 1); }
-template <int MPB, int NW, int KIND, bool WHITE, bool WIDE, bool CS>
+template <int MPB, int NW, int KIND, bool WHITE, bool WIDE, bool CS, bool TS = false>
 __global__ __launch_bounds__(NW * 64, (bwd_min_waves<MPB, NW, WIDE, CS>())) void k_layer_bwd_sm(const LayerBwdArgs a, const SmLds L) {
   extern __shared__ __attribute__((aligned(16))) double smem[];
   constexpr int Mp = MPB * 16, NQ = Own<MPB, NW>::NQ;
@@ -1026,7 +1028,41 @@
   } else {
   __syncthreads();
   constexpr bool PAIRD = (NQ == 2) && !D4 && (MPB % NW == 0);
-  if constexpr (PAIRD) {
+  static_assert(!TS || (!D4 && !CS), "the Tsave d-loop exists for the S_d form at Mp <= 256");
+  if constexpr (TS) {
+    constexpr int DG = NQ >= 4 ? 1 : 4 / NQ;
+    const int64_t rc = rin ? r : 0;
+    for (int d0 = d_lo; d0 < d_hi; d0 += DG) {
+      double vdl[DG], yv[DG][NQ][4];
+#pragma unroll
+      for (int j = 0; j < DG; ++j) {
+        const int d = d0 + j < d_hi ? d0 + j : d_hi - 1;
+        vdl[j] = a.VB[(int64_t)d * a.ldA + rc];
+#pragma unroll
+        for (int q = 0; q < NQ; ++q) {
+          const int ib = Own<MPB, NW>::ib(wave, q);
+          const double* __restrict__ tp = a.Tsave + ((int64_t)d * Mp + 16 * ((act && !Own<MPB, NW>::skip(ib)) ? ib : 0) + g) * a.ldA + rc;
+#pragma unroll
+          for (int t = 0; t < 4; ++t) yv[j][q][t] = tp[(int64_t)(4 * t) * a.ldA];
+        }
+      }
+#pragma unroll
+      for (int j = 0; j < DG; ++j) {
+        if (d0 + j >= d_hi) break;
+        const double vd = rin ? vdl[j] : 0.0;
+        gsum += vd;
+        const double vd2 = 2.0 * vd;
+        if (act) {
+#pragma unroll
+          for (int q = 0; q < NQ; ++q) {
+            if (Own<MPB, NW>::skip(Own<MPB, NW>::ib(wave, q))) continue;
+#pragma unroll
+            for (int t = 0; t < 4; ++t) acc[q][t] = fma(vd2, rin ? yv[j][q][t] : 0.0, acc[q][t]);
+          }
+        }
+      }
+    }
+  } else if constexpr (PAIRD) {
     const int ib0 = Own<MPB, NW>::ib(wave, 0), ib1 = Own<MPB, NW>::ib(wave, 1);
     const unsigned off0 = (unsigned)(g * Mp + 16 * ib0 + c), off1 = (unsigned)(g * Mp + 16 * ib1 + c);
     const int t_last = d_hi * MPB - 1;
@@ -1341,7 +1377,14 @@
             ph[5] * u, (ph[0] + ph[1] + ph[2] + ph[3] + ph[4] + ph[5]) * u);
     return DSDGP_OK;
   }
-  DS_LAUNCH((k_layer_fwd_sm<MPB, NW, KIND, WHITE, WIDE, LIK>), dim3(nrow, ds), dim3(NW * 64), lds, ctx->stream, a, L);
+  if (ctx->chain_done) {
+    g_dsdgp_launches.fetch_add(1, std::memory_order_relaxed);
+    hipExtLaunchKernelGGL((k_layer_fwd_sm<MPB, NW, KIND, WHITE, WIDE, LIK>), dim3(nrow, ds), dim3(NW * 64), (uint32_t)lds, ctx->stream, nullptr,
+                          ctx->chain_done, 0, a, L);
+    ctx->chain_done = nullptr;
+  } else {
+    DS_LAUNCH((k_layer_fwd_sm<MPB, NW, KIND, WHITE, WIDE, LIK>), dim3(nrow, ds), dim3(NW * 64), lds, ctx->stream, a, L);
+  }
   DS_HIP(hipGetLastError());
   return DSDGP_OK;
 }
@@ -1350,14 +1393,14 @@
   if (a.lik_Y) return fwd_sm_go2<MPB, NW, KIND, WHITE, WIDE, true>(ctx, a);
   return fwd_sm_go2<MPB, NW, KIND, WHITE, WIDE, false>(ctx, a);
 }
-template <int MPB, int NW, int KIND, bool WHITE, bool WIDE, bool CS>
+template <int MPB, int NW, int KIND, bool WHITE, bool WIDE, bool CS, bool TS>
 static int bwd_phase_timing(dsdgp_ctx* ctx, const LayerBwdArgs& a0, const SmLds& L, size_t lds) {
   const int nwg = (int)ceil_div(a0.ldA, 16);
   unsigned long long* clk = nullptr;
   DS_HIP(hipMalloc(&clk, (size_t)nwg * 8 * sizeof(unsigned long long)));
   LayerBwdArgs a = a0;
   a.phase_clk = clk;
-  DS_LAUNCH((k_layer_bwd_sm<MPB, NW, KIND, WHITE, WIDE, CS>), dim3(nwg, a.d_split > 1 ? a.d_split : 1), dim3(NW * 64), lds, ctx->stream, a, L);
+  DS_LAUNCH((k_layer_bwd_sm<MPB, NW, KIND, WHITE, WIDE, CS, TS>), dim3(nwg, a.d_split > 1 ? a.d_split : 1), dim3(NW * 64), lds, ctx->stream, a, L);
   DS_HIP(hipStreamSynchronize(ctx->stream));
   std::vector<unsigned long long> h((size_t)nwg * 8);
   DS_HIP(hipMemcpy(h.data(), clk, h.size() * sizeof(unsigned long long), hipMemcpyDeviceToHost));
@@ -1368,12 +1411,12 @@
   }
   phase_span_report(h, nwg, 7);
   const double u = 0.01 / nwg;
-  fprintf(stderr, "[bwd phases] Mp=%d NW=%d D_out=%d wgs=%d  us/wg: A-tile %.2f | d-loop %.2f | mean+abar %.2f | Kinv %.2f | x-stage %.2f | "
-          "kernel+E/GW %.2f | hyp+dX %.2f | sum %.2f\n", MPB * 16, NW, a.D_out, nwg, ph[0] * u, ph[1] * u, ph[2] * u, ph[3] * u, ph[4] * u, ph[5] * u,
+  fprintf(stderr, "[bwd phases] Mp=%d NW=%d D_out=%d wgs=%d%s  us/wg: A-tile %.2f | d-loop %.2f | mean+abar %.2f | Kinv %.2f | x-stage %.2f | "
+          "kernel+E/GW %.2f | hyp+dX %.2f | sum %.2f\n", MPB * 16, NW, a.D_out, nwg, TS ? " Tsave" : "", ph[0] * u, ph[1] * u, ph[2] * u, ph[3] * u, ph[4] * u, ph[5] * u,
           ph[6] * u, (ph[0] + ph[1] + ph[2] + ph[3] + ph[4] + ph[5] + ph[6]) * u);
   return DSDGP_OK;
 }
-template <int MPB, int NW, int KIND, bool WHITE, bool WIDE, bool CS>
+template <int MPB, int NW, int KIND, bool WHITE, bool WIDE, bool CS, bool TS = false>
 static int bwd_sm_go2(dsdgp_ctx* ctx, const LayerBwdArgs& a) {
   const SmLds L = sm_lds(MPB * 16, a.D_in, a.D_out, NW, WIDE, (CS && MPB <= 16) ? 2 : 1);
   const size_t lds = (size_t)L.total * sizeof(double);
@@ -1385,14 +1428,14 @@
     {
       static int lds_set = 0;
       if ((int)lds > lds_set) {
-        DS_HIP(hipFuncSetAttribute((const void*)k_layer_bwd_sm<MPB, NW, KIND, WHITE, WIDE, CS>, hipFuncAttributeMaxDynamicSharedMemorySize, (int)lds));
+        DS_HIP(hipFuncSetAttribute((const void*)k_layer_bwd_sm<MPB, NW, KIND, WHITE, WIDE, CS, TS>, hipFuncAttributeMaxDynamicSharedMemorySize, (int)lds));
         lds_set = (int)lds;
       }
     }
   ProfScope ps(ctx, "layer_bwd");
   static const bool timing = getenv("DSDGP_BWD_TIMING") != nullptr;
-  if (timing) return bwd_phase_timing<MPB, NW, KIND, WHITE, WIDE, CS>(ctx, a, L, lds);
-  DS_LAUNCH((k_layer_bwd_sm<MPB, NW, KIND, WHITE, WIDE, CS>), dim3(ceil_div(a.ldA, 16), a.d_split > 1 ? a.d_split : 1), dim3(NW * 64), lds,
+  if (timing) return bwd_phase_timing<MPB, NW, KIND, WHITE, WIDE, CS, TS>(ctx, a, L, lds);
+  DS_LAUNCH((k_layer_bwd_sm<MPB, NW, KIND, WHITE, WIDE, CS, TS>), dim3(ceil_div(a.ldA, 16), a.d_split > 1 ? a.d_split : 1), dim3(NW * 64), lds,
                      ctx->stream, a, L);
   DS_HIP(hipGetLastError());
   return DSDGP_OK;
@@ -1403,6 +1446,9 @@
 static int bwd_sm_go(dsdgp_ctx* ctx, const LayerBwdArgs& a) {
   if constexpr (sm_cs_inst<MPB, NW>()) {
     if (a.Csave) return bwd_sm_go2<MPB, NW, KIND, WHITE, WIDE, true>(ctx, a);
+  }
+  if constexpr (MPB <= 16) {
+    if (a.Tsave) return bwd_sm_go2<MPB, NW, KIND, WHITE, WIDE, false, true>(ctx, a);
   }
   return bwd_sm_go2<MPB, NW, KIND, WHITE, WIDE, false>(ctx, a);
 }
diff --git a/doubly-stochastic-dgp_amd/csrc/model.hip b/doubly-stochastic-dgp_amd/csrc/model.hip
--- a/doubly-stochastic-dgp_amd/csrc/model.hip
+++ b/doubly-stochastic-dgp_amd/csrc/model.hip
@@ -283,6 +283,8 @@
   const unsigned evf = hipEventDisableTiming;
   for (int l = 0; l < L; ++l) {
     DS_HIP(hipEventCreateWithFlags(&m->ev_bwd[l], evf));
+    DS_HIP(hipEventCreateWithFlags(&m->ev_tfork[l], evf));
+    DS_HIP(hipEventCreateWithFlags(&m->ev_tsave[l], evf));
   }
   DS_HIP(hipEventCreateWithFlags(&m->ev_side, evf));
   DS_HIP(hipEventCreateWithFlags(&m->ev_fork, evf));
@@ -302,6 +304,7 @@
 
     for (int l = 0; l < m->desc.L; ++l) {
       hipEventDestroy(m->ev_bwd[l]);
+      hipEventDestroy(m->ev_tfork[l]); hipEventDestroy(m->ev_tsave[l]);
     }
     hipEventDestroy(m->ev_side);
 
diff --git a/doubly-stochastic-dgp_amd/csrc/model_layout.hpp b/doubly-stochastic-dgp_amd/csrc/model_layout.hpp
--- a/doubly-stochastic-dgp_amd/csrc/model_layout.hpp
+++ b/doubly-stochastic-dgp_amd/csrc/model_layout.hpp
@@ -95,6 +95,8 @@
     const size_t Mw = pad_Mw(v.Mp);
     S.A = b.take<double>(Mw * S.ld_max); S.E = b.take<double>(Mw * S.ld_max); S.GW = b.take<double>(Mw * S.ld_max);
     S.C = save_c_enabled(m->force.save_c, (int)Mp) ? b.take<double>((size_t)d.D_out * Mp * S.ld_max) : nullptr;
+    S.t_cols = tsave_cols(m->force.t_save, l, (int)Mp, m->force.gemm_mp > 0 && v.Mp >= m->force.gemm_mp, S.ld_max);
+    S.T = S.t_cols ? b.take<double>((size_t)d.D_out * Mp * S.t_cols) : nullptr;
     S.VB = b.take<double>(v.DP16 * S.ld_max); S.MB = b.take<double>(v.DP16 * S.ld_max);
     S.XT1 = b.take<double>((size_t)round_up(v.DinP16, 64) * S.ld_max);
     S.F = b.take<double>(S.R_max * d.D_out); S.mean = b.take<double>(S.R_max * d.D_out);
diff --git a/doubly-stochastic-dgp_amd/csrc/model_schedule.hpp b/doubly-stochastic-dgp_amd/csrc/model_schedule.hpp
--- a/doubly-stochastic-dgp_amd/csrc/model_schedule.hpp
+++ b/doubly-stochastic-dgp_amd/csrc/model_schedule.hpp
@@ -188,10 +188,24 @@
     const LayerDev& v = St.dev;
     if (c.zs && c.zs[l]) in.caller_z |= 1u << l;
     in.layer[l] = FwdIn::Layer{v.Mp, v.M, v.D_in, v.D_out, v.kern_kind, St.d.mean_kind, St.prop, St.gemm, v.alg_g != 0, v.need_tpt != 0, St.C != nullptr,
-                               St.bpart != nullptr};
-  }
-  in.force = {f.white_fwd, f.cs_min_blocks, f.cs_min_dout, f.cs_max_dout, f.last_fuse, f.last_min_blocks, f.bwd_split, f.lik_fuse};
+                               St.bpart != nullptr, St.T ? St.t_cols : 0};
+  }
+  in.force = {f.white_fwd, f.cs_min_blocks, f.cs_min_dout, f.cs_max_dout, f.last_fuse, f.last_min_blocks, f.bwd_split, f.lik_fuse, f.t_save};
   return in;
+}
+
+static int tsave_behind_chain(dsdgp_model* m, int l, int64_t ld, bool overlap, bool signalled) {
+  const LayerState& St = m->L[l];
+  const LayerDev& v = St.dev;
+  m->t_on_side[l] = overlap;
+  if (!overlap) return tsave_launch(m->ctx, v.Sd, St.A, St.T, v.Mp, v.D_out, ld, m->ctx->stream);
+  if (!signalled) DS_HIP(hipEventRecord(m->ev_tfork[l], m->ctx->stream));
+  DS_HIP(hipStreamWaitEvent(m->side, m->ev_tfork[l], 0));
+  DS_TRY(tsave_launch(m->ctx, v.Sd, St.A, St.T, v.Mp, v.D_out, ld, m->side));
+  DS_HIP(hipEventRecord(m->ev_tsave[l], m->side));
+  DS_HIP(hipEventRecord(m->ev_prep_side, m->side));
+  m->side_pending = true;
+  return DSDGP_OK;
 }
 
 static int forward_layers(dsdgp_model* m, const FwdCall& c, const FwdIn& in, const FwdPlan& p) {
@@ -232,12 +246,22 @@
       a.lik_Y = c.lik_Y; a.lik_const = m->lik_const; a.lik_w = c.lik_w; a.lik_part = m->lik_part;
       a.lik_MB = St.MB; a.lik_VB = St.VB; a.lik_ld = y.ld;
     }
+    bool t_signalled = false;
     switch (y.launch) {
       case LAUNCH_WITH_REVERSE: break;
       case LAUNCH_GEMM: DS_TRY(layer_fwd_gemm_launch(ctx, a, v.Mp, v.kern_kind, m->desc.white ? 1 : 0, m->gws)); break;
-      case LAUNCH_CHAIN: DS_TRY(layer_fwd_sm_launch(ctx, a, v.Mp, v.kern_kind, m->desc.white || y.whitened)); break;
+      case LAUNCH_CHAIN:
+        if (y.save_T && in.overlap && m->force.t_fork != 0) ctx->chain_done = m->ev_tfork[l];
+        {
+          const int rc = layer_fwd_sm_launch(ctx, a, v.Mp, v.kern_kind, m->desc.white || y.whitened);
+          t_signalled = y.save_T && in.overlap && m->force.t_fork != 0 && ctx->chain_done == nullptr;
+          ctx->chain_done = nullptr;
+          DS_TRY(rc);
+        }
+        break;
     }
     used[l] = FwdUsed{a.X, a.z, a.zs_s, a.zs_n, a.zs_d};
+    if (y.save_T) DS_TRY(tsave_behind_chain(m, l, y.ld, in.overlap, t_signalled));
     if (y.concat) {
       const int64_t R = (int64_t)c.S * c.n, cnt = R * (v.D_out + St.prop);
       DS_LAUNCH(k_concat_prop, dim3((int)std::min<int64_t>(4096, ceil_div(cnt, 256))), dim3(256), 0, ctx->stream, Xin, y.Rin,
@@ -468,7 +492,7 @@
   LayerBwdArgs b{};
   b.X = R.X; b.Rin = R.Rin; b.D_in = v.D_in; b.D_out = v.D_out; b.M = v.M; b.DP4 = v.DP4;
   b.Zp = v.Zp; b.Zs = v.Zs; b.hyp = v.hyp; b.Kinv = v.Kinv; b.Linv = v.Linv; b.LinvT = v.LinvT; b.Sd = v.Sd; b.qmu4 = v.qmu4;
-  b.Asave = St.A; b.Csave = R.c_saved ? St.C : nullptr; b.Tp = v.Tp; b.TpT = v.TpT; b.ldA = R.ld; b.VB = St.VB; b.MB = St.MB;
+  b.Asave = St.A; b.Csave = R.c_saved ? St.C : nullptr; b.Tsave = R.t_saved ? St.T : nullptr; b.Tp = v.Tp; b.TpT = v.TpT; b.ldA = R.ld; b.VB = St.VB; b.MB = St.MB;
   b.E = v.alg_g ? nullptr : St.E; b.GW = St.GW;
   b.dX = (l > sc.gfirst) ? m->L[l - 1].dF : nullptr;
   if (l >= 2 && l > sc.gfirst) {
@@ -571,6 +595,7 @@
                          St.MB, St.VB, St.XT1, v.D_out + St.prop, St.prop);
     DS_HIP(hipGetLastError());
     const LayerBwdArgs b = fill_bwd_args(m, l, sc);
+    if (b.Tsave && m->t_on_side[l]) DS_HIP(hipStreamWaitEvent(ctx->stream, m->ev_tsave[l], 0));
     if (last && m->fwd.last_pending) {
       DS_TRY(layer_last_launch(ctx, m->fwd.last_fwd, b, v.Mp, v.kern_kind, m->fwd.hyp_rows));
       m->fwd.last_launched();
diff --git a/doubly-stochastic-dgp_amd/csrc/model_types.hpp b/doubly-stochastic-dgp_amd/csrc/model_types.hpp
--- a/doubly-stochastic-dgp_amd/csrc/model_types.hpp
+++ b/doubly-stochastic-dgp_amd/csrc/model_types.hpp
@@ -9,6 +9,8 @@
   int64_t R_max;
   int64_t ld_max;
   double* C;
+  double* T = nullptr;
+  int64_t t_cols = 0;
   double *F, *mean, *var, *zbuf, *dF;
   const double *meanA, *meanb;
   int njobs;
@@ -83,8 +85,10 @@
   hipStream_t side;
   hipEvent_t ev_bwd[DSDGP_MAX_LAYERS];
   hipEvent_t ev_side;
+  hipEvent_t ev_tfork[DSDGP_MAX_LAYERS], ev_tsave[DSDGP_MAX_LAYERS];
+  bool t_on_side[DSDGP_MAX_LAYERS] = {};
   bool overlap;
-  struct Force { int save_c = 1, cs_min_blocks = 160, cs_min_dout = 3, cs_max_dout = 1 << 20, wg_defer = -1, alg_g = -1, bwd_split = 1, pipe_tail = 0, head = 1, tail = 1, adj_fuse = 1, ext_ev = 1, lik_fuse = 1, red_ahead = 1, white_fwd = 1, gemm_mp = 512, last_fuse = 1, last_min_blocks = 1, asm_pre = 1, overlap_min = 1 << 18, wg_red = 1, wg_group = 1; } force;
+  struct Force { int save_c = 1, cs_min_blocks = 160, cs_min_dout = 3, cs_max_dout = 1 << 20, wg_defer = -1, alg_g = -1, bwd_split = 1, pipe_tail = 0, head = 1, tail = 1, adj_fuse = 1, ext_ev = 1, lik_fuse = 1, red_ahead = 1, white_fwd = 1, gemm_mp = 512, last_fuse = 1, last_min_blocks = 1, asm_pre = 1, overlap_min = 1 << 18, wg_red = 1, wg_group = 1, t_save = 1, t_fork = 1; } force;
 };
 static void parse_force(dsdgp_model* m) {
   using F = dsdgp_model::Force;
@@ -94,7 +98,7 @@
       {"white_fwd", &F::white_fwd}, {"pipe_tail", &F::pipe_tail}, {"head", &F::head}, {"tail", &F::tail}, {"adj_fuse", &F::adj_fuse},
       {"ext_ev", &F::ext_ev}, {"lik_fuse", &F::lik_fuse}, {"gemm_mp", &F::gemm_mp}, {"last_fuse", &F::last_fuse},
       {"last_min_blocks", &F::last_min_blocks}, {"asm_pre", &F::asm_pre}, {"overlap_min", &F::overlap_min}, {"wg_red", &F::wg_red},
-      {"wg_group", &F::wg_group}};
+      {"wg_group", &F::wg_group}, {"t_save", &F::t_save}, {"t_fork", &F::t_fork}};
   const char* e = getenv("DSDGP_FORCE");
   if (!e) return;
   const std::string str(e);
```

Result: no change. 2007, median of 5 (+0.1%).
